# PreferredAI/cornac

Hardware: AMD Instinct MI355X
Metric: bpr_triplets_per_sec (higher is better)
Workload: dtype f32

## Files before the change

cornac_amd/_lib.py:

```python
import ctypes as C
import os
import subprocess

import numpy as np

_HERE = os.path.dirname(os.path.abspath(__file__))
PROFILE = os.environ.get("CORNAC_HIP_PROFILE", "") == "1"
LIB_PATH = os.path.join(_HERE, "lib", "libcornac_hip_profile.so" if PROFILE else "libcornac_hip.so")
CSRC = os.path.join(_HERE, "csrc")

MODE_DETERMINISTIC = 0
MODE_HOGWILD = 1
VEBPR_NO_OWNERSHIP = 0x100
HOG_FORM_MASK, HOG_FORM_SHIFT = 0xF0000, 16
FORM_AUTO, FORM_FUSED, FORM_STRATA, FORM_LDSBIN = (f << HOG_FORM_SHIFT for f in range(4))
HOG_PLAIN_STORES, HOG_VEC4_LAYOUT, HOG_NO_OWNERSHIP, HOG_DENSE_BIAS, HOG_SHARE_NEG = 1, 2, 4, 8, 16
HOG_BINNED, HOG_FUSED_OPT_OUT = 64, 128
HOG_ABLATE_MASK, HOG_ABLATE_SHIFT = 0xFF00, 8
NEG_UNIFORM = 0
NEG_POPULARITY = 1

SYMBOLS = [
    "cornac_hip_last_error", "cornac_hip_version", "cornac_hip_device_count", "cornac_hip_device_info",
    "cornac_hip_device_probe",
    "cornac_hip_bpr_create", "cornac_hip_bpr_destroy", "cornac_hip_bpr_set_factors", "cornac_hip_bpr_get_factors",
    "cornac_hip_bpr_bind_device", "cornac_hip_bpr_rebind_items", "cornac_hip_bpr_conveyor_setup", "cornac_hip_bpr_conveyor_layout", "cornac_hip_bpr_conveyor_enqueue", "cornac_hip_bpr_set_negative_population", "cornac_hip_bpr_device_ptrs", "cornac_hip_bpr_set_stream",
    "cornac_hip_bpr_seed_mt19937", "cornac_hip_bpr_seed_hogwild", "cornac_hip_bpr_fit_epochs",
    "cornac_hip_bpr_set_factors_f64", "cornac_hip_bpr_get_factors_f64", "cornac_hip_bpr_fit_epochs_f64",
    "cornac_hip_bpr_hogwild_enqueue", "cornac_hip_bpr_sync", "cornac_hip_bpr_debug_draw",
    "cornac_hip_bpr_last_timing", "cornac_hip_bpr_kernel_timing", "cornac_hip_mf_kernel_timing",
    "cornac_hip_bpr_debug_ownership", "cornac_hip_bpr_set_views", "cornac_hip_bpr_seed_view_stream",
    "cornac_hip_vebpr_fit_epochs", "cornac_hip_vebpr_fit_epochs_f64", "cornac_hip_vebpr_hogwild_form",
    "cornac_hip_mmmf_fit_epochs", "cornac_hip_mmmf_fit_epochs_f64", "cornac_hip_mmmf_hogwild_enqueue",
    "cornac_hip_bpr_strata_config", "cornac_hip_bpr_chunk_records", "cornac_hip_bpr_strata_stats", "cornac_hip_bpr_debug_strata",
    "cornac_hip_bpr_ldsbin_config", "cornac_hip_bpr_ldsbin_pass_config", "cornac_hip_bpr_ldsbin_stats",
    "cornac_hip_bpr_ldsbin_deal_config", "cornac_hip_bpr_debug_ldsbin_deal",
    "cornac_hip_bpr_sample_triplets", "cornac_hip_bpr_apply_triplets", "cornac_hip_bpr_gather_rows",
    "cornac_hip_bpr_staged_slots", "cornac_hip_bpr_emit_triplets", "cornac_hip_bpr_apply_staged",
    "cornac_hip_bpr_shard_mark", "cornac_hip_bpr_shard_slots", "cornac_hip_bpr_shard_uniq",
    "cornac_hip_bpr_scatter_diff_rows", "cornac_hip_bpr_switch_stream",
    "cornac_hip_bpr_scatter_add_rows", "cornac_hip_bpr_table_delta_begin", "cornac_hip_bpr_table_delta_finish",
    "cornac_hip_bpr_table_delta_step", "cornac_hip_table_delta", "cornac_hip_bpr_table_delta",
    "cornac_hip_bpr_resident_exchange_bins", "cornac_hip_bpr_epoch_resident_enqueue", "cornac_hip_bpr_resident_flush",
    "cornac_hip_stream_wait_counter", "cornac_hip_stream_set_flag", "cornac_hip_stream_ring_standin",
    "cornac_hip_vbpr_create", "cornac_hip_vbpr_destroy", "cornac_hip_vbpr_set_params", "cornac_hip_vbpr_get_params",
    "cornac_hip_vbpr_fit_batches", "cornac_hip_vbpr_item_tables",
    "cornac_hip_wmf_create", "cornac_hip_wmf_destroy", "cornac_hip_wmf_set_factors", "cornac_hip_wmf_get_factors",
    "cornac_hip_wmf_fit_batches", "cornac_hip_wmf_kernel_timing", "cornac_hip_wmf_last_timing",
    "cornac_hip_mf_create", "cornac_hip_mf_destroy", "cornac_hip_mf_set_factors", "cornac_hip_mf_get_factors",
    "cornac_hip_mf_fit", "cornac_hip_mf_bind_items", "cornac_hip_mf_bind_users", "cornac_hip_mf_set_stream", "cornac_hip_mf_epoch_enqueue",
    "cornac_hip_mf_sync", "cornac_hip_mf_fit_sgd", "cornac_hip_mf_last_timing",
    "cornac_hip_mf_hogwild_form", "cornac_hip_mf_hogwild_stats", "cornac_hip_mf_debug_split", "cornac_hip_mf_debug_ownership",
    "cornac_hip_mf_fit_minibatch", "cornac_hip_mf_fit_minibatch_dropout", "cornac_hip_mf_reset_optimizer",
    "cornac_hip_mf_pmf_set_factors", "cornac_hip_mf_pmf_get_factors", "cornac_hip_mf_pmf_fit", "cornac_hip_mf_pmf_form",
    "cornac_hip_mf_nmf_set_factors", "cornac_hip_mf_nmf_get_factors", "cornac_hip_mf_nmf_fit", "cornac_hip_mf_nmf_form",
    "cornac_hip_mf_hpf_set_tables", "cornac_hip_mf_hpf_get_tables", "cornac_hip_mf_hpf_fit", "cornac_hip_mf_hpf_elog",
    "cornac_hip_mf_hpf_form",
    "cornac_hip_scorer_create", "cornac_hip_scorer_destroy", "cornac_hip_scorer_set", "cornac_hip_score_user",
    "cornac_hip_scorer_set_f64", "cornac_hip_score_user_f64",
    "cornac_hip_score_block", "cornac_hip_rank_topk", "cornac_hip_rank_topk_device", "cornac_hip_score_pairs",
    "cornac_hip_scorer_set_exclusions", "cornac_hip_rank_topk_resident", "cornac_hip_scorer_host_buffer",
    "cornac_hip_rank_positions",
    "cornac_hip_knn_sim_create", "cornac_hip_knn_sim_destroy", "cornac_hip_knn_sim_run", "cornac_hip_knn_sim_nnz",
    "cornac_hip_knn_sim_get",
    "cornac_hip_knn_scorer_create", "cornac_hip_knn_scorer_destroy", "cornac_hip_knn_scorer_score_users",
    "cornac_hip_knn_scorer_score_pairs",
    "cornac_hip_ease_create", "cornac_hip_ease_destroy", "cornac_hip_ease_gram", "cornac_hip_ease_invert",
    "cornac_hip_ease_weights", "cornac_hip_ease_fit", "cornac_hip_ease_get_table", "cornac_hip_ease_set_table",
    "cornac_hip_ease_score_users", "cornac_hip_ease_score_pairs",
    "cornac_hip_vaecf_create", "cornac_hip_vaecf_destroy", "cornac_hip_vaecf_set_params", "cornac_hip_vaecf_get_params",
    "cornac_hip_vaecf_get_state", "cornac_hip_vaecf_reset_optimizer", "cornac_hip_vaecf_fit_epoch",
    "cornac_hip_vaecf_encode_users", "cornac_hip_vaecf_score_users", "cornac_hip_vaecf_score_pairs",
]


class HipError(RuntimeError):

    def __init__(self, code, msg):
        super().__init__("libcornac_hip error %d: %s" % (code, msg))
        self.code = code


def build(force=False, verbose=False):
    cmd = ["make", "-C", CSRC, "-j", "4"] + (["-B"] if force else []) + (["PROFILE=1"] if PROFILE else [])
    out = subprocess.run(cmd, stdout=subprocess.PIPE, stderr=subprocess.STDOUT, text=True)
    if verbose or out.returncode != 0:
        print(out.stdout)
    if out.returncode != 0:
        raise RuntimeError("building libcornac_hip.so failed")
    return LIB_PATH


_lib = None

_f32 = np.ctypeslib.ndpointer(np.float32, flags="C_CONTIGUOUS")
_i32 = np.ctypeslib.ndpointer(np.int32, flags="C_CONTIGUOUS")
_i64 = np.ctypeslib.ndpointer(np.int64, flags="C_CONTIGUOUS")
_vp = C.c_void_p


def _preload_torch_hip_runtime():
    import importlib.util
    import sys

    if "torch" in sys.modules:
        return
    try:
        spec = importlib.util.find_spec("torch")
        libdir = os.path.join(list(spec.submodule_search_locations)[0], "lib")
    except Exception:
        return
    for name in ("libhsa-runtime64.so", "libamdhip64.so"):
        path = os.path.join(libdir, name)
        if os.path.exists(path):
            try:
                C.CDLL(path, mode=C.RTLD_GLOBAL)
            except OSError:
                return


def lib():
    global _lib
    if _lib is None:
        if not os.path.exists(LIB_PATH):
            raise RuntimeError(
                "libcornac_hip.so not found at %s. Build it with `python -c 'import __graft_entry__ as g; g.build()'` "
                "or `make -C cornac_amd/csrc`. cornac_amd has no CPU fallback." % LIB_PATH)
        _preload_torch_hip_runtime()
        L = C.CDLL(LIB_PATH)
        L.cornac_hip_last_error.restype = C.c_char_p
        L.cornac_hip_version.restype = C.c_char_p
        L.cornac_hip_device_count.argtypes = [C.POINTER(C.c_int)]
        L.cornac_hip_device_info.argtypes = [C.c_int, C.c_char_p, C.c_int, C.POINTER(C.c_int), C.POINTER(C.c_int64)]
        L.cornac_hip_device_probe.argtypes = [C.c_int, C.c_int64, C.POINTER(C.c_double)]
        L.cornac_hip_bpr_create.argtypes = [C.POINTER(_vp), C.c_int, C.c_int64, C.c_int64, C.c_int64, C.c_int64,
                                            C.c_int, _i32, _i32, C.c_int64]
        L.cornac_hip_bpr_destroy.argtypes = [_vp]
        L.cornac_hip_bpr_set_factors.argtypes = [_vp, _vp, _vp, _vp]
        L.cornac_hip_bpr_get_factors.argtypes = [_vp, _vp, _vp, _vp]
        L.cornac_hip_bpr_bind_device.argtypes = [_vp, _vp, _vp, _vp]
        L.cornac_hip_bpr_rebind_items.argtypes = [_vp, _vp, _vp]
        L.cornac_hip_bpr_conveyor_setup.argtypes = [_vp, C.c_int, _vp, C.c_uint64, C.c_int, C.POINTER(C.c_int), C.POINTER(C.c_int),
                                                    C.POINTER(C.c_int)]
        L.cornac_hip_bpr_conveyor_layout.argtypes = [_vp, C.c_uint32, _vp, _vp]
        L.cornac_hip_bpr_conveyor_enqueue.argtypes = [_vp, C.c_uint32, C.c_uint32, C.c_int, C.POINTER(C.c_int32), C.POINTER(_vp),
                                                      C.c_float, C.c_float, C.c_int, C.c_int, C.c_int]
        L.cornac_hip_bpr_set_negative_population.argtypes = [_vp, _vp, C.c_int64]
        L.cornac_hip_bpr_device_ptrs.argtypes = [_vp, C.POINTER(_vp), C.POINTER(_vp), C.POINTER(_vp)]
        L.cornac_hip_bpr_set_stream.argtypes = [_vp, _vp]
        L.cornac_hip_bpr_switch_stream.argtypes = [_vp, _vp]
        L.cornac_hip_bpr_seed_mt19937.argtypes = [_vp, C.c_uint32, C.c_uint32, C.c_int]
        L.cornac_hip_bpr_seed_hogwild.argtypes = [_vp, C.c_uint64]
        L.cornac_hip_bpr_fit_epochs.argtypes = [_vp, C.c_int, C.c_float, C.c_float, C.c_int, C.c_int, C.c_int,
                                                C.c_int, C.POINTER(C.c_int64), C.POINTER(C.c_int64)]
        L.cornac_hip_bpr_set_factors_f64.argtypes = [_vp, _vp, _vp, _vp]
        L.cornac_hip_bpr_get_factors_f64.argtypes = [_vp, _vp, _vp, _vp]
        L.cornac_hip_bpr_fit_epochs_f64.argtypes = [_vp, C.c_int, C.c_double, C.c_double, C.c_int, C.c_int,
                                                    C.POINTER(C.c_int64), C.POINTER(C.c_int64)]
        L.cornac_hip_bpr_hogwild_enqueue.argtypes = [_vp, C.c_int64, C.c_float, C.c_float, C.c_int, C.c_int, C.c_int]
        L.cornac_hip_bpr_sync.argtypes = [_vp, C.POINTER(C.c_int64), C.POINTER(C.c_int64)]
        L.cornac_hip_bpr_debug_draw.argtypes = [_vp, C.c_int, C.c_uint64, C.c_int64, _i64]
        L.cornac_hip_bpr_last_timing.argtypes = [_vp, C.POINTER(C.c_double)]
        L.cornac_hip_bpr_set_views.argtypes = [_vp, _i32, _i32, C.c_int64]
        L.cornac_hip_bpr_seed_view_stream.argtypes = [_vp, C.c_uint32]
        L.cornac_hip_vebpr_hogwild_form.argtypes = [_vp, C.POINTER(C.c_int)]
        L.cornac_hip_vebpr_fit_epochs.argtypes = [_vp, C.c_int, C.c_float, C.c_float, C.c_float, C.c_int,
                                                  C.POINTER(C.c_int64), C.POINTER(C.c_int64)]
        L.cornac_hip_vebpr_fit_epochs_f64.argtypes = [_vp, C.c_int, C.c_double, C.c_double, C.c_double,
                                                      C.POINTER(C.c_int64), C.POINTER(C.c_int64)]
        L.cornac_hip_mmmf_fit_epochs.argtypes = [_vp, C.c_int, C.c_float, C.c_float, C.c_int, C.POINTER(C.c_int64),
                                                 C.POINTER(C.c_int64)]
        L.cornac_hip_mmmf_fit_epochs_f64.argtypes = [_vp, C.c_int, C.c_double, C.c_double, C.POINTER(C.c_int64),
                                                     C.POINTER(C.c_int64)]
        L.cornac_hip_mmmf_hogwild_enqueue.argtypes = [_vp, C.c_int64, C.c_float, C.c_float]
        L.cornac_hip_bpr_sample_triplets.argtypes = [_vp, C.c_int64, C.c_int, _vp, _vp, _vp]
        L.cornac_hip_bpr_apply_triplets.argtypes = [_vp, _vp, _vp, _vp, C.c_int64, _vp, _vp, C.c_int, C.c_float,
                                                    C.c_float, C.c_int]
        L.cornac_hip_bpr_gather_rows.argtypes = [_vp, _vp, _vp, C.c_int64, C.c_int, _vp]
        L.cornac_hip_bpr_staged_slots.argtypes = [_vp, C.c_int64, C.POINTER(C.c_int64)]
        L.cornac_hip_bpr_emit_triplets.argtypes = [_vp, C.c_int64, C.c_int, _vp, _vp, _vp, C.c_int64, C.POINTER(C.c_int64)]
        L.cornac_hip_bpr_apply_staged.argtypes = [_vp, _vp, _vp, _vp, C.c_int64, _vp, _vp, C.c_int, C.c_float, C.c_float,
                                                  C.c_int]
        L.cornac_hip_bpr_shard_mark.argtypes = [_vp, _vp, _vp, C.c_int64, C.c_int, C.c_int64, _vp]
        L.cornac_hip_bpr_shard_slots.argtypes = [_vp, _vp, _vp, C.c_int64, C.c_int, C.c_int64, _vp, _vp, _vp]
        L.cornac_hip_bpr_shard_uniq.argtypes = [_vp, _vp, _vp, C.c_int64, C.c_int64, _vp]
        L.cornac_hip_bpr_scatter_diff_rows.argtypes = [_vp, _vp, _vp, C.c_int64, C.c_int, _vp, _vp, _vp]
        L.cornac_hip_bpr_scatter_add_rows.argtypes = [_vp, _vp, _vp, C.c_int64, C.c_int, _vp]
        L.cornac_hip_bpr_table_delta_begin.argtypes = [_vp, _vp, _vp, C.c_int64, C.c_int, _vp, _vp]
        L.cornac_hip_bpr_table_delta_finish.argtypes = [_vp, _vp, _vp, _vp, _vp, C.c_int64, C.c_int]
        L.cornac_hip_bpr_table_delta_step.argtypes = [_vp, _vp, _vp, _vp, _vp, C.c_int64, C.c_int, _vp, _vp]
        L.cornac_hip_table_delta.argtypes = [C.c_int, C.c_int, _vp, _vp, _vp, _vp, _vp, C.c_int64, C.c_int, _vp, _vp]
        L.cornac_hip_bpr_table_delta.argtypes = [_vp, C.c_int, C.c_int, _vp, _vp, _vp, _vp, C.c_int64, C.c_int, _vp, _vp]
        L.cornac_hip_bpr_resident_exchange_bins.argtypes = [_vp, C.c_int, C.c_int, C.POINTER(C.c_int)]
        L.cornac_hip_bpr_epoch_resident_enqueue.argtypes = [_vp, C.c_float, C.c_float, C.c_int, C.c_int, C.c_int, C.c_int,
                                                            C.c_int, _vp, _vp, C.c_int64, _vp, C.c_int64, _vp, _vp, _vp,
                                                            C.POINTER(C.c_int)]
        L.cornac_hip_bpr_resident_flush.argtypes = [_vp, C.c_int, C.c_int, _vp, _vp, C.c_int64, _vp, C.c_int64, _vp, _vp]
        L.cornac_hip_stream_wait_counter.argtypes = [C.c_int, _vp, _vp, C.c_uint32, _vp, C.c_int]
        L.cornac_hip_stream_set_flag.argtypes = [C.c_int, _vp, _vp, C.c_uint32, _vp]
        L.cornac_hip_stream_ring_standin.argtypes = [C.c_int, _vp, _vp, C.c_int64, _vp, C.c_int64, C.c_int64, C.c_int]
        L.cornac_hip_bpr_debug_ownership.argtypes = [_vp, C.POINTER(C.c_int64), _vp, _vp, _vp]
        L.cornac_hip_bpr_strata_config.argtypes = [_vp, C.c_int, C.c_int, C.c_int]
        L.cornac_hip_bpr_chunk_records.argtypes = [_vp, C.c_int]
        L.cornac_hip_bpr_strata_stats.argtypes = [_vp, C.POINTER(C.c_int64)]
        L.cornac_hip_bpr_debug_strata.argtypes = [_vp, C.c_uint32, _vp, _vp, _vp, _vp, C.POINTER(C.c_uint32)]
        L.cornac_hip_bpr_ldsbin_config.argtypes = [_vp, C.c_int, C.c_int, C.c_int]
        L.cornac_hip_bpr_ldsbin_pass_config.argtypes = [_vp, C.c_int, C.c_int, C.c_int, C.c_int]
        L.cornac_hip_bpr_ldsbin_stats.argtypes = [_vp, C.POINTER(C.c_int64)]
        L.cornac_hip_bpr_ldsbin_deal_config.argtypes = [_vp, C.c_int, C.c_int]
        L.cornac_hip_bpr_debug_ldsbin_deal.argtypes = [_vp, C.c_uint64, C.c_uint32, _vp, _vp, _vp, _vp, _vp]
        L.cornac_hip_bpr_kernel_timing.argtypes = [_vp, C.c_int, C.POINTER(C.c_double), C.POINTER(C.c_int64)]
        L.cornac_hip_mf_kernel_timing.argtypes = [_vp, C.c_int, C.POINTER(C.c_double), C.POINTER(C.c_int64)]
        L.cornac_hip_vbpr_create.argtypes = [C.POINTER(_vp), C.c_int, C.c_int64, C.c_int64, C.c_int, C.c_int, C.c_int, _f32]
        L.cornac_hip_vbpr_destroy.argtypes = [_vp]
        L.cornac_hip_vbpr_set_params.argtypes = [_vp] + [_vp] * 6
        L.cornac_hip_vbpr_get_params.argtypes = [_vp] + [_vp] * 6
        L.cornac_hip_vbpr_fit_batches.argtypes = [_vp, _i32, _i32, _i32, C.c_int64, C.c_int, C.c_float, C.c_float,
                                                  C.c_float, C.c_float, C.POINTER(C.c_double)]
        L.cornac_hip_vbpr_item_tables.argtypes = [_vp, _f32, _f32]
        L.cornac_hip_mf_fit_minibatch.argtypes = [_vp, _i64, C.c_int64, C.c_int, C.c_int, C.c_float, C.c_float,
                                                  C.c_float, C.c_int, C.POINTER(C.c_double)]
        L.cornac_hip_mf_fit_minibatch_dropout.argtypes = [_vp, _i64, C.c_int64, C.c_int, C.c_int, C.c_float, C.c_float,
                                                          C.c_float, C.c_int, _vp, _vp, C.c_float, C.POINTER(C.c_double)]
        L.cornac_hip_mf_reset_optimizer.argtypes = [_vp]
        L.cornac_hip_mf_pmf_set_factors.argtypes = [_vp, _vp, _vp]
        L.cornac_hip_mf_pmf_get_factors.argtypes = [_vp, _vp, _vp]
        L.cornac_hip_mf_pmf_fit.argtypes = [_vp, C.c_int, C.c_float, C.c_float, C.c_float, C.c_int, _vp]
        L.cornac_hip_mf_pmf_form.argtypes = [_vp, C.POINTER(C.c_int), C.POINTER(C.c_int)]
        L.cornac_hip_mf_nmf_set_factors.argtypes = [_vp, _vp, _vp, _vp, _vp]
        L.cornac_hip_mf_nmf_get_factors.argtypes = [_vp, _vp, _vp, _vp, _vp]
        L.cornac_hip_mf_nmf_fit.argtypes = [_vp, C.c_int] + [C.c_float] * 6 + [C.c_int, C.c_int, _vp]
        L.cornac_hip_mf_nmf_form.argtypes = [_vp] + [C.POINTER(C.c_int)] * 3
        L.cornac_hip_mf_hpf_set_tables.argtypes = [_vp] * 5
        L.cornac_hip_mf_hpf_get_tables.argtypes = [_vp] * 7
        L.cornac_hip_mf_hpf_fit.argtypes = [_vp, C.c_int, C.c_int]
        L.cornac_hip_mf_hpf_elog.argtypes = [_vp, _vp, _vp]
        L.cornac_hip_mf_hpf_form.argtypes = [_vp] + [C.POINTER(C.c_int)] * 2
        L.cornac_hip_wmf_create.argtypes = [C.POINTER(_vp), C.c_int, C.c_int64, C.c_int64, C.c_int, _i64, _i32, _f32,
                                            C.c_int64]
        L.cornac_hip_wmf_destroy.argtypes = [_vp]
        L.cornac_hip_wmf_destroy.restype = None
        L.cornac_hip_wmf_set_factors.argtypes = [_vp, _f32, _f32]
        L.cornac_hip_wmf_get_factors.argtypes = [_vp, _f32, _f32]
        L.cornac_hip_wmf_fit_batches.argtypes = [_vp, _i32, _i64, C.c_int64, C.c_float, C.c_float, C.c_float,
                                                 C.c_float, C.c_float, _vp]
        L.cornac_hip_wmf_kernel_timing.argtypes = [_vp, C.c_int]
        L.cornac_hip_wmf_last_timing.argtypes = [_vp, C.POINTER(C.c_double)]
        L.cornac_hip_mf_create.argtypes = [C.POINTER(_vp), C.c_int, C.c_int64, C.c_int64, C.c_int, _i64, _i64, _f32,
                                           C.c_int64]
        L.cornac_hip_mf_destroy.argtypes = [_vp]
        L.cornac_hip_mf_set_factors.argtypes = [_vp, _vp, _vp, _vp, _vp]
        L.cornac_hip_mf_get_factors.argtypes = [_vp, _vp, _vp, _vp, _vp]
        L.cornac_hip_mf_bind_items.argtypes = [_vp, _vp, _vp]
        L.cornac_hip_mf_bind_users.argtypes = [_vp, _vp, _vp]
        L.cornac_hip_mf_set_stream.argtypes = [_vp, _vp]
        L.cornac_hip_mf_epoch_enqueue.argtypes = [_vp, C.c_int, C.c_int, C.c_float, C.c_float, C.c_float, C.c_int]
        L.cornac_hip_mf_sync.argtypes = [_vp, C.POINTER(C.c_double)]
        L.cornac_hip_mf_fit.argtypes = [_vp, C.c_int, C.c_float, C.c_float, C.c_float, C.c_int, C.c_int, C.c_int, _vp,
                                        C.POINTER(C.c_int)]
        L.cornac_hip_mf_fit_sgd.argtypes = [C.c_int, _i64, _i64, _f32, C.c_int64, _f32, _f32, _f32, _f32, C.c_int64,
                                            C.c_int64, C.c_int, C.c_float, C.c_float, C.c_float, C.c_int, C.c_int,
                                            C.c_int, C.c_int, _vp, C.POINTER(C.c_int)]
        L.cornac_hip_mf_last_timing.argtypes = [_vp, C.POINTER(C.c_double)]
        L.cornac_hip_mf_hogwild_form.argtypes = [_vp, C.c_int]
        L.cornac_hip_mf_hogwild_stats.argtypes = [_vp, C.POINTER(C.c_int64)]
        L.cornac_hip_mf_debug_split.argtypes = [_vp, C.POINTER(C.c_int64), C.POINTER(C.c_int64), _vp, _vp]
        L.cornac_hip_mf_debug_ownership.argtypes = [_vp, C.POINTER(C.c_int64), _vp, _vp, _vp]
        L.cornac_hip_scorer_create.argtypes = [C.POINTER(_vp), C.c_int, C.c_int64, C.c_int64, C.c_int]
        L.cornac_hip_scorer_destroy.argtypes = [_vp]
        L.cornac_hip_scorer_set.argtypes = [_vp, _f32, _f32, _vp, _vp]
        L.cornac_hip_score_user.argtypes = [_vp, C.c_int64, _f32]
        L.cornac_hip_scorer_set_f64.argtypes = [_vp, _vp, _vp, _vp, _vp]
        L.cornac_hip_score_user_f64.argtypes = [_vp, C.c_int64, _vp]
        L.cornac_hip_score_block.argtypes = [_vp, _i32, C.c_int64, _f32]
        L.cornac_hip_score_pairs.argtypes = [_vp, _i32, _i32, C.c_int64, C.c_int, C.c_float, C.c_float, _f32]
        L.cornac_hip_rank_topk.argtypes = [_vp, _i32, C.c_int64, C.c_int, _vp, _vp, _i32, _f32]
        L.cornac_hip_rank_positions.argtypes = [_vp, _i32, C.c_int64, _vp, _vp, _vp, _vp, _i32, _i32, _i32, _f32]
        L.cornac_hip_rank_topk_device.argtypes = [_vp, C.c_int64, C.c_int64, C.c_int, C.c_int, C.POINTER(C.c_double)]
        L.cornac_hip_scorer_set_exclusions.argtypes = [_vp, _vp, _vp]
        L.cornac_hip_scorer_host_buffer.argtypes = [_vp, C.c_size_t, C.POINTER(_vp)]
        L.cornac_hip_rank_topk_resident.argtypes = [_vp, _vp, C.c_int64, C.c_int64, C.c_int, _vp, _vp, _vp]
        L.cornac_hip_knn_sim_create.argtypes = [C.POINTER(_vp), C.c_int, C.c_int64, C.c_int64, _vp, _vp, _vp]
        L.cornac_hip_knn_sim_destroy.argtypes = [_vp]
        L.cornac_hip_knn_sim_run.argtypes = [_vp, C.c_int64]
        L.cornac_hip_knn_sim_nnz.argtypes = [_vp, C.POINTER(C.c_int64)]
        L.cornac_hip_knn_sim_get.argtypes = [_vp, _vp, _vp, _vp]
        L.cornac_hip_knn_scorer_create.argtypes = [C.POINTER(_vp), C.c_int, C.c_int64, C.c_int64, C.c_int64] + [_vp] * 6 + [C.c_int]
        L.cornac_hip_knn_scorer_destroy.argtypes = [_vp]
        L.cornac_hip_knn_scorer_score_users.argtypes = [_vp, _vp, C.c_int64, C.c_int, _vp]
        L.cornac_hip_knn_scorer_score_pairs.argtypes = [_vp, _vp, _vp, C.c_int64, C.c_int, _vp]
        L.cornac_hip_ease_create.argtypes = [C.POINTER(_vp), C.c_int, C.c_int64, C.c_int64, _vp, _vp, _vp]
        L.cornac_hip_ease_destroy.argtypes = [_vp]
        L.cornac_hip_ease_gram.argtypes = [_vp]
        L.cornac_hip_ease_invert.argtypes = [_vp, C.c_double]
        L.cornac_hip_ease_weights.argtypes = [_vp, C.c_int]
        L.cornac_hip_ease_fit.argtypes = [_vp, C.c_double, C.c_int]
        L.cornac_hip_ease_get_table.argtypes = [_vp, _vp]
        L.cornac_hip_ease_set_table.argtypes = [_vp, _vp]
        L.cornac_hip_ease_score_users.argtypes = [_vp, _vp, C.c_int64, _vp]
        L.cornac_hip_ease_score_pairs.argtypes = [_vp, _vp, _vp, C.c_int64, _vp]
        L.cornac_hip_vaecf_create.argtypes = [C.POINTER(_vp), C.c_int, C.c_int64, C.c_int64, _vp, _vp, C.c_int, C.c_int, C.c_int,
                                              C.c_int]
        L.cornac_hip_vaecf_destroy.argtypes = [_vp]
        L.cornac_hip_vaecf_set_params.argtypes = [_vp, _vp]
        L.cornac_hip_vaecf_get_params.argtypes = [_vp, _vp]
        L.cornac_hip_vaecf_get_state.argtypes = [_vp, _vp, _vp, C.POINTER(C.c_int64)]
        L.cornac_hip_vaecf_reset_optimizer.argtypes = [_vp]
        L.cornac_hip_vaecf_fit_epoch.argtypes = [_vp, C.c_int64, C.c_float, C.c_float, _vp, C.c_uint64, C.POINTER(C.c_double), _vp]
        L.cornac_hip_vaecf_encode_users.argtypes = [_vp, _vp, C.c_int64, _vp]
        L.cornac_hip_vaecf_score_users.argtypes = [_vp, _vp, C.c_int64, _vp]
        L.cornac_hip_vaecf_score_pairs.argtypes = [_vp, _vp, _vp, C.c_int64, _vp]
        _lib = L
    return _lib


def check(rc):
    if rc != 0:
        raise HipError(rc, lib().cornac_hip_last_error().decode("utf-8", "replace"))


def stream_wait_counter(device, stream, d_counter, target, d_error, timeout_ms=5000):
    check(lib().cornac_hip_stream_wait_counter(int(device), stream, d_counter, int(target), d_error, int(timeout_ms)))


def stream_ring_standin(device, stream, d_src, src_floats, d_dst, dst_floats, n_floats, n_workgroups=16):
    check(lib().cornac_hip_stream_ring_standin(int(device), stream, d_src, int(src_floats), d_dst, int(dst_floats),
                                               int(n_floats), int(n_workgroups)))


def stream_set_flag(device, stream, d_flag, value=1, d_unless=None):
    check(lib().cornac_hip_stream_set_flag(int(device), stream, d_flag, int(value), d_unless))


def device_count():
    n = C.c_int(0)
    check(lib().cornac_hip_device_count(C.byref(n)))
    return n.value


def device_probe(device=0, nbytes=6 << 30):
    o = (C.c_double * 3)()
    check(lib().cornac_hip_device_probe(device, int(nbytes), o))
    return {"d2d_copy_GBps": o[0], "stream_read_GBps": o[1], "row_gather_512B_GBps": o[2], "buffer_bytes": int(nbytes)}


def device_info(device=0):
    name = C.create_string_buffer(256)
    cus = C.c_int()
    mem = C.c_int64()
    check(lib().cornac_hip_device_info(device, name, 256, C.byref(cus), C.byref(mem)))
    return {"name": name.value.decode(), "compute_units": cus.value, "hbm_bytes": mem.value}


def _ptr(a):
    return None if a is None else a.ctypes.data


def _f32c(a):
    return None if a is None else np.ascontiguousarray(a, dtype=np.float32)


class _HandleOwner:
    _DESTROY = None
    _HANDLE = "h"

    def close(self):
        h = getattr(self, self._HANDLE, None)
        if h is not None and h and lib is not None:
            getattr(lib(), self._DESTROY)(h)
            setattr(self, self._HANDLE, None)

    __del__ = close


def _score_by_ids(symbol, h, dtype, users, items=None, width=None, extra=()):
    ids = [np.ascontiguousarray(users, np.int32)] + ([] if items is None else [np.ascontiguousarray(items, np.int32)])
    n = len(ids[0])
    assert all(len(a) == n for a in ids)
    out = np.empty(n if width is None else (n, width), dtype)
    check(getattr(lib(), symbol)(h, *[_ptr(a) for a in ids], n, *extra, _ptr(out)))
    return out


class BprTrainer(_HandleOwner):
    _DESTROY = "cornac_hip_bpr_destroy"

    def __init__(self, indptr, indices, n_users, n_items, total_users, total_items, k, device=0):
        self.indptr = np.ascontiguousarray(indptr, np.int32)
        self.indices = np.ascontiguousarray(indices, np.int32)
        self.shape = (int(total_users), int(total_items), int(k))
        self.nnz = len(self.indices)
        self.n_items = int(n_items)
        self.device, self._stream = int(device), None
        self.h = _vp()
        check(lib().cornac_hip_bpr_create(C.byref(self.h), device, n_users, n_items, total_users, total_items, k,
                                          self.indptr, self.indices, self.nnz))

    def set_factors(self, U=None, V=None, B=None):
        U, V, B = _f32c(U), _f32c(V), _f32c(B)
        tu, ti, k = self.shape
        assert U is None or U.shape == (tu, k)
        assert V is None or V.shape == (ti, k)
        assert B is None or B.shape == (ti,)
        check(lib().cornac_hip_bpr_set_factors(self.h, _ptr(U), _ptr(V), _ptr(B)))

    def get_factors(self):
        tu, ti, k = self.shape
        U, V, B = np.empty((tu, k), np.float32), np.empty((ti, k), np.float32), np.empty(ti, np.float32)
        check(lib().cornac_hip_bpr_get_factors(self.h, U.ctypes.data, V.ctypes.data, B.ctypes.data))
        return U, V, B

    def set_factors_f64(self, U, V, B):
        tu, ti, k = self.shape
        U, V, B = (np.ascontiguousarray(a, np.float64) for a in (U, V, B))
        assert U.shape == (tu, k) and V.shape == (ti, k) and B.shape == (ti,)
        check(lib().cornac_hip_bpr_set_factors_f64(self.h, U.ctypes.data, V.ctypes.data, B.ctypes.data))

    def get_factors_f64(self):
        tu, ti, k = self.shape
        U, V, B = np.empty((tu, k), np.float64), np.empty((ti, k), np.float64), np.empty(ti, np.float64)
        check(lib().cornac_hip_bpr_get_factors_f64(self.h, U.ctypes.data, V.ctypes.data, B.ctypes.data))
        return U, V, B

    def fit_epochs_f64(self, n_epochs, lr, reg, use_bias=True, neg_population=NEG_UNIFORM):
        c, s = C.c_int64(), C.c_int64()
        check(lib().cornac_hip_bpr_fit_epochs_f64(self.h, n_epochs, float(lr), float(reg), int(use_bias), neg_population,
                                                  C.byref(c), C.byref(s)))
        return c.value, s.value

    def get_user_factors(self):
        tu, _, k = self.shape
        U = np.empty((tu, k), np.float32)
        check(lib().cornac_hip_bpr_get_factors(self.h, U.ctypes.data, None, None))
        return U

    def get_item_factors(self):
        _, ti, k = self.shape
        V, B = np.empty((ti, k), np.float32), np.empty(ti, np.float32)
        check(lib().cornac_hip_bpr_get_factors(self.h, None, V.ctypes.data, B.ctypes.data))
        return V, B

    def seed_mt19937(self, seed_pos, seed_neg, shared_stream=False):
        check(lib().cornac_hip_bpr_seed_mt19937(self.h, seed_pos, seed_neg, int(shared_stream)))

    def seed_hogwild(self, seed):
        check(lib().cornac_hip_bpr_seed_hogwild(self.h, int(seed) & 0xFFFFFFFFFFFFFFFF))

    def fit_epochs(self, n_epochs, lr, reg, use_bias=True, neg_population=NEG_UNIFORM, mode=MODE_HOGWILD, flags=0):
        c, s = C.c_int64(), C.c_int64()
        check(lib().cornac_hip_bpr_fit_epochs(self.h, n_epochs, lr, reg, int(use_bias), neg_population, mode, flags,
                                              C.byref(c), C.byref(s)))
        return c.value, s.value

    def hogwild_enqueue(self, n_samples, lr, reg, use_bias=True, neg_population=NEG_UNIFORM, flags=0):
        check(lib().cornac_hip_bpr_hogwild_enqueue(self.h, n_samples, lr, reg, int(use_bias), neg_population, flags))

    def sync(self):
        c, s = C.c_int64(), C.c_int64()
        check(lib().cornac_hip_bpr_sync(self.h, C.byref(c), C.byref(s)))
        return c.value, s.value

    def bind_device(self, dU=None, dV=None, dB=None):
        check(lib().cornac_hip_bpr_bind_device(self.h, dU, dV, dB))

    def set_negative_population(self, items):
        items = np.ascontiguousarray(items if items is not None else [], np.int32)
        check(lib().cornac_hip_bpr_set_negative_population(self.h, items.ctypes.data if len(items) else None, len(items)))

    def rebind_items(self, dV, dB):
        check(lib().cornac_hip_bpr_rebind_items(self.h, dV, dB))

    def conveyor_setup(self, n_blocks, rank_item=None, deal_seed=0, release_item_tables=True):
        order = None if rank_item is None else np.ascontiguousarray(rank_item, np.int32)
        nb, bpb, cap = C.c_int(), C.c_int(), C.c_int()
        check(lib().cornac_hip_bpr_conveyor_setup(self.h, int(n_blocks), None if order is None else order.ctypes.data,
                                                  int(deal_seed) & 0xFFFFFFFFFFFFFFFF, int(bool(release_item_tables)),
                                                  C.byref(nb), C.byref(bpb), C.byref(cap)))
        return nb.value, bpb.value, cap.value

    def conveyor_layout(self, layout_epoch, d_slot_item, d_item_slot):
        check(lib().cornac_hip_bpr_conveyor_layout(self.h, int(layout_epoch), d_slot_item, d_item_slot))

    def conveyor_enqueue(self, epoch, layout_epoch, first_blocks, d_rows, lr, reg, use_bias=True, neg_population=NEG_UNIFORM,
                         flags=0):
        n = len(first_blocks)
        fb = (C.c_int32 * n)(*[int(b) for b in first_blocks])
        rows = (_vp * n)(*[int(p) for p in d_rows])
        check(lib().cornac_hip_bpr_conveyor_enqueue(self.h, int(epoch), int(layout_epoch), n, fb, rows, lr, reg, int(use_bias),
                                                    neg_population, int(flags)))

    def device_ptrs(self):
        u, v, b = _vp(), _vp(), _vp()
        check(lib().cornac_hip_bpr_device_ptrs(self.h, C.byref(u), C.byref(v), C.byref(b)))
        return u.value, v.value, b.value

    def set_stream(self, stream_ptr):
        check(lib().cornac_hip_bpr_set_stream(self.h, stream_ptr))
        self._stream = stream_ptr

    def switch_stream(self, stream_ptr):
        check(lib().cornac_hip_bpr_switch_stream(self.h, stream_ptr))
        self._stream = stream_ptr

    def sample_triplets(self, n_draws, d_u, d_i, d_j, neg_population=NEG_UNIFORM):
        check(lib().cornac_hip_bpr_sample_triplets(self.h, int(n_draws), neg_population, d_u, d_i, d_j))

    def apply_triplets(self, d_u, d_slot_i, d_slot_j, n, d_rows, d_bias, bias_stride, lr, reg, use_bias=True):
        check(lib().cornac_hip_bpr_apply_triplets(self.h, d_u, d_slot_i, d_slot_j, int(n), d_rows, d_bias,
                                                  int(bias_stride), lr, reg, int(use_bias)))

    def staged_slots(self, n_draws):
        n = C.c_int64()
        check(lib().cornac_hip_bpr_staged_slots(self.h, int(n_draws), C.byref(n)))
        return n.value

    def emit_triplets(self, n_draws, d_u, d_i, d_j, slots_cap, neg_population=NEG_UNIFORM):
        n = C.c_int64()
        check(lib().cornac_hip_bpr_emit_triplets(self.h, int(n_draws), neg_population, d_u, d_i, d_j, int(slots_cap),
                                                 C.byref(n)))
        return n.value

    def apply_staged(self, d_u, d_slot_i, d_slot_j, n_slots, d_rows, d_bias, bias_stride, lr, reg, use_bias=True):
        check(lib().cornac_hip_bpr_apply_staged(self.h, d_u, d_slot_i, d_slot_j, int(n_slots), d_rows, d_bias,
                                                int(bias_stride), lr, reg, int(use_bias)))

    def shard_mark(self, d_i, d_j, n, world, rows_per_rank, d_mark):
        check(lib().cornac_hip_bpr_shard_mark(self.h, d_i, d_j, int(n), int(world), int(rows_per_rank), d_mark))

    def shard_slots(self, d_i, d_j, n, world, rows_per_rank, d_scan, d_slot_i, d_slot_j):
        check(lib().cornac_hip_bpr_shard_slots(self.h, d_i, d_j, int(n), int(world), int(rows_per_rank), d_scan, d_slot_i,
                                               d_slot_j))

    def shard_uniq(self, d_mark, d_scan, n_rows, rows_per_rank, d_uniq_local):
        check(lib().cornac_hip_bpr_shard_uniq(self.h, d_mark, d_scan, int(n_rows), int(rows_per_rank), d_uniq_local))

    def scatter_diff_rows(self, d_table, d_ids, n, width, d_now, d_before, d_scale=None):
        check(lib().cornac_hip_bpr_scatter_diff_rows(self.h, d_table, d_ids, int(n), int(width), d_now, d_before, d_scale))

    def _delta(self, op, rule, *args):
        check(lib().cornac_hip_bpr_table_delta(self.h, op, int(rule), *args))

    def table_delta_begin(self, d_flat, d_base, n_items, k, d_bucket, d_local, rule=0):
        if rule:
            return self._delta(0, rule, d_flat, d_base, None, None, int(n_items), int(k), d_bucket, d_local)
        check(lib().cornac_hip_bpr_table_delta_begin(self.h, d_flat, d_base, int(n_items), int(k), d_bucket, d_local))

    def table_delta_finish(self, d_flat, d_base, d_bucket, d_local, n_items, k, rule=0):
        if rule:
            return self._delta(1, rule, d_flat, d_base, d_bucket, d_local, int(n_items), int(k), None, None)
        check(lib().cornac_hip_bpr_table_delta_finish(self.h, d_flat, d_base, d_bucket, d_local, int(n_items), int(k)))

    def table_delta_step(self, d_flat, d_base, d_bucket_prev, d_local_prev, n_items, k, d_bucket, d_local, rule=0):
        if rule:
            return self._delta(2, rule, d_flat, d_base, d_bucket_prev, d_local_prev, int(n_items), int(k), d_bucket, d_local)
        check(lib().cornac_hip_bpr_table_delta_step(self.h, d_flat, d_base, d_bucket_prev, d_local_prev, int(n_items),
                                                    int(k), d_bucket, d_local))

    def resident_exchange_bins(self, neg_population=NEG_UNIFORM, flags=0):
        n = C.c_int()
        check(lib().cornac_hip_bpr_resident_exchange_bins(self.h, neg_population, flags, C.byref(n)))
        return n.value

    def epoch_resident_enqueue(self, lr, reg, use_bias, neg_population, flags, n_exchanges, rule, d_base, d_buckets,
                               bucket_stride, d_keeps, keep_stride, d_arrive, d_landed, d_applied):
        n = C.c_int()
        check(lib().cornac_hip_bpr_epoch_resident_enqueue(self.h, lr, reg, int(use_bias), neg_population, flags,
                                                          int(n_exchanges), int(rule), d_base, d_buckets, int(bucket_stride),
                                                          d_keeps, int(keep_stride), d_arrive, d_landed, d_applied, C.byref(n)))
        return n.value

    def resident_flush(self, n_exchanges, rule, d_base, d_buckets, bucket_stride, d_keeps, keep_stride, d_applied, d_landed=None):
        check(lib().cornac_hip_bpr_resident_flush(self.h, int(n_exchanges), int(rule), d_base, d_buckets, int(bucket_stride),
                                                  d_keeps, int(keep_stride), d_applied, d_landed))

    def gather_rows(self, d_table, d_ids, n, width, d_out):
        check(lib().cornac_hip_bpr_gather_rows(self.h, d_table, d_ids, int(n), int(width), d_out))

    def scatter_add_rows(self, d_table, d_ids, n, width, d_delta):
        check(lib().cornac_hip_bpr_scatter_add_rows(self.h, d_table, d_ids, int(n), int(width), d_delta))

    def debug_draw(self, stream, hi, n):
        out = np.empty(n, np.int64)
        check(lib().cornac_hip_bpr_debug_draw(self.h, stream, hi, n, out))
# ... 129 lines not shown
        nu, ni, k = self.shape
        U, V = np.empty((nu, k), np.float32), np.empty((ni, k), np.float32)
        Bu, Bi = np.empty(nu, np.float32), np.empty(ni, np.float32)
        check(lib().cornac_hip_mf_get_factors(self.h, U.ctypes.data, V.ctypes.data, Bu.ctypes.data, Bi.ctypes.data))
        return U, V, Bu, Bi

    def fit(self, max_iter, lr, reg, mu, use_bias=True, early_stop=False, mode=MODE_HOGWILD):
        loss = np.zeros(max(max_iter, 1), np.float32)
        n = C.c_int()
        check(lib().cornac_hip_mf_fit(self.h, max_iter, lr, reg, mu, int(use_bias), int(early_stop), mode,
                                      loss.ctypes.data, C.byref(n)))
        return loss[:n.value], n.value

    def bind_items(self, d_V, d_Bi):
        check(lib().cornac_hip_mf_bind_items(self.h, d_V, d_Bi))

    def bind_users(self, d_U, d_Bu):
        check(lib().cornac_hip_mf_bind_users(self.h, d_U, d_Bu))

    def set_stream(self, hip_stream):
        check(lib().cornac_hip_mf_set_stream(self.h, hip_stream))
        self._stream = hip_stream

    def epoch_enqueue(self, part, n_parts, lr, reg, mu, use_bias=True):
        check(lib().cornac_hip_mf_epoch_enqueue(self.h, int(part), int(n_parts), lr, reg, mu, int(use_bias)))

    def sync(self):
        l = C.c_double()
        check(lib().cornac_hip_mf_sync(self.h, C.byref(l)))
        return l.value

    def table_delta_begin(self, d_flat, d_base, n_items, k, d_bucket, d_local, rule=0):
        check(lib().cornac_hip_table_delta(0 | (int(rule) << 4), self.device, self._stream, d_flat, d_base, None, None,
                                           int(n_items), int(k), d_bucket, d_local))

    def table_delta_finish(self, d_flat, d_base, d_bucket, d_local, n_items, k, rule=0):
        check(lib().cornac_hip_table_delta(1 | (int(rule) << 4), self.device, self._stream, d_flat, d_base, d_bucket, d_local,
                                           int(n_items), int(k), None, None))

    def table_delta_step(self, d_flat, d_base, d_bucket_prev, d_local_prev, n_items, k, d_bucket, d_local, rule=0):
        check(lib().cornac_hip_table_delta(2 | (int(rule) << 4), self.device, self._stream, d_flat, d_base, d_bucket_prev,
                                           d_local_prev, int(n_items), int(k), d_bucket, d_local))

    OPTIMIZERS = {"sgd": 0, "adam": 1, "rmsprop": 2, "adagrad": 3}

    def fit_minibatch(self, order, batch_size, optimizer, lr, reg, mu, use_bias=True, keep_u=None, keep_i=None,
                      keep_scale=1.0):
        order = np.ascontiguousarray(order, np.int64)
        loss = C.c_double()
        if keep_u is not None:
            keep_u, keep_i = np.ascontiguousarray(keep_u, np.uint8), np.ascontiguousarray(keep_i, np.uint8)
            if keep_u.shape != (len(order), self.shape[2]) or keep_i.shape != keep_u.shape:
                raise ValueError("keep masks must be [len(order), k] = %r, got %r / %r"
                                 % ((len(order), self.shape[2]), keep_u.shape, keep_i.shape))
            check(lib().cornac_hip_mf_fit_minibatch_dropout(self.h, order, len(order), int(batch_size),
                                                            self.OPTIMIZERS[optimizer], lr, reg, mu, int(use_bias),
                                                            keep_u.ctypes.data, keep_i.ctypes.data, float(keep_scale),
                                                            C.byref(loss)))
            return loss.value
        check(lib().cornac_hip_mf_fit_minibatch(self.h, order, len(order), int(batch_size), self.OPTIMIZERS[optimizer],
                                                lr, reg, mu, int(use_bias), C.byref(loss)))
        return loss.value

    def reset_optimizer(self):
        check(lib().cornac_hip_mf_reset_optimizer(self.h))

    PMF_VARIANTS = {"linear": 0, "non_linear": 1}

    def pmf_set_factors(self, U, V):
        nu, ni, k = self.shape
        U, V = np.ascontiguousarray(U, np.float64), np.ascontiguousarray(V, np.float64)
        if U.shape != (nu, k) or V.shape != (ni, k):
            raise ValueError("PMF tables must be %r and %r, got %r and %r" % ((nu, k), (ni, k), U.shape, V.shape))
        check(lib().cornac_hip_mf_pmf_set_factors(self.h, U.ctypes.data, V.ctypes.data))

    def pmf_get_factors(self):
        nu, ni, k = self.shape
        U, V = np.empty((nu, k), np.float64), np.empty((ni, k), np.float64)
        check(lib().cornac_hip_mf_pmf_get_factors(self.h, U.ctypes.data, V.ctypes.data))
        return U, V

    def pmf_fit(self, n_epochs, lr, reg, gamma, variant):
        loss = np.zeros(max(int(n_epochs), 1), np.float64)
        check(lib().cornac_hip_mf_pmf_fit(self.h, int(n_epochs), lr, reg, gamma, self.PMF_VARIANTS.get(variant, variant),
                                          loss.ctypes.data))
        return loss[:max(int(n_epochs), 0)]

    def pmf_form(self):
        form, group = C.c_int(), C.c_int()
        check(lib().cornac_hip_mf_pmf_form(self.h, C.byref(form), C.byref(group)))
        return form.value, group.value

    def nmf_set_factors(self, U, V, Bu=None, Bi=None):
        nu, ni, k = self.shape
        U, V, Bu, Bi = _f32c(U), _f32c(V), _f32c(Bu), _f32c(Bi)
        if U.shape != (nu, k) or V.shape != (ni, k):
            raise ValueError("NMF tables must be %r and %r, got %r and %r" % ((nu, k), (ni, k), U.shape, V.shape))
        if (Bu is not None and Bu.shape != (nu,)) or (Bi is not None and Bi.shape != (ni,)):
            raise ValueError("NMF biases must be (%d,) and (%d,)" % (nu, ni))
        check(lib().cornac_hip_mf_nmf_set_factors(self.h, _ptr(U), _ptr(V), _ptr(Bu), _ptr(Bi)))

    def nmf_get_factors(self):
        nu, ni, k = self.shape
        U, V = np.empty((nu, k), np.float32), np.empty((ni, k), np.float32)
        Bu, Bi = np.empty(nu, np.float32), np.empty(ni, np.float32)
        check(lib().cornac_hip_mf_nmf_get_factors(self.h, U.ctypes.data, V.ctypes.data, Bu.ctypes.data, Bi.ctypes.data))
        return U, V, Bu, Bi

    def nmf_fit(self, n_epochs, lr, lambda_u, lambda_v, lambda_bu, lambda_bi, mu, use_bias=False, mode=MODE_HOGWILD):
        loss = np.zeros(max(int(n_epochs), 1), np.float64)
        check(lib().cornac_hip_mf_nmf_fit(self.h, int(n_epochs), lr, lambda_u, lambda_v, lambda_bu, lambda_bi, mu,
                                          int(bool(use_bias)), int(mode), loss.ctypes.data))
        return loss[:max(int(n_epochs), 0)]

    def nmf_form(self):
        o = [C.c_int(), C.c_int(), C.c_int()]
        check(lib().cornac_hip_mf_nmf_form(self.h, *[C.byref(x) for x in o]))
        return tuple(x.value for x in o)

    HPF_MAX_K = 256

    def hpf_set_tables(self, G_s, G_r, L_s, L_r):
        nu, ni, k = self.shape
        if k > self.HPF_MAX_K:
            raise ValueError("HPF keeps a row's sums in registers: k = %d is above its limit of %d" % (k, self.HPF_MAX_K))
        tables = [np.ascontiguousarray(a, np.float64) for a in (G_s, G_r, L_s, L_r)]
        for a, name, shape in zip(tables, ("G_s", "G_r", "L_s", "L_r"), ((nu, k), (nu, k), (ni, k), (ni, k))):
            if a.shape != shape:
                raise ValueError("HPF table %s must be %r, got %r" % (name, shape, a.shape))
            if not (np.isfinite(a).all() and (a > 0).all()):
                raise ValueError("HPF table %s must be strictly positive and finite" % name)
        check(lib().cornac_hip_mf_hpf_set_tables(self.h, *[a.ctypes.data for a in tables]))

    def hpf_get_tables(self):
        nu, ni, k = self.shape
        out = [np.empty(s, np.float64) for s in ((nu, k), (nu, k), (ni, k), (ni, k), (nu,), (ni,))]
        check(lib().cornac_hip_mf_hpf_get_tables(self.h, *[a.ctypes.data for a in out]))
        return tuple(out)

    def hpf_fit(self, n_iters, hierarchical=True):
        check(lib().cornac_hip_mf_hpf_fit(self.h, int(n_iters), int(bool(hierarchical))))

    def hpf_elog(self):
        nu, ni, k = self.shape
        Lt, Lb = np.empty((nu, k), np.float64), np.empty((ni, k), np.float64)
        check(lib().cornac_hip_mf_hpf_elog(self.h, Lt.ctypes.data, Lb.ctypes.data))
        return Lt, Lb

    def hpf_form(self):
        o = [C.c_int(), C.c_int()]
        check(lib().cornac_hip_mf_hpf_form(self.h, *[C.byref(x) for x in o]))
        return tuple(x.value for x in o)

    def kernel_timing(self, enable=True):
        ms, n = C.c_double(), C.c_int64()
        check(lib().cornac_hip_mf_kernel_timing(self.h, int(enable), C.byref(ms), C.byref(n)))
        return ms.value, n.value

    def hogwild_form(self, form):
        check(lib().cornac_hip_mf_hogwild_form(self.h, int(form)))

    def hogwild_stats(self):
        o = (C.c_int64 * 4)()
        check(lib().cornac_hip_mf_hogwild_stats(self.h, o))
        return {"form_used": o[0], "tiles": o[1], "rows_per_bin": o[2], "gave_up": bool(o[3])}

    def debug_split(self):
        ns, nv = C.c_int64(), C.c_int64()
        check(lib().cornac_hip_mf_debug_split(self.h, C.byref(ns), C.byref(nv), None, None))
        items, ptr = np.empty(ns.value, np.int32), np.zeros(ns.value + 1, np.int32)
        if ns.value:
            check(lib().cornac_hip_mf_debug_split(self.h, C.byref(ns), C.byref(nv), items.ctypes.data, ptr.ctypes.data))
        return items, ptr

    def debug_ownership(self):
        w = C.c_int64()
        check(lib().cornac_hip_mf_debug_ownership(self.h, C.byref(w), None, None, None))
        if w.value == 0:
            return None
        wp = np.empty(w.value + 1, np.int64)
        ou, oi = np.empty(len(self.val), np.int32), np.empty(len(self.val), np.int32)
        check(lib().cornac_hip_mf_debug_ownership(self.h, C.byref(w), wp.ctypes.data, ou.ctypes.data, oi.ctypes.data))
        return wp, ou, oi

    def last_timing(self):
        t = (C.c_double * 4)()
        check(lib().cornac_hip_mf_last_timing(self.h, t))
        return {"schedule_ms": t[1], "sgd_ms": t[2], "total_ms": t[3]}


def mf_fit_sgd(rid, cid, val, U, V, Bu, Bi, lr, reg, mu, max_iter, use_bias, early_stop, mode, device=0):
    loss = np.zeros(max(max_iter, 1), np.float32)
    n = C.c_int()
    check(lib().cornac_hip_mf_fit_sgd(device, np.ascontiguousarray(rid, np.int64), np.ascontiguousarray(cid, np.int64),
                                      np.ascontiguousarray(val, np.float32), len(val), U, V, Bu, Bi, U.shape[0],
                                      V.shape[0], U.shape[1], lr, reg, mu, max_iter, int(use_bias), int(early_stop),
                                      mode, loss.ctypes.data, C.byref(n)))
    return loss[:n.value]


class Scorer(_HandleOwner):
    _DESTROY = "cornac_hip_scorer_destroy"

    def __init__(self, U, V, item_base=None, user_base=None, device=0):
        U, V = _f32c(U), _f32c(V)
        self.n_users, self.k = U.shape
        self.n_items = V.shape[0]
        self.h = _vp()
        check(lib().cornac_hip_scorer_create(C.byref(self.h), device, self.n_users, self.n_items, self.k))
        self.set(U, V, item_base, user_base)

    def set(self, U, V, item_base=None, user_base=None):
        ib, ub = _f32c(item_base), _f32c(user_base)
        check(lib().cornac_hip_scorer_set(self.h, _f32c(U), _f32c(V), _ptr(ib), _ptr(ub)))

    def score_user(self, user):
        out = np.empty(self.n_items, np.float32)
        check(lib().cornac_hip_score_user(self.h, int(user), out))
        return out

    def set_f64(self, U, V, item_base=None, user_base=None):
        U, V = np.ascontiguousarray(U, np.float64), np.ascontiguousarray(V, np.float64)
        assert U.shape == (self.n_users, self.k) and V.shape == (self.n_items, self.k)
        ib = None if item_base is None else np.ascontiguousarray(item_base, np.float64)
        ub = None if user_base is None else np.ascontiguousarray(user_base, np.float64)
        check(lib().cornac_hip_scorer_set_f64(self.h, U.ctypes.data, V.ctypes.data, _ptr(ib), _ptr(ub)))

    def score_user_f64(self, user):
        out = np.empty(self.n_items, np.float64)
        check(lib().cornac_hip_score_user_f64(self.h, int(user), out.ctypes.data))
        return out

    def score_block(self, users):
        users = np.ascontiguousarray(users, np.int32)
        out = np.empty((len(users), self.n_items), np.float32)
        check(lib().cornac_hip_score_block(self.h, users, len(users), out))
        return out

    def score_pairs(self, users, items, clip=None):
        users = np.ascontiguousarray(users, np.int32)
        items = np.ascontiguousarray(items, np.int32)
        out = np.empty(len(users), np.float32)
        lo, hi = (0.0, 0.0) if clip is None else (float(clip[0]), float(clip[1]))
        check(lib().cornac_hip_score_pairs(self.h, users, items, len(users), int(clip is not None), lo, hi, out))
        return out

    def rank_topk(self, users, topk, exclude=None):
        users = np.ascontiguousarray(users, np.int32)
        items = np.empty((len(users), topk), np.int32)
        scores = np.empty((len(users), topk), np.float32)
        ip = ix = None
        if exclude is not None:
            ip = np.ascontiguousarray(exclude[0], np.int64)
            ix = np.ascontiguousarray(exclude[1], np.int32)
        check(lib().cornac_hip_rank_topk(self.h, users, len(users), topk, _ptr(ip), _ptr(ix), items, scores))
        return items, scores

    def rank_positions(self, users, targets, exclude=None):
        users = np.ascontiguousarray(users, np.int32)
        tp = np.ascontiguousarray(targets[0], np.int64)
        tx = np.ascontiguousarray(targets[1], np.int32)
        nt = int(tp[-1])
        greater, pos, ge = (np.empty(nt, np.int32) for _ in range(3))
        scores = np.empty(nt, np.float32)
        ip = ix = None
        if exclude is not None:
            ip = np.ascontiguousarray(exclude[0], np.int64)
            ix = np.ascontiguousarray(exclude[1], np.int32)
        check(lib().cornac_hip_rank_positions(self.h, users, len(users), _ptr(ip), _ptr(ix), _ptr(tp), _ptr(tx), greater,
                                              pos, ge, scores))
        return greater, pos, ge, scores

    def set_exclusions(self, indptr=None, indices=None):
        if indptr is None:
            check(lib().cornac_hip_scorer_set_exclusions(self.h, None, None))
            return
        ip = np.ascontiguousarray(indptr, np.int64)
        ix = np.ascontiguousarray(indices, np.int32)
        assert len(ip) == self.n_users + 1
        check(lib().cornac_hip_scorer_set_exclusions(self.h, ip.ctypes.data, _ptr(ix) if len(ix) else None))

    def rank_topk_resident(self, users, topk, fetch=True, timed=False, pinned=False):
        if isinstance(users, tuple):
            up, u0, n = None, int(users[0]), int(users[1])
        else:
            ua = np.ascontiguousarray(users, np.int32)
            up, u0, n = ua.ctypes.data, 0, len(ua)
        if fetch and pinned:
            want_scores = fetch != "items"
            nbytes = n * topk * 4 * (2 if want_scores else 1)
            buf = _vp()
            check(lib().cornac_hip_scorer_host_buffer(self.h, nbytes, C.byref(buf)))
            raw = (C.c_char * nbytes).from_address(buf.value)
            items = np.frombuffer(raw, np.int32, n * topk).reshape(n, topk)
            scores = np.frombuffer(raw, np.float32, n * topk, offset=n * topk * 4).reshape(n, topk) if want_scores else None
        else:
            items = np.empty((n, topk), np.int32) if fetch else None
            scores = np.empty((n, topk), np.float32) if fetch and fetch != "items" else None
        ms = C.c_double()
        check(lib().cornac_hip_rank_topk_resident(self.h, up, u0, n, topk, _ptr(items), _ptr(scores),
                                                  C.cast(C.byref(ms), _vp) if timed else None))
        return (items, scores, ms.value) if timed else (items, scores)

    def rank_topk_device_ms(self, u0, n, topk, repeats=1):
        ms = C.c_double()
        check(lib().cornac_hip_rank_topk_device(self.h, u0, n, topk, repeats, C.byref(ms)))
        return ms.value


class VbprTrainer(_HandleOwner):
    _DESTROY = "cornac_hip_vbpr_destroy"
    NAMES = ("Bi", "Gu", "Gi", "Tu", "E", "Bp")

    def __init__(self, features, n_users, n_items, k, k2, device=0):
        self.F = np.ascontiguousarray(features, np.float32)
        assert self.F.shape[0] == n_items
        self.dims = dict(n_users=int(n_users), n_items=int(n_items), k=int(k), k2=int(k2), n_feat=self.F.shape[1])
        self.h = _vp()
        check(lib().cornac_hip_vbpr_create(C.byref(self.h), device, n_users, n_items, k, k2, self.F.shape[1], self.F))

    def _shapes(self):
        d = self.dims
        return {"Bi": (d["n_items"],), "Gu": (d["n_users"], d["k"]), "Gi": (d["n_items"], d["k"]),
                "Tu": (d["n_users"], d["k2"]), "E": (d["n_feat"], d["k2"]), "Bp": (d["n_feat"],)}

    def set_params(self, **params):
        arrs = []
        for n in self.NAMES:
            a = params.get(n)
            if a is not None:
                a = np.ascontiguousarray(np.asarray(a, np.float32).reshape(self._shapes()[n]))
            arrs.append(a)
        check(lib().cornac_hip_vbpr_set_params(self.h, *[_ptr(a) for a in arrs]))

    def get_params(self):
        out = {n: np.empty(s, np.float32) for n, s in self._shapes().items()}
        check(lib().cornac_hip_vbpr_get_params(self.h, *[out[n].ctypes.data for n in self.NAMES]))
        return out

    def fit_batches(self, u, i, j, batch_size, lr, lambda_w, lambda_b, lambda_e):
        u, i, j = (np.ascontiguousarray(x, np.int32) for x in (u, i, j))
        nll = C.c_double()
        check(lib().cornac_hip_vbpr_fit_batches(self.h, u, i, j, len(u), batch_size, lr, lambda_w, lambda_b, lambda_e,
                                                C.byref(nll)))
        return nll.value

    def item_tables(self):
        d = self.dims
        th, vb = np.empty((d["n_items"], d["k2"]), np.float32), np.empty(d["n_items"], np.float32)
        check(lib().cornac_hip_vbpr_item_tables(self.h, th, vb))
        return th, vb


class WmfTrainer(_HandleOwner):
    _DESTROY = "cornac_hip_wmf_destroy"

    def __init__(self, csc, k, device=0):
        csc = csc.tocsc()
        self.n_users, self.n_items = (int(x) for x in csc.shape)
        self.k = int(k)
        self._indptr = np.ascontiguousarray(csc.indptr, np.int64)
        self._rows = np.ascontiguousarray(csc.indices, np.int32)
        self._vals = np.ascontiguousarray(csc.data, np.float32)
        self.h = _vp()
        check(lib().cornac_hip_wmf_create(C.byref(self.h), device, self.n_users, self.n_items, self.k, self._indptr,
                                          self._rows if len(self._rows) else np.zeros(1, np.int32),
                                          self._vals if len(self._vals) else np.zeros(1, np.float32), len(self._vals)))

    def set_factors(self, U, V):
        U = np.ascontiguousarray(np.asarray(U, np.float32).reshape(self.n_users, self.k))
        V = np.ascontiguousarray(np.asarray(V, np.float32).reshape(self.n_items, self.k))
        check(lib().cornac_hip_wmf_set_factors(self.h, U, V))

    def get_factors(self):
        U, V = np.empty((self.n_users, self.k), np.float32), np.empty((self.n_items, self.k), np.float32)
        check(lib().cornac_hip_wmf_get_factors(self.h, U, V))
        return U, V

    def fit_batches(self, batches, lambda_u, lambda_v, a, b, lr):
        batches = [np.asarray(x, np.int32).ravel() for x in batches]
        if not batches:
            return np.zeros(0)
        ptr = np.zeros(len(batches) + 1, np.int64)
        np.cumsum([len(x) for x in batches], out=ptr[1:])
        ids = np.ascontiguousarray(np.concatenate(batches), np.int32)
        loss = np.zeros(len(batches), np.float64)
        check(lib().cornac_hip_wmf_fit_batches(self.h, ids, ptr, len(batches), lambda_u, lambda_v, a, b, lr,
                                               loss.ctypes.data))
        return loss

    def kernel_timing(self, enabled=True):
        check(lib().cornac_hip_wmf_kernel_timing(self.h, int(enabled)))

    def last_device_ms(self):
        ms = C.c_double()
        check(lib().cornac_hip_wmf_last_timing(self.h, C.byref(ms)))
        return ms.value


KNN_MAX_K = 64


def _csr_arrays(mat):
    mat = mat.tocsr()
    if not mat.has_sorted_indices:
        mat = mat.sorted_indices()
    return (np.ascontiguousarray(mat.indptr, np.int64), np.ascontiguousarray(mat.indices, np.int32),
            np.ascontiguousarray(mat.data, np.float64))


class KnnSimilarity(_HandleOwner):
    _DESTROY = "cornac_hip_knn_sim_destroy"

    def __init__(self, W, device=0):
        self.shape = tuple(int(x) for x in W.shape)
        self._csr = _csr_arrays(W)
        self.h = _vp()
        check(lib().cornac_hip_knn_sim_create(C.byref(self.h), device, self.shape[0], self.shape[1],
                                              *[_ptr(a) for a in self._csr]))

    def run(self, rows_per_pass=0):
        import scipy.sparse as sp

        check(lib().cornac_hip_knn_sim_run(self.h, int(rows_per_pass)))
        nnz = C.c_int64()
        check(lib().cornac_hip_knn_sim_nnz(self.h, C.byref(nnz)))
        n = self.shape[0]
        indptr, indices, data = np.empty(n + 1, np.int64), np.empty(nnz.value, np.int32), np.empty(nnz.value, np.float64)
        check(lib().cornac_hip_knn_sim_get(self.h, _ptr(indptr), _ptr(indices), _ptr(data)))
        return sp.csr_matrix((data, indices, indptr.astype(np.int32) if nnz.value < 2 ** 31 else indptr), shape=(n, n))


class KnnScorer(_HandleOwner):
    _DESTROY = "cornac_hip_knn_scorer_destroy"

    MAX_K = KNN_MAX_K

    def __init__(self, N, Q, user_mode, device=0):
        self.n_items, self.n_neighbours = (int(x) for x in N.shape)
        self.n_users = int(Q.shape[0])
        assert int(Q.shape[1]) == self.n_neighbours, "N and Q must have the same number of columns"
        n, q = _csr_arrays(N), _csr_arrays(Q)
        self.h = _vp()
        check(lib().cornac_hip_knn_scorer_create(C.byref(self.h), device, self.n_items, self.n_neighbours, self.n_users,
                                                 *[_ptr(a) for a in n + q], int(bool(user_mode))))

    def score_users(self, users, k):
        return _score_by_ids("cornac_hip_knn_scorer_score_users", self.h, np.float64, users, width=self.n_items, extra=(int(k),))

    def score_pairs(self, users, items, k):
        return _score_by_ids("cornac_hip_knn_scorer_score_pairs", self.h, np.float64, users, items, extra=(int(k),))


class EaseModel(_HandleOwner):
    _DESTROY = "cornac_hip_ease_destroy"

    def __init__(self, X, device=0):
        self.n_users, self.n_items = (int(x) for x in X.shape)
        csr = _csr_arrays(X)
        self.h = _vp()
        check(lib().cornac_hip_ease_create(C.byref(self.h), device, self.n_users, self.n_items, *[_ptr(a) for a in csr]))

    def gram(self):
        check(lib().cornac_hip_ease_gram(self.h))

    def invert(self, lamb):
        check(lib().cornac_hip_ease_invert(self.h, float(lamb)))

    def weights(self, posB):
        check(lib().cornac_hip_ease_weights(self.h, int(bool(posB))))

    def fit(self, lamb, posB):
        check(lib().cornac_hip_ease_fit(self.h, float(lamb), int(bool(posB))))

    def get_table(self):
        out = np.empty((self.n_items, self.n_items), np.float64)
        check(lib().cornac_hip_ease_get_table(self.h, _ptr(out)))
        return out

    def set_table(self, table):
        table = np.ascontiguousarray(table, np.float64)
        assert table.shape == (self.n_items, self.n_items), "the table is items x items"
        check(lib().cornac_hip_ease_set_table(self.h, _ptr(table)))

    def score_users(self, users):
        return _score_by_ids("cornac_hip_ease_score_users", self.h, np.float64, users, width=self.n_items)

    def score_pairs(self, users, items):
        return _score_by_ids("cornac_hip_ease_score_pairs", self.h, np.float64, users, items)


class VaecfModel(_HandleOwner):
    _DESTROY = "cornac_hip_vaecf_destroy"
    _HANDLE = "h_"
    NAMES = ("encoder.fc0.weight", "encoder.fc0.bias", "enc_mu.weight", "enc_mu.bias", "enc_logvar.weight", "enc_logvar.bias",
             "decoder.fc0.weight", "decoder.fc0.bias", "decoder.fc1.weight", "decoder.fc1.bias")
    ACTS = ("tanh", "sigmoid", "relu", "relu6", "elu")
    LIKELIHOODS = ("mult", "bern", "gaus", "pois")

    @staticmethod
    def shapes(n_items, k, h):
        return dict(zip(VaecfModel.NAMES, ((h, n_items), (h,), (k, h), (k,), (k, h), (k,), (h, k), (h,), (n_items, h), (n_items,))))

    def __init__(self, X, k, h, act_fn="tanh", likelihood="mult", device=0):
        self.n_users, self.n_items = (int(x) for x in X.shape)
        self.k, self.h = int(k), int(h)
        indptr, indices, _ = _csr_arrays(X)
        self.h_ = _vp()
        check(lib().cornac_hip_vaecf_create(C.byref(self.h_), device, self.n_users, self.n_items, _ptr(indptr), _ptr(indices),
                                            self.k, self.h, self.ACTS.index(act_fn), self.LIKELIHOODS.index(likelihood)))

    def _empty(self):
        sh = self.shapes(self.n_items, self.k, self.h)
        return {n: np.empty(sh[n], np.float32) for n in self.NAMES}

    def _pointers(self, tables):
        return (_vp * 10)(*[None if tables.get(n) is None else tables[n].ctypes.data for n in self.NAMES])

    def set_params(self, params):
        sh = self.shapes(self.n_items, self.k, self.h)
        tables = {n: np.ascontiguousarray(a, np.float32) for n, a in params.items() if a is not None}
        for n, a in tables.items():
            assert a.shape == sh[n], "%s is %r, not %r" % (n, a.shape, sh[n])
        check(lib().cornac_hip_vaecf_set_params(self.h_, self._pointers(tables)))

    def get_params(self):
        out = self._empty()
        check(lib().cornac_hip_vaecf_get_params(self.h_, self._pointers(out)))
        return out

    def get_state(self):
        m, v, t = self._empty(), self._empty(), C.c_int64()
        check(lib().cornac_hip_vaecf_get_state(self.h_, self._pointers(m), self._pointers(v), C.byref(t)))
        return m, v, int(t.value)

    def reset_optimizer(self):
        check(lib().cornac_hip_vaecf_reset_optimizer(self.h_))

    def fit_epoch(self, batch_size, lr, beta, eps=None, seed=0):
        if eps is not None:
            eps = np.ascontiguousarray(eps, np.float32)
            assert eps.shape == (self.n_users, self.k)
        steps = np.zeros(max(1, -(-self.n_users // max(int(batch_size), 1))), np.float64)
        total = C.c_double()
        check(lib().cornac_hip_vaecf_fit_epoch(self.h_, int(batch_size), float(lr), float(beta), _ptr(eps),
                                               int(seed) & 0xFFFFFFFFFFFFFFFF, C.byref(total), _ptr(steps)))
        return float(total.value), steps

    def encode_users(self, users):
        return _score_by_ids("cornac_hip_vaecf_encode_users", self.h_, np.float32, users, width=self.h)

    def score_users(self, users):
        return _score_by_ids("cornac_hip_vaecf_score_users", self.h_, np.float32, users, width=self.n_items)

    def score_pairs(self, users, items):
        return _score_by_ids("cornac_hip_vaecf_score_pairs", self.h_, np.float32, users, items)
```

cornac_amd/csrc/score.hip:

```cpp
#include <algorithm>
#include <cmath>
#include <cstdlib>

#include "common.h"

namespace chip {

constexpr int kBlk = 256;
typedef float f32x16 __attribute__((ext_vector_type(16)));
typedef float v4f32 __attribute__((ext_vector_type(4)));

__device__ __forceinline__ uint32_t order_key(float s) {
    const uint32_t b = __float_as_uint(s);
    const uint32_t k = (b & 0x80000000u) ? ~b : (b | 0x80000000u);
    return k ? k : 1u;
}
__device__ __forceinline__ float key_to_float(uint32_t k) {
    const uint32_t b = (k & 0x80000000u) ? (k & 0x7fffffffu) : ~k;
    return __uint_as_float(b);
}

__global__ __launch_bounds__(kBlk) void score_valu_kernel(const float *__restrict__ U, const float *__restrict__ V,
                                                          const float *__restrict__ item_base,
                                                          const float *__restrict__ user_base,
                                                          const int32_t *__restrict__ users, int64_t u0,
                                                          int64_t n_items, int k, int ld, float *__restrict__ out) {
    extern __shared__ float urow[];
    const int64_t b = blockIdx.y;
    const int64_t u = users ? (int64_t)users[b] : u0 + b;
    for (int f = threadIdx.x; f < k; f += kBlk) urow[f] = U[u * ld + f];
    __syncthreads();
    const int64_t i = (int64_t)blockIdx.x * kBlk + threadIdx.x;
    if (i >= n_items) return;
    const float *row = V + i * ld;
    float acc = 0.f;
    for (int f = 0; f < k; ++f) acc = fmaf(urow[f], row[f], acc);
    const float ub = user_base ? user_base[u] : 0.f;
    const float ib = item_base ? item_base[i] : 0.f;
    out[b * n_items + i] = (ib + ub) + acc;
}

__global__ __launch_bounds__(kBlk) void score_pairs_kernel(const float *__restrict__ U, const float *__restrict__ V,
                                                           const float *__restrict__ item_base,
                                                           const float *__restrict__ user_base,
                                                           const int32_t *__restrict__ users,
                                                           const int32_t *__restrict__ items, int64_t n, int k, int ld,
                                                           int do_clip, float lo, float hi, float *__restrict__ out) {
    const int64_t p = (int64_t)blockIdx.x * kBlk + threadIdx.x;
    if (p >= n) return;
    const int64_t u = users[p], i = items[p];
    const float *pu = U + u * ld, *pv = V + i * ld;
    float acc = 0.f;
    for (int f = 0; f < k; ++f) acc = fmaf(pu[f], pv[f], acc);
    float s = ((item_base ? item_base[i] : 0.f) + (user_base ? user_base[u] : 0.f)) + acc;
    if (do_clip) s = fminf(fmaxf(s, lo), hi);
    out[p] = s;
}

template <int KT, int MT>
__global__ __launch_bounds__(kBlk) void score_gemm_mfma_kernel(const float *__restrict__ U,
                                                               const float *__restrict__ V,
                                                               const float *__restrict__ item_base,
                                                               const float *__restrict__ user_base,
                                                               const int32_t *__restrict__ users, int64_t u0,
                                                               int64_t n_rows, int64_t n_items, int k,
                                                               int tiles_per_strip, float *__restrict__ out) {
    const int wave = threadIdx.x >> 6, lane = threadIdx.x & 63;
    const int col = lane & 31, half = lane >> 5;
    const int64_t row_tile0 = ((int64_t)blockIdx.y * (kBlk / 64) + wave) * MT;
    if (row_tile0 * 32 >= n_rows) return;
    float a[MT][KT];
    float ubias[MT];
    int64_t urow[MT];
#pragma unroll
    for (int m = 0; m < MT; ++m) {
        const int64_t r = (row_tile0 + m) * 32 + col;
        const bool ok = r < n_rows;
        const int64_t u = ok ? (users ? (int64_t)users[r] : u0 + r) : 0;
        urow[m] = u;
        const float *p = U + u * (2 * KT) + half;
#pragma unroll
        for (int t = 0; t < KT; ++t) a[m][t] = p[2 * t];
        ubias[m] = 0.f;
    }
    const int64_t n_item_tiles = (n_items + 31) / 32;
    const int64_t t_begin = (int64_t)blockIdx.x * tiles_per_strip;
    const int64_t t_end = min(n_item_tiles, t_begin + tiles_per_strip);
    for (int64_t it = t_begin; it < t_end; ++it) {
        const int64_t item = it * 32 + col;
        const bool iok = item < n_items;
        const float *q = V + (iok ? item : 0) * (2 * KT) + half;
        float bfrag[KT];
#pragma unroll
        for (int t = 0; t < KT; ++t) bfrag[t] = q[2 * t];
        const float ib = (iok && item_base) ? item_base[item] : 0.f;
#pragma unroll
        for (int m = 0; m < MT; ++m) {
            f32x16 acc = {0.f, 0.f, 0.f, 0.f, 0.f, 0.f, 0.f, 0.f, 0.f, 0.f, 0.f, 0.f, 0.f, 0.f, 0.f, 0.f};
#pragma unroll
            for (int t = 0; t < KT; ++t) acc = __builtin_amdgcn_mfma_f32_32x32x2f32(a[m][t], bfrag[t], acc, 0, 0, 0);
            if (iok) {
#pragma unroll
                for (int r = 0; r < 16; ++r) {
                    const int64_t row = (row_tile0 + m) * 32 + (r & 3) + 8 * (r >> 2) + 4 * half;
                    if (row < n_rows) {
                        float ub = 0.f;
                        if (user_base) ub = user_base[users ? (int64_t)users[row] : u0 + row];
                        out[row * n_items + item] = (ib + ub) + acc[r];
                    }
                }
            }
        }
    }
    (void)ubias;
    (void)urow;
}

template <typename T>
__device__ __forceinline__ uint32_t lds_offset(T *p) {
    return (uint32_t)(uintptr_t)(__attribute__((address_space(3))) T *)p;
}

template <int KT, int CAP, bool UB>
__global__ __launch_bounds__(kBlk, ((KT <= 32 || CAP <= 42) ? 2 : 1)) void rank_fused_kernel(const float *__restrict__ U, const float *__restrict__ V,
                                                          const float *__restrict__ item_base,
                                                          const float *__restrict__ user_base,
                                                          const int32_t *__restrict__ users, int64_t u0,
                                                          int64_t n_rows, int64_t n_items, int64_t work_per_wg,
                                                          int topk, const int64_t *__restrict__ excl_indptr,
                                                          const int32_t *__restrict__ excl_indices, int64_t excl_row0,
                                                          const uint32_t *__restrict__ excl_bits,
                                                          const int32_t *__restrict__ perm, float *tau_pub,
                                                          unsigned long long *__restrict__ part, int ablate) {
    constexpr int KP = 2 * KT;
    __shared__ unsigned long long keys[kBlk / 64][32][CAP];
    __shared__ int32_t ipos[3][32];
    __shared__ int cnt[kBlk / 64][32];
    __shared__ float tau[kBlk / 64][32];
    __shared__ float btile[2][32][KP + 1];
    __shared__ uint32_t meta_dump[1];
    __shared__ uint32_t wmask[3][kBlk / 64][32];
    __shared__ float ibase[3][32];
    const int wave = threadIdx.x >> 6, lane = threadIdx.x & 63;
    const int col = lane & 31, half = lane >> 5;
    const int64_t n_item_tiles = (n_items + 31) / 32;
    const int64_t n_row_blocks = (n_rows + 127) / 128;
    const int64_t work_total = n_row_blocks * n_item_tiles;
    int64_t pos = (int64_t)blockIdx.x * work_per_wg;
    const int64_t work_end = min(work_total, pos + work_per_wg);
    int64_t cur_rb = 0;
    float bcur[KT];
    constexpr int STG = (32 * KP / 4 + kBlk - 1) / kBlk;
    v4f32 stg[STG];
    uint32_t voff[STG];
#pragma unroll
    for (int q = 0; q < STG; ++q) {
        const int idx = threadIdx.x + q * kBlk;
        voff[q] = idx < 32 * KP / 4 ? (uint32_t)(((idx / (KP / 4)) * KP + 4 * (idx % (KP / 4))) * 4) : 0u;
    }
    uint32_t stg_a = 0;
    int32_t stg_id = 0;
    const uint32_t *pa = reinterpret_cast<const uint32_t *>(item_base);
    int64_t pa_stride = 0;
    const bool wave0 = __builtin_amdgcn_readfirstlane((int)(threadIdx.x >> 6)) == 0;
    const int32_t *pb = perm;
    auto stage_seek = [&](int64_t it) {
        if (threadIdx.x < 32) {
            pa = reinterpret_cast<const uint32_t *>(item_base) + it * 32 + threadIdx.x;
            pa_stride = 32;
        } else if (excl_bits && threadIdx.x < 32 + 32 * (kBlk / 64) && !(ablate & 32)) {
            const int w = (threadIdx.x - 32) >> 5, rl = (threadIdx.x - 32) & 31;
            pa = excl_bits + ((cur_rb * (kBlk / 64) + w) * 32 + rl) * n_item_tiles + it;
            pa_stride = 1;
        } else {
            pa = reinterpret_cast<const uint32_t *>(item_base);
            pa_stride = 0;
        }
        pb = perm + it * 32 + (threadIdx.x & 31);
    };
    auto stage_load = [&](int64_t it) {
        const char *vb = reinterpret_cast<const char *>(V) + it * (int64_t)(32 * KP * 4);
#pragma unroll
        for (int q = 0; q < STG; ++q) stg[q] = *reinterpret_cast<const v4f32 *>(vb + voff[q]);
        stg_a = *pa;
        pa += pa_stride;
        if (wave0) {
            stg_id = *pb;
            pb += 32;
        }
    };
    uint32_t meta_addr0 = lds_offset(&meta_dump[0]), meta_stride = 0;
    if (threadIdx.x < 32) {
        meta_addr0 = lds_offset(&ibase[0][threadIdx.x]);
        meta_stride = 32 * sizeof(float);
    } else if (excl_bits && threadIdx.x < 32 + 32 * (kBlk / 64)) {
        meta_addr0 = lds_offset(&wmask[0][(threadIdx.x - 32) >> 5][(threadIdx.x - 32) & 31]);
        meta_stride = (kBlk / 64) * 32 * sizeof(uint32_t);
    }
    auto stage_store = [&](int buf, int wbuf) {
#pragma unroll
        for (int q = 0; q < STG; ++q) {
            const int idx = threadIdx.x + q * kBlk;
            if ((q + 1) * kBlk <= 32 * KP / 4 || idx < 32 * KP / 4) {
                float *dst = &btile[buf][idx / (KP / 4)][4 * (idx % (KP / 4))];
                dst[0] = stg[q].x; dst[1] = stg[q].y; dst[2] = stg[q].z; dst[3] = stg[q].w;
            }
        }
        *reinterpret_cast<__attribute__((address_space(3))) uint32_t *>(meta_addr0 + (uint32_t)wbuf * meta_stride) = stg_a;
        if (wave0) ipos[wbuf][threadIdx.x & 31] = stg_id;
    };
    constexpr int FG = KT < 8 ? KT : 8;
    auto load_frags = [&](int buf, int g) {
#pragma unroll
        for (int t = g * FG; t < (g + 1) * FG; ++t) bcur[t] = btile[buf][col][2 * t + half];
    };
    const f32x16 zero16 = {0.f, 0.f, 0.f, 0.f, 0.f, 0.f, 0.f, 0.f, 0.f, 0.f, 0.f, 0.f, 0.f, 0.f, 0.f, 0.f};

    int64_t pos_hi = work_end;
    while (pos_hi > pos) {
        const int64_t rb = (pos_hi - 1) / n_item_tiles;
        cur_rb = rb;
        const int64_t seg_lo = max(pos, rb * n_item_tiles);
        const int64_t t_begin = seg_lo - rb * n_item_tiles;
        const int64_t t_end = pos_hi - rb * n_item_tiles;
        const int64_t seg = (int64_t)blockIdx.x - (rb * n_item_tiles) / work_per_wg;
        pos_hi = seg_lo;
        const int64_t row_tile = rb * (kBlk / 64) + wave;
        if (lane < 32) {
            cnt[wave][lane] = 0;
            const int64_t row = row_tile * 32 + lane;
            float t0 = -INFINITY;
            if (row >= n_rows) t0 = INFINITY;
            else if (t_begin > 0) t0 = __hip_atomic_load(tau_pub + row, __ATOMIC_RELAXED, __HIP_MEMORY_SCOPE_AGENT);
            tau[wave][lane] = t0;
        }
        float a[KT];
        {
            const int64_t r = row_tile * 32 + col;
            const bool ok = r < n_rows;
            const int64_t u = ok ? (users ? (int64_t)users[r] : u0 + r) : 0;
            const float *p = U + u * (2 * KT) + half;
#pragma unroll
            for (int t = 0; t < KT; ++t) a[t] = p[2 * t];
        }
        float ubias[16], thr[16];
        int cnt_r[16];
#pragma unroll
        for (int r = 0; r < 16; ++r) {
            const int rl = (r & 3) + 8 * (r >> 2) + 4 * half;
            const int64_t row = row_tile * 32 + rl;
            const bool row_ok = row < n_rows;
            ubias[r] = 0.f;
            if (user_base && row_ok) ubias[r] = user_base[users ? (int64_t)users[row] : u0 + row];
            thr[r] = row_ok ? -INFINITY : INFINITY;
            cnt_r[r] = 0;
        }
        if (t_begin > 0) {
            __builtin_amdgcn_fence(__ATOMIC_ACQ_REL, "wavefront");
            __builtin_amdgcn_wave_barrier();
#pragma unroll
            for (int r = 0; r < 16; ++r) thr[r] = tau[wave][(r & 3) + 8 * (r >> 2) + 4 * half];
        }
        auto compact = [&](unsigned need_l) __attribute__((always_inline)) {
            unsigned need = __builtin_amdgcn_readlane(need_l, 0) | __builtin_amdgcn_readlane(need_l, 32);
            if (col == 0) {
#pragma unroll
                for (int r = 0; r < 16; ++r) cnt[wave][(r & 3) + 8 * (r >> 2) + 4 * half] = cnt_r[r];
            }
            __builtin_amdgcn_fence(__ATOMIC_ACQ_REL, "wavefront");
            __builtin_amdgcn_wave_barrier();
            while (need) {
                const int rl = __builtin_ctz(need);
                need &= need - 1u;
                const int c = cnt[wave][rl];
                unsigned long long *krow = keys[wave][rl];
                unsigned long long mine = lane < c ? krow[lane] : 0ull;
                if (excl_indptr && !excl_bits) {
                    bool dropped = false;
                    if (mine != 0ull) {
                        const int32_t item = (int32_t)(uint32_t)mine;
                        const int64_t grow = excl_row0 + row_tile * 32 + rl;
                        int64_t lo = excl_indptr[grow], hi = excl_indptr[grow + 1];
                        const int64_t end = hi;
                        while (lo < hi) {
                            const int64_t mid = lo + ((hi - lo) >> 1);
                            if (excl_indices[mid] < item) lo = mid + 1; else hi = mid;
                        }
                        dropped = lo < end && excl_indices[lo] == item;
                    }
                    if (dropped) {
                        mine = 0ull;
                        krow[lane] = 0ull;
                    }
                    __builtin_amdgcn_fence(__ATOMIC_ACQ_REL, "wavefront");
                    __builtin_amdgcn_wave_barrier();
                }
                int rank = 0;
                for (int j0 = 0; j0 < c; j0 += 8) {
                    unsigned long long kj[8];
#pragma unroll
                    for (int q = 0; q < 8; ++q) kj[q] = krow[min(j0 + q, CAP - 1)];
#pragma unroll
                    for (int q = 0; q < 8; ++q) rank += (j0 + q < c && kj[q] > mine) ? 1 : 0;
                }
                const bool live = mine != 0ull;
                const int n_keep = min(__popcll(__ballot(live)), topk);
                const unsigned long long kth_mask = __ballot(live && rank == topk - 1);
                if (lane < CAP) krow[lane] = 0ull;
                if (live && rank < topk) krow[rank] = mine;
                if (kth_mask != 0ull) {
                    const int src = __builtin_ctzll(kth_mask);
                    const unsigned hi = __builtin_amdgcn_readlane((unsigned)(mine >> 32), src);
                    if (lane == 0 && row_tile * 32 + rl < n_rows) tau[wave][rl] = key_to_float(hi);
                }
                if (lane == 0) cnt[wave][rl] = n_keep;
            }
            __builtin_amdgcn_fence(__ATOMIC_ACQ_REL, "wavefront");
            __builtin_amdgcn_wave_barrier();
#pragma unroll
            for (int r = 0; r < 16; ++r) {
                const int rl = (r & 3) + 8 * (r >> 2) + 4 * half;
                thr[r] = tau[wave][rl];
                cnt_r[r] = cnt[wave][rl];
            }
        };
        f32x16 acc_a = zero16, acc_b = zero16;
        int wb = 0;
        float ib_a = 0.f, ib_b = 0.f;
        int32_t id_a = 0, id_b = 0;
        stage_seek(t_begin);
        stage_load(t_begin);
        stage_store(0, 0);
        __syncthreads();
        if (t_begin + 1 < t_end) stage_load(t_begin + 1);
        {
#pragma unroll
            for (int t = 0; t < KT; ++t) bcur[t] = btile[0][col][2 * t + half];
            ib_a = ibase[0][col];
            id_a = ipos[0][col];
#pragma unroll
            for (int t = 0; t < KT; ++t) acc_a = __builtin_amdgcn_mfma_f32_32x32x2f32(a[t], bcur[t], acc_a, 0, 0, 0);
        }
        if (t_begin + 1 < t_end) stage_store(1, 1);
        __syncthreads();
        auto step = [&](int64_t it, f32x16 &acc_cur, f32x16 &acc_nxt, float &ib_cur, float &ib_nxt, int32_t &id_cur,
                        int32_t &id_nxt) __attribute__((always_inline)) {
            const int buf_next = (int)((it + 1 - t_begin) & 1);
            load_frags(buf_next, 0);
            __builtin_amdgcn_sched_barrier(0);
            if (it + 2 < t_end && !(ablate & 2)) stage_load(it + 2);
            const int wb1 = wb == 2 ? 0 : wb + 1, wb2 = wb1 == 2 ? 0 : wb1 + 1;
            ib_nxt = ibase[wb1][col];
            id_nxt = ipos[wb1][col];
            const int32_t item = id_cur;
            unsigned long long hm[16];
            float sc[16];
#pragma unroll
            for (int g = 0; g < KT / FG; ++g) {
                if (g + 1 < KT / FG) load_frags(buf_next, g + 1);
                __builtin_amdgcn_sched_barrier(0);
#pragma unroll
                for (int t = g * FG; t < (g + 1) * FG; ++t) {
                    if (t == 0) acc_nxt = __builtin_amdgcn_mfma_f32_32x32x2f32(a[t], bcur[t], zero16, 0, 0, 0);
                    else acc_nxt = __builtin_amdgcn_mfma_f32_32x32x2f32(a[t], bcur[t], acc_nxt, 0, 0, 0);
                    if (t < 16) {
                        const int r = t;
                        sc[r] = UB ? (ib_cur + ubias[r]) + acc_cur[r] : ib_cur + acc_cur[r];
                        hm[r] = __ballot(sc[r] >= thr[r]);
                    }
                }
                __builtin_amdgcn_sched_barrier(0);
            }
            if (KT < 16) {
#pragma unroll
                for (int r = KT; r < 16; ++r) {
                    sc[r] = UB ? (ib_cur + ubias[r]) + acc_cur[r] : ib_cur + acc_cur[r];
                    hm[r] = __ballot(sc[r] >= thr[r]);
                }
            }
            unsigned long long any = 0ull;
#pragma unroll
            for (int r = 0; r < 16; ++r) any |= hm[r];
            if (ablate & 1) any = 0ull;
            auto drop_excluded = [&]() __attribute__((always_inline)) {
                const uint32_t wv = wmask[wb][wave][col];
                unsigned long long left = 0ull;
#pragma unroll
                for (int r = 0; r < 16; ++r) {
                    if (hm[r] != 0ull) {
                        const int rl = (r & 3) + 8 * (r >> 2);
                        const unsigned long long m = (unsigned long long)(uint32_t)__builtin_amdgcn_readlane(wv, rl) |
                                                     ((unsigned long long)(uint32_t)__builtin_amdgcn_readlane(wv, rl + 4) << 32);
                        hm[r] &= ~m;
                        left |= hm[r];
                    }
                }
                return left;
            };
            if (any != 0ull && excl_bits) any = drop_excluded();
            if (any != 0ull) {
                unsigned over_l = 0;
#pragma unroll
                for (int r = 0; r < 16; ++r) {
                    if (hm[r] != 0ull) {
                        const unsigned mine = half ? (unsigned)(hm[r] >> 32) : (unsigned)hm[r];
                        if (cnt_r[r] + __popc(mine) > CAP) over_l |= 1u << ((r & 3) + 8 * (r >> 2) + 4 * half);
                    }
                }
                if ((__builtin_amdgcn_readlane(over_l, 0) | __builtin_amdgcn_readlane(over_l, 32)) != 0u) {
                    compact(over_l);
#pragma unroll
                    for (int r = 0; r < 16; ++r) hm[r] = __ballot(sc[r] >= thr[r]);
                    if (excl_bits) (void)drop_excluded();
                }
#pragma unroll
                for (int r = 0; r < 16; ++r) {
                    const unsigned long long m = hm[r];
                    if (m != 0ull) {
                        const unsigned mine = half ? (unsigned)(m >> 32) : (unsigned)m;
                        if ((mine >> col) & 1u) {
                            const int rl = (r & 3) + 8 * (r >> 2) + 4 * half;
                            const int slot = cnt_r[r] + __popc(mine & ((1u << col) - 1u));
                            keys[wave][rl][slot] =
                                ((unsigned long long)order_key(sc[r]) << 32) | (unsigned long long)(uint32_t)item;
                        }
                        cnt_r[r] += __popc(mine);
                    }
                }
            }
            if (it + 2 < t_end && !(ablate & 8)) stage_store((int)((it + 2 - t_begin) & 1), wb2);
            if (!(ablate & 4)) __syncthreads();
            wb = wb1;
        };
        for (int64_t it = t_begin; it < t_end; it += 2) {
            step(it, acc_a, acc_b, ib_a, ib_b, id_a, id_b);
            if (it + 1 < t_end) step(it + 1, acc_b, acc_a, ib_b, ib_a, id_b, id_a);
        }
        compact(0xffffffffu);
        for (int rl = 0; rl < 32; ++rl) {
            const int64_t row = row_tile * 32 + rl;
            if (row >= n_rows) break;
            if (lane < topk) part[(seg * n_rows + row) * topk + lane] = keys[wave][rl][lane];
        }
        if (t_begin == 0 && t_end < n_item_tiles && lane < 32 && row_tile * 32 + lane < n_rows)
            __hip_atomic_store(tau_pub + row_tile * 32 + lane, tau[wave][lane], __ATOMIC_RELAXED, __HIP_MEMORY_SCOPE_AGENT);
        __builtin_amdgcn_fence(__ATOMIC_ACQ_REL, "wavefront");
        __builtin_amdgcn_wave_barrier();
    }
}

constexpr int kBitmapChunk = 1024;
constexpr int kBitmapRows = 1;
__global__ __launch_bounds__(kBlk) void excl_bitmap_kernel(const int64_t *__restrict__ indptr,
                                                          const int32_t *__restrict__ indices,
                                                          const int32_t *__restrict__ users, int64_t u0, int by_user,
                                                          const int32_t *__restrict__ inv_perm, int64_t n_rows,
                                                          int64_t n_rows_padded, int64_t n_item_tiles,
                                                          uint32_t *__restrict__ bits) {
    constexpr int NR = kBitmapRows;
    __shared__ uint32_t bm_all[kBlk / 64][NR][kBitmapChunk];
    const int wave = threadIdx.x >> 6, lane = threadIdx.x & 63;
    const int64_t row0 = ((int64_t)blockIdx.x * (kBlk / 64) + wave) * NR;
    if (row0 >= n_rows_padded) return;
    int64_t lo[NR], cnt[NR];
    int64_t cnt_max = 0;
#pragma unroll
    for (int q = 0; q < NR; ++q) {
        lo[q] = 0;
        cnt[q] = 0;
        const int64_t row = row0 + q;
        if (row < n_rows) {
            const int64_t key = by_user ? (users ? (int64_t)users[row] : u0 + row) : row;
            lo[q] = indptr[key];
            cnt[q] = indptr[key + 1] - lo[q];
        }
        cnt_max = max(cnt_max, cnt[q]);
    }
    for (int64_t c0 = 0; c0 < n_item_tiles; c0 += kBitmapChunk) {
        const int nt = (int)min((int64_t)kBitmapChunk, n_item_tiles - c0);
#pragma unroll
        for (int q = 0; q < NR; ++q)
            for (int i = lane; i < nt; i += 64) bm_all[wave][q][i] = 0u;
        __builtin_amdgcn_fence(__ATOMIC_ACQ_REL, "wavefront");
        __builtin_amdgcn_wave_barrier();
        for (int64_t p = lane; p < cnt_max; p += 64) {
            int32_t e[NR], pos[NR];
#pragma unroll
            for (int q = 0; q < NR; ++q) e[q] = p < cnt[q] ? indices[lo[q] + p] : 0;
#pragma unroll
            for (int q = 0; q < NR; ++q) pos[q] = inv_perm[e[q]];
#pragma unroll
            for (int q = 0; q < NR; ++q) {
                const int t = (pos[q] >> 5) - (int)c0;
                if (p < cnt[q] && t >= 0 && t < nt) atomicOr(&bm_all[wave][q][t], 1u << (pos[q] & 31));
            }
        }
        __builtin_amdgcn_fence(__ATOMIC_ACQ_REL, "wavefront");
        __builtin_amdgcn_wave_barrier();
#pragma unroll
        for (int q = 0; q < NR; ++q) {
            if (row0 + q < n_rows_padded)
                for (int i = lane; i < nt; i += 64)
                    __builtin_nontemporal_store(bm_all[wave][q][i], &bits[(row0 + q) * n_item_tiles + c0 + i]);
        }
        __builtin_amdgcn_fence(__ATOMIC_ACQ_REL, "wavefront");
        __builtin_amdgcn_wave_barrier();
    }
}

__global__ __launch_bounds__(64) void rank_merge_kernel(const unsigned long long *__restrict__ part, int n_strips,
                                                        int64_t n_rows, int topk, int pad,
                                                        int32_t *__restrict__ items_out,
                                                        float *__restrict__ scores_out) {
    extern __shared__ unsigned long long mlist[];
    const int64_t row = blockIdx.x;
    const int tid = threadIdx.x;
    const int n = n_strips * topk;
    for (int i = tid; i < pad; i += 64) {
        unsigned long long key = 0ull;
        if (i < n) key = part[((int64_t)(i / topk) * n_rows + row) * topk + (i % topk)];
        mlist[i] = key;
    }
    __syncthreads();
    for (int kk = 2; kk <= pad; kk <<= 1) {
        for (int j = kk >> 1; j > 0; j >>= 1) {
            for (int i = tid; i < pad; i += 64) {
                const int ixj = i ^ j;
                if (ixj > i) {
                    const unsigned long long x = mlist[i], y = mlist[ixj];
                    const bool desc = (i & kk) == 0;
                    if (desc ? (x < y) : (x > y)) {
                        mlist[i] = y;
                        mlist[ixj] = x;
                    }
                }
            }
            __syncthreads();
        }
    }
    for (int i = tid; i < topk; i += 64) {
        const unsigned long long key = mlist[i];
        items_out[row * topk + i] = key ? (int32_t)(uint32_t)key : -1;
        scores_out[row * topk + i] = key ? key_to_float((uint32_t)(key >> 32)) : -INFINITY;
    }
}

__global__ __launch_bounds__(kBlk) void mark_excluded_kernel(const int64_t *__restrict__ excl_indptr,
                                                             const int32_t *__restrict__ excl_indices, int64_t row0,
                                                             int64_t n_items, uint8_t *__restrict__ excl_mask) {
    const int64_t row = blockIdx.x;
    const int64_t lo = excl_indptr[row0 + row], hi = excl_indptr[row0 + row + 1];
    for (int64_t p = lo + threadIdx.x; p < hi; p += kBlk) {
        const int32_t it = excl_indices[p];
        if (it >= 0 && it < n_items) excl_mask[row * n_items + it] = 1;
    }
}

__device__ __forceinline__ unsigned long long composite_key(const float *__restrict__ scores,
                                                            const uint8_t *__restrict__ excl, int64_t i) {
    if (excl && excl[i]) return 0ull;
    return ((unsigned long long)order_key(scores[i]) << 32) | (unsigned long long)(uint32_t)i;
}

constexpr int TOPK_MAX = 2048;

__global__ __launch_bounds__(kBlk) void topk_select_kernel(const float *__restrict__ scores,
                                                           const uint8_t *__restrict__ excl_mask, int64_t n_items,
                                                           int topk, int topk_pad, int32_t *__restrict__ items_out,
                                                           float *__restrict__ scores_out) {
    __shared__ unsigned int hist[256];
    __shared__ unsigned long long sh_prefix;
    __shared__ unsigned int sh_remaining, sh_count;
    extern __shared__ unsigned long long list[];
    const int64_t row = blockIdx.x;
    const float *srow = scores + row * n_items;
    const uint8_t *erow = excl_mask ? excl_mask + row * n_items : nullptr;
    const int tid = threadIdx.x;
    if (tid == 0) {
        sh_prefix = 0ull;
        sh_remaining = (unsigned)topk;
        sh_count = 0;
    }
    __syncthreads();
    for (int pass = 0; pass < 8; ++pass) {
        const int shift = 56 - 8 * pass;
        hist[tid] = 0;
        __syncthreads();
        const unsigned long long prefix = sh_prefix;
        for (int64_t i = tid; i < n_items; i += kBlk) {
            const unsigned long long key = composite_key(srow, erow, i);
            const bool match = pass == 0 ? true : ((key >> (shift + 8)) == prefix);
            if (match) atomicAdd(&hist[(unsigned)(key >> shift) & 255u], 1u);
        }
        __syncthreads();
        if (tid == 0) {
            unsigned int rem = sh_remaining, acc = 0;
            int b = 255;
            for (; b > 0; --b) {
                if (acc + hist[b] >= rem) break;
                acc += hist[b];
            }
            sh_remaining = rem - acc;
            sh_prefix = (prefix << 8) | (unsigned long long)b;
        }
        __syncthreads();
    }
    const unsigned long long thresh = sh_prefix;
    for (int i = tid; i < topk_pad; i += kBlk) list[i] = 0ull;
    __syncthreads();
    for (int64_t i = tid; i < n_items; i += kBlk) {
        const unsigned long long key = composite_key(srow, erow, i);
        if (key >= thresh && key != 0ull) {
            const unsigned int pos = atomicAdd(&sh_count, 1u);
            if (pos < (unsigned)topk_pad) list[pos] = key;
        }
    }
    __syncthreads();
    for (int kk = 2; kk <= topk_pad; kk <<= 1) {
        for (int j = kk >> 1; j > 0; j >>= 1) {
            for (int i = tid; i < topk_pad; i += kBlk) {
                const int ixj = i ^ j;
                if (ixj > i) {
                    const unsigned long long x = list[i], y = list[ixj];
                    const bool desc = (i & kk) == 0;
                    if (desc ? (x < y) : (x > y)) {
                        list[i] = y;
                        list[ixj] = x;
                    }
                }
            }
            __syncthreads();
        }
    }
    for (int i = tid; i < topk; i += kBlk) {
        const unsigned long long key = list[i];
        items_out[row * topk + i] = key ? (int32_t)(uint32_t)key : -1;
        scores_out[row * topk + i] = key ? key_to_float((uint32_t)(key >> 32)) : -INFINITY;
    }
}

constexpr int kSortBlk = 1024;
constexpr int kSortChunk = 8192;
__global__ __launch_bounds__(kSortBlk) void full_sort_kernel(const float *__restrict__ scores,
                                                             const uint8_t *__restrict__ excl_mask, int64_t n_items,
                                                             int64_t n_pad, unsigned long long *__restrict__ scratch,
                                                             int topk, int32_t *__restrict__ items_out,
                                                             float *__restrict__ scores_out) {
    __shared__ unsigned long long lk[kSortChunk];
    const int64_t row = blockIdx.x;
    const float *srow = scores + row * n_items;
    const uint8_t *erow = excl_mask ? excl_mask + row * n_items : nullptr;
    unsigned long long *keys = scratch + row * n_pad;
    const int tid = threadIdx.x;
    const int64_t ch = n_pad < kSortChunk ? n_pad : kSortChunk;
    auto lds_stages = [&](int64_t c0, int64_t kk, int64_t j_hi) {
        for (int64_t j = j_hi; j > 0; j >>= 1) {
            for (int64_t p = tid; p < (ch >> 1); p += kSortBlk) {
                const int64_t i = ((p & ~(j - 1)) << 1) | (p & (j - 1)), ixj = i | j;
                const unsigned long long x = lk[i], y = lk[ixj];
                const bool desc = ((c0 + i) & kk) == 0;
                if (desc ? (x < y) : (x > y)) {
                    lk[i] = y;
                    lk[ixj] = x;
                }
            }
            __syncthreads();
        }
    };
    for (int64_t c0 = 0; c0 < n_pad; c0 += ch) {
        for (int64_t i = tid; i < ch; i += kSortBlk) {
            const int64_t g = c0 + i;
            lk[i] = g < n_items ? composite_key(srow, erow, g) : 0ull;
        }
        __syncthreads();
        for (int64_t kk = 2; kk <= ch; kk <<= 1) lds_stages(c0, kk, kk >> 1);
        for (int64_t i = tid; i < ch; i += kSortBlk) keys[c0 + i] = lk[i];
        __syncthreads();
    }
    for (int64_t kk = ch << 1; kk <= n_pad; kk <<= 1) {
        for (int64_t j = kk >> 1; j >= ch; j >>= 1) {
            for (int64_t p = tid; p < (n_pad >> 1); p += kSortBlk) {
                const int64_t i = ((p & ~(j - 1)) << 1) | (p & (j - 1)), ixj = i | j;
                const unsigned long long x = keys[i], y = keys[ixj];
                const bool desc = (i & kk) == 0;
                if (desc ? (x < y) : (x > y)) {
                    keys[i] = y;
                    keys[ixj] = x;
                }
            }
            __syncthreads();
        }
        for (int64_t c0 = 0; c0 < n_pad; c0 += ch) {
            for (int64_t i = tid; i < ch; i += kSortBlk) lk[i] = keys[c0 + i];
            __syncthreads();
            lds_stages(c0, kk, ch >> 1);
            for (int64_t i = tid; i < ch; i += kSortBlk) keys[c0 + i] = lk[i];
            __syncthreads();
        }
    }
    for (int64_t i = tid; i < topk; i += kSortBlk) {
        const unsigned long long key = keys[i];
        items_out[row * topk + i] = key ? (int32_t)(uint32_t)key : -1;
        scores_out[row * topk + i] = key ? key_to_float((uint32_t)(key >> 32)) : -INFINITY;
    }
}


constexpr int kPosT = 8;
__global__ __launch_bounds__(kBlk) void rank_positions_kernel(const float *__restrict__ scores,
                                                              const uint8_t *__restrict__ excl_mask, int64_t n_items,
                                                              const int64_t *__restrict__ tgt_indptr,
                                                              const int32_t *__restrict__ tgt_indices, int64_t row0,
                                                              int32_t *__restrict__ greater_out,
                                                              int32_t *__restrict__ pos_out,
                                                              int32_t *__restrict__ ge_out,
                                                              float *__restrict__ score_out) {
    const int64_t row = blockIdx.x;
    const float *srow = scores + row * n_items;
    const uint8_t *erow = excl_mask ? excl_mask + row * n_items : nullptr;
    const int64_t lo = tgt_indptr[row0 + row], hi = tgt_indptr[row0 + row + 1];
    __shared__ int cnt[kPosT * 3];
    const int64_t mis = (int64_t)((reinterpret_cast<uintptr_t>(srow) >> 2) & 3);
    const int64_t head = min(n_items, (4 - mis) & 3);
    const int64_t body_end = head + ((n_items - head) & ~int64_t(3));
    const bool vec_mask = !erow || ((reinterpret_cast<uintptr_t>(erow) + head) & 3) == 0;
    for (int64_t t0 = lo; t0 < hi; t0 += kPosT) {
        uint32_t ts[kPosT];
        bool ok[kPosT];
        int32_t titem[kPosT];
#pragma unroll
        for (int q = 0; q < kPosT; ++q) {
            const int64_t t = t0 + q;
            const int32_t item = t < hi ? tgt_indices[t] : -1;
            ok[q] = item >= 0 && item < n_items && !(erow && erow[item]);
            ts[q] = ok[q] ? order_key(srow[item]) : 0xFFFFFFFFu;
            titem[q] = item;
        }
        int g[kPosT], eq[kPosT], tie[kPosT];
#pragma unroll
        for (int q = 0; q < kPosT; ++q) g[q] = eq[q] = tie[q] = 0;
        auto visit = [&](const bool *live, const float *sc, int64_t i, int n) __attribute__((always_inline)) {
            uint32_t oc[4];
            unsigned long long any_eq = 0;
#pragma unroll
            for (int c = 0; c < n; ++c) {
                oc[c] = live[c] ? order_key(sc[c]) : 0u;
#pragma unroll
                for (int q = 0; q < kPosT; ++q) {
                    g[q] += oc[c] > ts[q];
                    any_eq |= __ballot(oc[c] == ts[q]);
                }
            }
            if (any_eq) {
#pragma unroll
                for (int c = 0; c < n; ++c) {
                    asm volatile("" : "+v"(oc[c]));
#pragma unroll
                    for (int q = 0; q < kPosT; ++q) {
                        const bool same = live[c] && oc[c] == ts[q];
                        eq[q] += same;
                        tie[q] += same && (uint32_t)(i + c) > (uint32_t)titem[q];
                    }
                }
            }
        };
        for (int64_t i = threadIdx.x; i < head; i += kBlk) {
            const bool lv = !(erow && erow[i]);
            const float sc = srow[i];
            visit(&lv, &sc, i, 1);
        }
        auto fetch = [&](int64_t i0, v4f32 &sv, uint32_t &em) __attribute__((always_inline)) {
            const bool in = i0 < body_end;
            sv = in ? *reinterpret_cast<const v4f32 *>(srow + i0) : v4f32{0.f, 0.f, 0.f, 0.f};
            em = 0u;
            if (erow && in) {
                if (vec_mask) em = *reinterpret_cast<const uint32_t *>(erow + i0);
                else em = (uint32_t)erow[i0] | ((uint32_t)erow[i0 + 1] << 8) | ((uint32_t)erow[i0 + 2] << 16) | ((uint32_t)erow[i0 + 3] << 24);
            }
        };
        const int64_t i_first = head + 4 * (int64_t)threadIdx.x, i_stop = body_end + 4 * (int64_t)(kBlk - 1);
        v4f32 sv_n = {0.f, 0.f, 0.f, 0.f};
        uint32_t em_n = 0u;
        if (i_first < i_stop) fetch(i_first, sv_n, em_n);
        for (int64_t i0 = i_first; i0 < i_stop; i0 += 4 * kBlk) {
            const v4f32 sv = sv_n;
            const uint32_t em = em_n;
            if (i0 + 4 * kBlk < i_stop) fetch(i0 + 4 * kBlk, sv_n, em_n);
            const bool in = i0 < body_end;
            const bool lv[4] = {in && !(em & 0xffu), in && !(em & 0xff00u), in && !(em & 0xff0000u), in && !(em & 0xff000000u)};
            const float sc[4] = {sv.x, sv.y, sv.z, sv.w};
            visit(lv, sc, i0, 4);
        }
        for (int64_t i = body_end + threadIdx.x; i < n_items; i += kBlk) {
            const bool lv = !(erow && erow[i]);
            const float sc = srow[i];
            visit(&lv, &sc, i, 1);
        }
#pragma unroll
        for (int q = 0; q < kPosT; ++q)
            for (int o = 32; o > 0; o >>= 1) {
                g[q] += __shfl_xor(g[q], o, 64);
                eq[q] += __shfl_xor(eq[q], o, 64);
                tie[q] += __shfl_xor(tie[q], o, 64);
            }
        if (threadIdx.x < kPosT * 3) cnt[threadIdx.x] = 0;
        __syncthreads();
        if ((threadIdx.x & 63) == 0) {
#pragma unroll
            for (int q = 0; q < kPosT; ++q) {
                atomicAdd(&cnt[q * 3 + 0], g[q]);
                atomicAdd(&cnt[q * 3 + 1], g[q] + tie[q]);
                atomicAdd(&cnt[q * 3 + 2], g[q] + eq[q]);
            }
        }
        __syncthreads();
#pragma unroll
        for (int q = 0; q < kPosT; ++q) {
            const int64_t t = t0 + q;
            if (threadIdx.x == q && t < hi) {
                greater_out[t] = ok[q] ? cnt[q * 3 + 0] : -1;
                pos_out[t] = ok[q] ? cnt[q * 3 + 1] : -1;
                ge_out[t] = ok[q] ? cnt[q * 3 + 2] : -1;
                score_out[t] = ok[q] ? srow[titem[q]] : -INFINITY;
            }
        }
        __syncthreads();
    }
}

}

using namespace chip;

struct cornac_hip_scorer {
    int device = 0;
    int64_t n_users = 0, n_items = 0;
    int k = 0;
    int ld = 0;
    hipStream_t stream = nullptr;
    DevBuf<float> U, V, item_base, user_base;
    DevBuf<float> Vr, ibr;
    DevBuf<int32_t> perm, inv_perm;
    DevBuf<uint32_t> excl_bits;
    void *pinned_out = nullptr;
    size_t pinned_bytes = 0;
    std::vector<void *> pinned_retired;
    DevBuf<int64_t> res_excl_indptr;
    DevBuf<int32_t> res_excl_indices;
    bool has_res_excl = false;
    DevBuf<float> tau_pub;
    bool has_user_base = false, is_set = false;
    DevBuf<float> scores;
    DevBuf<uint8_t> excl;
    DevBuf<int32_t> d_users, d_items_out, d_excl_indices;
    DevBuf<int64_t> d_excl_indptr;
    DevBuf<float> d_scores_out;
    DevBuf<int64_t> d_tgt_indptr;
    DevBuf<int32_t> d_tgt_indices, d_tgt_counts;
    DevBuf<float> d_tgt_scores;
    DevBuf<unsigned long long> sort_scratch, part;
    DevBuf<double> U64, V64, ib64, ub64, scores64;
    bool f64_set = false, f64_user_base = false;
};

static __global__ __launch_bounds__(256) void permute_rows_kernel(const float *__restrict__ V, const float *__restrict__ ib,
                                                                  const int32_t *__restrict__ perm, int64_t n, int ld,
                                                                  float *__restrict__ Vr, float *__restrict__ ibr) {
    const int gl = threadIdx.x & 15;
    for (int64_t p = ((int64_t)blockIdx.x * 256 + threadIdx.x) >> 4; p < n; p += ((int64_t)gridDim.x * 256) >> 4) {
        const int64_t src = perm[p];
        for (int f = gl * 4; f < ld; f += 64)
            *reinterpret_cast<v4f32 *>(Vr + p * ld + f) = *reinterpret_cast<const v4f32 *>(V + src * ld + f);
        if (gl == 0) ibr[p] = ib[src];
    }
}

static void build_rank_order(cornac_hip_scorer_t h, const float *U, const float *V, const float *item_base) {
    const int64_t ni = h->n_items, nu = h->n_users;
    const int k = h->k;
    const int64_t sample = std::min<int64_t>(nu, 16384), stride = std::max<int64_t>(1, nu / sample);
    const bool full_cov = (double)ni * k * k <= 4e9;
    std::vector<double> mean((size_t)k, 0.0), cov(full_cov ? (size_t)k * k : 0, 0.0);
    double ss = 0;
    int64_t cnt = 0;
    for (int64_t u = 0; u < nu; u += stride, ++cnt) {
        const float *ur = U + u * k;
        for (int f = 0; f < k; ++f) {
            mean[(size_t)f] += ur[f];
            ss += (double)ur[f] * ur[f];
        }
        if (full_cov)
            for (int f = 0; f < k; ++f)
                for (int g = f; g < k; ++g) cov[(size_t)f * k + g] += (double)ur[f] * ur[g];
    }
    const double inv = 1.0 / (double)std::max<int64_t>(cnt, 1);
    for (int f = 0; f < k; ++f) mean[(size_t)f] *= inv;
    if (full_cov)
        for (int f = 0; f < k; ++f)
            for (int g = f; g < k; ++g) {
                const double c = cov[(size_t)f * k + g] * inv - mean[(size_t)f] * mean[(size_t)g];
                cov[(size_t)f * k + g] = cov[(size_t)g * k + f] = c;
            }
    const double iso = std::max(0.0, ss * inv - [&] { double m2 = 0; for (int f = 0; f < k; ++f) m2 += mean[(size_t)f] * mean[(size_t)f]; return m2; }()) / (double)k;
    std::vector<float> pri((size_t)ni);
    std::vector<double> tmp((size_t)k);
    for (int64_t i = 0; i < ni; ++i) {
        const float *vr = V + i * k;
        double m = 0, var = 0;
        for (int f = 0; f < k; ++f) m += mean[(size_t)f] * vr[f];
        if (full_cov) {
            for (int f = 0; f < k; ++f) {
                double t = 0;
                for (int g = 0; g < k; ++g) t += cov[(size_t)f * k + g] * vr[g];
                var += t * vr[f];
            }
        } else {
            for (int f = 0; f < k; ++f) var += (double)vr[f] * vr[f];
            var *= iso;
        }
        pri[(size_t)i] = (float)((item_base ? (double)item_base[i] : 0.0) + m + 2.0 * std::sqrt(std::max(var, 0.0)));
    }
    std::vector<int32_t> order((size_t)ni);
    for (int64_t i = 0; i < ni; ++i) order[(size_t)i] = (int32_t)i;
    std::stable_sort(order.begin(), order.end(), [&](int32_t a, int32_t b) {
        const float pa = pri[(size_t)a], pb = pri[(size_t)b];
        return (pa > pb) || (pa != pa && pb == pb);
    });
    const int64_t ni_pad = (ni + 31) / 32 * 32;
    h->perm.ensure((size_t)ni_pad);
    h->Vr.ensure((size_t)ni_pad * h->ld);
    h->ibr.ensure((size_t)ni_pad);
    HIP_CHECK(hipMemsetAsync(h->perm.p, 0, (size_t)ni_pad * sizeof(int32_t), h->stream));
    HIP_CHECK(hipMemsetAsync(h->Vr.p, 0, (size_t)ni_pad * h->ld * sizeof(float), h->stream));
    HIP_CHECK(hipMemsetD32Async((hipDeviceptr_t)h->ibr.p, 0x7fc00000u , (size_t)ni_pad, h->stream));
    h->perm.upload(order.data(), (size_t)ni, h->stream);
    std::vector<int32_t> inv_order((size_t)ni);
    for (int64_t p = 0; p < ni; ++p) inv_order[(size_t)order[(size_t)p]] = (int32_t)p;
    h->inv_perm.ensure((size_t)ni);
    h->inv_perm.upload(inv_order.data(), (size_t)ni, h->stream);
    const unsigned grid = (unsigned)std::max<int64_t>(1, std::min<int64_t>((ni * 16 + 255) / 256, 8192));
    hipLaunchKernelGGL(permute_rows_kernel, dim3(grid), dim3(256), 0, h->stream, h->V.p, h->item_base.p, h->perm.p, ni, h->ld,
                       h->Vr.p, h->ibr.p);
    HIP_CHECK(hipGetLastError());
    HIP_CHECK(hipStreamSynchronize(h->stream));
}

static void validate_csr(const int64_t *indptr, const int32_t *indices, int64_t n, int64_t n_items, const char *what) {
    REQUIRE(indptr[0] == 0, "%s_indptr must start at 0", what);
    for (int64_t r = 0; r < n; ++r)
        REQUIRE(indptr[r + 1] >= indptr[r], "%s_indptr decreases at row %lld", what, (long long)r);
    const int64_t ne = indptr[n];
    int32_t lo = 0, hi = 0;
    for (int64_t p = 0; p < ne; ++p) {
        lo = std::min(lo, indices[p]);
        hi = std::max(hi, indices[p]);
    }
    REQUIRE(lo >= 0 && hi < n_items, "%s_indices out of range [0, %lld)", what, (long long)n_items);
}

static void sc_check(cornac_hip_scorer_t h, bool need_set = true) {
    REQUIRE(h != nullptr, "scorer handle is NULL");
    HIP_CHECK(hipSetDevice(h->device));
    if (need_set) REQUIRE(h->is_set, "cornac_hip_scorer_set has not been called");
}

static int64_t rows_per_batch(cornac_hip_scorer_t h) {
    const int64_t cap = (int64_t(2) << 30) / (h->n_items * (int64_t)sizeof(float));
    return std::max<int64_t>(32, std::min<int64_t>(cap / 32 * 32, 16384));
}

static void launch_scores(cornac_hip_scorer_t h, const int32_t *d_users, int64_t u0, int64_t n, bool use_mfma) {
    const float *ub = h->has_user_base ? h->user_base.p : nullptr;
    const int k = h->k;
    if (use_mfma && k <= 128) {
        const int64_t n_item_tiles = (h->n_items + 31) / 32;
        const DeviceInfo &di = device_info(h->device);
        auto go = [&](auto kernel, int MT) {
            const int64_t row_tiles = (n + 31) / 32;
            const int64_t wg_rows = (row_tiles + (int64_t)MT * 4 - 1) / ((int64_t)MT * 4);
            int64_t strips = std::max<int64_t>(1, ((int64_t)di.cus * 8 + wg_rows - 1) / wg_rows);
            strips = std::min(strips, n_item_tiles);
            const int tiles_per_strip = (int)((n_item_tiles + strips - 1) / strips);
            const int64_t gx = (n_item_tiles + tiles_per_strip - 1) / tiles_per_strip;
            hipLaunchKernelGGL(kernel, dim3((unsigned)gx, (unsigned)wg_rows), dim3(kBlk), 0, h->stream, h->U.p, h->V.p,
                               h->item_base.p, ub, d_users, u0, n, h->n_items, k, tiles_per_strip, h->scores.p);
        };
        if (h->ld == 16) go(score_gemm_mfma_kernel<8, 2>, 2);
        else if (h->ld == 32) go(score_gemm_mfma_kernel<16, 2>, 2);
        else if (h->ld == 64) go(score_gemm_mfma_kernel<32, 2>, 2);
        else go(score_gemm_mfma_kernel<64, 1>, 1);
    } else {
        dim3 grid((unsigned)((h->n_items + kBlk - 1) / kBlk), (unsigned)n);
        hipLaunchKernelGGL(score_valu_kernel, grid, dim3(kBlk), (size_t)k * sizeof(float), h->stream, h->U.p, h->V.p,
                           h->item_base.p, ub, d_users, u0, h->n_items, k, h->ld, h->scores.p);
    }
    HIP_CHECK(hipGetLastError());
}

static void launch_rank(cornac_hip_scorer_t h, int64_t n, int topk, bool have_excl, int32_t *items_out,
                        float *scores_out) {
    const uint8_t *excl = have_excl ? h->excl.p : nullptr;
    if (topk <= TOPK_MAX) {
        int pad = 1;
        while (pad < topk) pad <<= 1;
        hipLaunchKernelGGL(topk_select_kernel, dim3((unsigned)n), dim3(kBlk), (size_t)pad * 8, h->stream, h->scores.p,
                           excl, h->n_items, topk, pad, items_out, scores_out);
    } else {
        int64_t pad = 1;
        while (pad < h->n_items) pad <<= 1;
        h->sort_scratch.ensure((size_t)(n * pad));
        hipLaunchKernelGGL(full_sort_kernel, dim3((unsigned)n), dim3(kSortBlk), 0, h->stream, h->scores.p, excl,
                           h->n_items, pad, h->sort_scratch.p, topk, items_out, scores_out);
    }
    HIP_CHECK(hipGetLastError());
}

constexpr int kFusedMaxTopk = 32;

static bool can_fuse(cornac_hip_scorer_t h, int topk) { return topk <= kFusedMaxTopk && h->k <= 128; }

constexpr int64_t kMaxBitmapTiles = 8192;

static void launch_rank_fused_rows(cornac_hip_scorer_t h, const int32_t *d_users, int64_t u0, int64_t n, int topk,
                                   const int64_t *d_excl_indptr, const int32_t *d_excl_indices, int64_t excl_row0,
                                   int32_t *items_out, float *scores_out, bool excl_by_user) {
    const float *ub = h->has_user_base ? h->user_base.p : nullptr;
    const DeviceInfo &di = device_info(h->device);
    const int ablate = prof_env_int("CORNAC_HIP_RANK_ABLATE", 0);
    const int64_t n_item_tiles = (h->n_items + 31) / 32;
    const int64_t wg_rows = (n + 127) / 128;
    const int wgs_per_cu = (h->ld <= 64 || topk <= 10) ? 2 : 1;
    const int64_t work_total = wg_rows * n_item_tiles;
    int64_t work_per_wg = std::max<int64_t>((work_total + (int64_t)di.cus * wgs_per_cu - 1) / ((int64_t)di.cus * wgs_per_cu),
                                            std::min<int64_t>(16, n_item_tiles));
    const int64_t n_wgs = (work_total + work_per_wg - 1) / work_per_wg;
    const int64_t max_segs = (n_item_tiles + work_per_wg - 1) / work_per_wg + 1;
    h->part.ensure((size_t)(max_segs * n * topk));
    HIP_CHECK(hipMemsetAsync(h->part.p, 0, (size_t)(max_segs * n * topk) * sizeof(unsigned long long), h->stream));
    h->tau_pub.ensure((size_t)n);
    HIP_CHECK(hipMemsetD32Async((hipDeviceptr_t)h->tau_pub.p, 0xff800000u , (size_t)n, h->stream));
    const uint32_t *d_bits = nullptr;
    const bool no_bitmap = prof_env_set("CORNAC_HIP_RANK_NO_BITMAP");
    if (d_excl_indptr && n_item_tiles <= kMaxBitmapTiles && !no_bitmap) {
        const int64_t rows_padded = wg_rows * 128;
        h->excl_bits.ensure((size_t)(rows_padded * n_item_tiles));
        hipLaunchKernelGGL(excl_bitmap_kernel, dim3((unsigned)((rows_padded + kBitmapRows * (kBlk / 64) - 1) / (kBitmapRows * (kBlk / 64)))), dim3(kBlk), 0,
                           h->stream, d_excl_indptr + (excl_by_user ? 0 : excl_row0), d_excl_indices, d_users, u0,
                           excl_by_user ? 1 : 0, h->inv_perm.p, n, rows_padded, n_item_tiles, h->excl_bits.p);
        d_bits = h->excl_bits.p;
    } else if (d_excl_indptr) {
        REQUIRE(!excl_by_user, "resident exclusion lists need the bitmap path (catalogue too large)");
    }
    dim3 grid((unsigned)n_wgs), block(kBlk);
#define FUSED(KT_, CAP_) do {                                                                                    \
    if (prof_env_set("CORNAC_HIP_RANK_ABLATE")) {                                                                 \
        int occ = 0;                                                                                              \
        (void)hipOccupancyMaxActiveBlocksPerMultiprocessor(&occ, rank_fused_kernel<KT_, CAP_, true>, kBlk, 0);     \
        fprintf(stderr, "[rank_fused<%d,%d>] %u workgroups x %lld block-tiles, <= %lld segments/row, %d workgroups/CU\n", \
                KT_, CAP_, grid.x, (long long)work_per_wg, (long long)max_segs, occ);                              \
    }                                                                                                             \
    if (ub)                                                                                                       \
        hipLaunchKernelGGL((rank_fused_kernel<KT_, CAP_, true>), grid, block, 0, h->stream, h->U.p, h->Vr.p,       \
                           h->ibr.p, ub, d_users, u0, n, h->n_items, work_per_wg, topk, d_bits ? nullptr : d_excl_indptr, \
                           d_excl_indices, excl_row0, d_bits, h->perm.p, h->tau_pub.p, h->part.p, ablate);       \
    else                                                                                                          \
        hipLaunchKernelGGL((rank_fused_kernel<KT_, CAP_, false>), grid, block, 0, h->stream, h->U.p, h->Vr.p,      \
                           h->ibr.p, ub, d_users, u0, n, h->n_items, work_per_wg, topk, d_bits ? nullptr : d_excl_indptr, \
                           d_excl_indices, excl_row0, d_bits, h->perm.p, h->tau_pub.p, h->part.p, ablate); } while (0)
    if (topk <= 10 && h->ld == 128) {
        FUSED(64, 42);
    } else if (topk <= 24) {
        if (h->ld == 16) FUSED(8, 56);
        else if (h->ld == 32) FUSED(16, 56);
        else if (h->ld == 64) FUSED(32, 56);
        else FUSED(64, 56);
    } else {
        if (h->ld == 16) FUSED(8, 64);
        else if (h->ld == 32) FUSED(16, 64);
        else if (h->ld == 64) FUSED(32, 64);
        else FUSED(64, 64);
    }
#undef FUSED
    int pad = 1;
    while (pad < (int)max_segs * topk) pad <<= 1;
    hipLaunchKernelGGL(rank_merge_kernel, dim3((unsigned)n), dim3(64), (size_t)pad * 8, h->stream, h->part.p,
                       (int)max_segs, n, topk, pad, items_out, scores_out);
    HIP_CHECK(hipGetLastError());
}

constexpr int64_t kExclBitmapBudget = int64_t(512) << 20;
static void launch_rank_fused(cornac_hip_scorer_t h, const int32_t *d_users, int64_t u0, int64_t n, int topk,
                              const int64_t *d_excl_indptr, const int32_t *d_excl_indices, int64_t excl_row0,
                              int32_t *items_out, float *scores_out, bool excl_by_user = false) {
    const int64_t n_item_tiles = (h->n_items + 31) / 32;
    int64_t rows = n;
    if (d_excl_indptr && n_item_tiles <= kMaxBitmapTiles)
        rows = std::max<int64_t>(128, (kExclBitmapBudget / (n_item_tiles * 4)) / 128 * 128);
    for (int64_t r0 = 0; r0 < n; r0 += rows) {
        const int64_t m = std::min(rows, n - r0);
        launch_rank_fused_rows(h, d_users ? d_users + r0 : nullptr, u0 + r0, m, topk, d_excl_indptr, d_excl_indices,
                               excl_row0 + r0, items_out + r0 * topk, scores_out ? scores_out + r0 * topk : nullptr,
                               excl_by_user);
    }
}

extern "C" {

int cornac_hip_scorer_create(cornac_hip_scorer_t *out, int device, int64_t n_users, int64_t n_items, int k) {
    return guarded([&] {
        REQUIRE(out != nullptr, "out handle pointer is NULL");
        *out = nullptr;
        REQUIRE(n_users > 0 && n_items > 0 && k > 0, "n_users, n_items and k must be positive");
        REQUIRE(n_items < (int64_t(1) << 31), "n_items exceeds int32");
        use_device(device);
        std::unique_ptr<cornac_hip_scorer> h(new cornac_hip_scorer());
        h->device = device; h->n_users = n_users; h->n_items = n_items; h->k = k;
        h->ld = k <= 16 ? 16 : k <= 32 ? 32 : k <= 64 ? 64 : k <= 128 ? 128 : k;
        HIP_CHECK(hipStreamCreateWithFlags(&h->stream, hipStreamNonBlocking));
        h->U.alloc((size_t)n_users * h->ld);
        h->V.alloc((size_t)n_items * h->ld);
        HIP_CHECK(hipMemsetAsync(h->U.p, 0, h->U.n * sizeof(float), h->stream));
        HIP_CHECK(hipMemsetAsync(h->V.p, 0, h->V.n * sizeof(float), h->stream));
        HIP_CHECK(hipStreamSynchronize(h->stream));
        h->item_base.alloc((size_t)n_items);
        h->user_base.alloc((size_t)n_users);
        *out = h.release();
    });
}

int cornac_hip_scorer_destroy(cornac_hip_scorer_t h) {
    return guarded([&] {
        if (!h) return;
        (void)hipSetDevice(h->device);
        if (h->stream) {
            (void)hipStreamSynchronize(h->stream);
            (void)hipStreamDestroy(h->stream);
        }
        if (h->pinned_out) (void)hipHostFree(h->pinned_out);
        for (void *q : h->pinned_retired) (void)hipHostFree(q);
        delete h;
    });
}

int cornac_hip_scorer_set(cornac_hip_scorer_t h, const float *U, const float *V, const float *item_base,
                          const float *user_base) {
    return guarded([&] {
        sc_check(h, false);
        REQUIRE(U && V, "U and V are required");
        HIP_CHECK(hipMemcpy2DAsync(h->U.p, (size_t)h->ld * 4, U, (size_t)h->k * 4, (size_t)h->k * 4, (size_t)h->n_users,
                                   hipMemcpyHostToDevice, h->stream));
        HIP_CHECK(hipMemcpy2DAsync(h->V.p, (size_t)h->ld * 4, V, (size_t)h->k * 4, (size_t)h->k * 4, (size_t)h->n_items,
                                   hipMemcpyHostToDevice, h->stream));
        if (item_base) h->item_base.upload(item_base, (size_t)h->n_items, h->stream);
        else HIP_CHECK(hipMemsetAsync(h->item_base.p, 0, (size_t)h->n_items * 4, h->stream));
        h->has_user_base = user_base != nullptr;
        if (user_base) h->user_base.upload(user_base, (size_t)h->n_users, h->stream);
        build_rank_order(h, U, V, item_base);
        HIP_CHECK(hipStreamSynchronize(h->stream));
        h->is_set = true;
    });
}

int cornac_hip_score_user(cornac_hip_scorer_t h, int64_t user, float *out) {
    return guarded([&] {
        sc_check(h);
        REQUIRE(user >= 0 && user < h->n_users, "user %lld out of range", (long long)user);
        REQUIRE(out != nullptr, "out is NULL");
        h->scores.ensure((size_t)h->n_items);
        launch_scores(h, nullptr, user, 1, false);
        h->scores.download(out, (size_t)h->n_items, h->stream);
        HIP_CHECK(hipStreamSynchronize(h->stream));
    });
}

namespace chip {
__global__ __launch_bounds__(256) void score_user_f64_kernel(const double *__restrict__ u, const double *__restrict__ V,
                                                             const double *__restrict__ item_base, double user_base,
                                                             int64_t n_items, int k, double *__restrict__ out) {
    const int64_t i = (int64_t)blockIdx.x * 256 + threadIdx.x;
    if (i >= n_items) return;
    double acc = 0.0;
    const double *v = V + i * k;
    for (int f = 0; f < k; ++f) acc = acc + u[f] * v[f];
    out[i] = (item_base ? item_base[i] : 0.0) + user_base + acc;
}
}

int cornac_hip_scorer_set_f64(cornac_hip_scorer_t h, const double *U, const double *V, const double *item_base,
                              const double *user_base) {
    return guarded([&] {
        sc_check(h, false);
        REQUIRE(U && V, "U and V are required");
        h->U64.ensure((size_t)h->n_users * h->k);
        h->V64.ensure((size_t)h->n_items * h->k);
        h->U64.upload(U, (size_t)h->n_users * h->k, h->stream);
        h->V64.upload(V, (size_t)h->n_items * h->k, h->stream);
        h->ib64.ensure((size_t)h->n_items);
        if (item_base) h->ib64.upload(item_base, (size_t)h->n_items, h->stream);
        else HIP_CHECK(hipMemsetAsync(h->ib64.p, 0, (size_t)h->n_items * sizeof(double), h->stream));
        h->f64_user_base = user_base != nullptr;
        if (user_base) {
            h->ub64.ensure((size_t)h->n_users);
            h->ub64.upload(user_base, (size_t)h->n_users, h->stream);
        }
        h->scores64.ensure((size_t)h->n_items);
        HIP_CHECK(hipStreamSynchronize(h->stream));
        h->f64_set = true;
    });
}

int cornac_hip_score_user_f64(cornac_hip_scorer_t h, int64_t user, double *out) {
    return guarded([&] {
        sc_check(h, false);
        REQUIRE(h->f64_set, "no float64 tables (cornac_hip_scorer_set_f64)");
        REQUIRE(user >= 0 && user < h->n_users, "user %lld out of range", (long long)user);
        REQUIRE(out != nullptr, "out is NULL");
        double ub = 0.0;
        if (h->f64_user_base) HIP_CHECK(hipMemcpyAsync(&ub, h->ub64.p + user, sizeof ub, hipMemcpyDeviceToHost, h->stream));
        if (h->f64_user_base) HIP_CHECK(hipStreamSynchronize(h->stream));
        hipLaunchKernelGGL(score_user_f64_kernel, dim3((unsigned)((h->n_items + 255) / 256)), dim3(256), 0, h->stream,
                           h->U64.p + (size_t)user * h->k, h->V64.p, h->ib64.p, ub, h->n_items, h->k, h->scores64.p);
        HIP_CHECK(hipGetLastError());
        h->scores64.download(out, (size_t)h->n_items, h->stream);
        HIP_CHECK(hipStreamSynchronize(h->stream));
    });
}

int cornac_hip_score_block(cornac_hip_scorer_t h, const int32_t *users, int64_t n, float *out) {
    return guarded([&] {
        sc_check(h);
        REQUIRE(users && out && n > 0, "bad arguments");
        for (int64_t b = 0; b < n; ++b)
            REQUIRE(users[b] >= 0 && users[b] < h->n_users, "user %d out of range", users[b]);
        const int64_t cap = rows_per_batch(h);
        h->scores.ensure((size_t)(std::min(cap, n) * h->n_items));
        h->d_users.ensure((size_t)std::min(cap, n));
        for (int64_t b0 = 0; b0 < n; b0 += cap) {
            const int64_t nb = std::min(cap, n - b0);
            h->d_users.upload(users + b0, (size_t)nb, h->stream);
            launch_scores(h, h->d_users.p, 0, nb, true);
            h->scores.download(out + b0 * h->n_items, (size_t)(nb * h->n_items), h->stream);
            HIP_CHECK(hipStreamSynchronize(h->stream));
        }
    });
}

int cornac_hip_rank_topk(cornac_hip_scorer_t h, const int32_t *users, int64_t n, int topk, const int64_t *excl_indptr,
                         const int32_t *excl_indices, int32_t *items_out, float *scores_out) {
    return guarded([&] {
        sc_check(h);
        REQUIRE(users && items_out && scores_out && n > 0, "bad arguments");
        REQUIRE(topk >= 1 && topk <= h->n_items, "topk must be in [1, n_items]");
        for (int64_t b = 0; b < n; ++b)
            REQUIRE(users[b] >= 0 && users[b] < h->n_users, "user %d out of range", users[b]);
        const bool have_excl = excl_indptr != nullptr && excl_indices != nullptr;
        if (have_excl) {
            validate_csr(excl_indptr, excl_indices, n, h->n_items, "excl");
            h->d_excl_indptr.ensure((size_t)n + 1);
            h->d_excl_indptr.upload(excl_indptr, (size_t)n + 1, h->stream);
            const int64_t ne = excl_indptr[n];
            h->d_excl_indices.ensure((size_t)std::max<int64_t>(ne, 1));
            if (ne > 0) h->d_excl_indices.upload(excl_indices, (size_t)ne, h->stream);
        }
        if (can_fuse(h, topk)) {
            if (have_excl && (h->n_items + 31) / 32 > kMaxBitmapTiles)
                for (int64_t b = 0; b < n; ++b)
                    for (int64_t p = excl_indptr[b] + 1; p < excl_indptr[b + 1]; ++p)
                        REQUIRE(excl_indices[p] > excl_indices[p - 1], "exclusion row %lld is not strictly sorted",
                                (long long)b);
            h->d_users.ensure((size_t)n);
            h->d_items_out.ensure((size_t)(n * topk));
            h->d_scores_out.ensure((size_t)(n * topk));
            h->d_users.upload(users, (size_t)n, h->stream);
            launch_rank_fused(h, h->d_users.p, 0, n, topk, have_excl ? h->d_excl_indptr.p : nullptr,
                              have_excl ? h->d_excl_indices.p : nullptr, 0, h->d_items_out.p, h->d_scores_out.p);
            h->d_items_out.download(items_out, (size_t)(n * topk), h->stream);
            h->d_scores_out.download(scores_out, (size_t)(n * topk), h->stream);
            HIP_CHECK(hipStreamSynchronize(h->stream));
            return;
        }
        int64_t cap = rows_per_batch(h);
        if (topk > TOPK_MAX) cap = std::min<int64_t>(cap, 1024);
        const int64_t nb_max = std::min(cap, n);
        h->scores.ensure((size_t)(nb_max * h->n_items));
        h->d_users.ensure((size_t)nb_max);
        h->d_items_out.ensure((size_t)(nb_max * topk));
        h->d_scores_out.ensure((size_t)(nb_max * topk));
        if (have_excl) h->excl.ensure((size_t)(nb_max * h->n_items));
        for (int64_t b0 = 0; b0 < n; b0 += cap) {
            const int64_t nb = std::min(cap, n - b0);
            h->d_users.upload(users + b0, (size_t)nb, h->stream);
            launch_scores(h, h->d_users.p, 0, nb, true);
            if (have_excl) {
                HIP_CHECK(hipMemsetAsync(h->excl.p, 0, (size_t)(nb * h->n_items), h->stream));
                hipLaunchKernelGGL(mark_excluded_kernel, dim3((unsigned)nb), dim3(kBlk), 0, h->stream,
                                   h->d_excl_indptr.p, h->d_excl_indices.p, b0, h->n_items, h->excl.p);
            }
            launch_rank(h, nb, topk, have_excl, h->d_items_out.p, h->d_scores_out.p);
            h->d_items_out.download(items_out + b0 * topk, (size_t)(nb * topk), h->stream);
            h->d_scores_out.download(scores_out + b0 * topk, (size_t)(nb * topk), h->stream);
            HIP_CHECK(hipStreamSynchronize(h->stream));
        }
    });
}

int cornac_hip_rank_positions(cornac_hip_scorer_t h, const int32_t *users, int64_t n, const int64_t *excl_indptr,
                              const int32_t *excl_indices, const int64_t *tgt_indptr, const int32_t *tgt_indices,
                              int32_t *greater_out, int32_t *pos_out, int32_t *ge_out, float *tgt_scores_out) {
    return guarded([&] {
        sc_check(h);
        REQUIRE(users && tgt_indptr && n > 0, "bad arguments");
        REQUIRE(tgt_indptr[0] == 0, "tgt_indptr must start at 0");
        for (int64_t b = 0; b < n; ++b) {
            REQUIRE(users[b] >= 0 && users[b] < h->n_users, "user %d out of range", users[b]);
            REQUIRE(tgt_indptr[b + 1] >= tgt_indptr[b], "tgt_indptr must not decrease");
        }
        const int64_t nt = tgt_indptr[n];
        if (nt == 0) return;
        REQUIRE(tgt_indices && greater_out && pos_out && ge_out && tgt_scores_out, "bad arguments");
        const bool have_excl = excl_indptr != nullptr && excl_indices != nullptr;
        if (have_excl) {
            validate_csr(excl_indptr, excl_indices, n, h->n_items, "excl");
            h->d_excl_indptr.ensure((size_t)n + 1);
            h->d_excl_indptr.upload(excl_indptr, (size_t)n + 1, h->stream);
            const int64_t ne = excl_indptr[n];
            h->d_excl_indices.ensure((size_t)std::max<int64_t>(ne, 1));
            if (ne > 0) h->d_excl_indices.upload(excl_indices, (size_t)ne, h->stream);
        }
        h->d_tgt_indptr.ensure((size_t)n + 1);
        h->d_tgt_indptr.upload(tgt_indptr, (size_t)n + 1, h->stream);
        h->d_tgt_indices.ensure((size_t)nt);
        h->d_tgt_indices.upload(tgt_indices, (size_t)nt, h->stream);
        h->d_tgt_counts.ensure((size_t)(3 * nt));
        h->d_tgt_scores.ensure((size_t)nt);
        const int64_t cap = rows_per_batch(h);
        const int64_t nb_max = std::min(cap, n);
        h->scores.ensure((size_t)(nb_max * h->n_items));
        h->d_users.ensure((size_t)nb_max);
        if (have_excl) h->excl.ensure((size_t)(nb_max * h->n_items));
        for (int64_t b0 = 0; b0 < n; b0 += cap) {
            const int64_t nb = std::min(cap, n - b0);
            h->d_users.upload(users + b0, (size_t)nb, h->stream);
            launch_scores(h, h->d_users.p, 0, nb, true);
            if (have_excl) {
                HIP_CHECK(hipMemsetAsync(h->excl.p, 0, (size_t)(nb * h->n_items), h->stream));
                hipLaunchKernelGGL(mark_excluded_kernel, dim3((unsigned)nb), dim3(kBlk), 0, h->stream,
                                   h->d_excl_indptr.p, h->d_excl_indices.p, b0, h->n_items, h->excl.p);
            }
            hipLaunchKernelGGL(rank_positions_kernel, dim3((unsigned)nb), dim3(kBlk), 0, h->stream, h->scores.p,
                               have_excl ? h->excl.p : nullptr, h->n_items, h->d_tgt_indptr.p, h->d_tgt_indices.p, b0,
                               h->d_tgt_counts.p, h->d_tgt_counts.p + nt, h->d_tgt_counts.p + 2 * nt,
                               h->d_tgt_scores.p);
            HIP_CHECK(hipGetLastError());
            HIP_CHECK(hipStreamSynchronize(h->stream));
        }
        HIP_CHECK(hipMemcpyAsync(greater_out, h->d_tgt_counts.p, (size_t)nt * 4, hipMemcpyDeviceToHost, h->stream));
        HIP_CHECK(hipMemcpyAsync(pos_out, h->d_tgt_counts.p + nt, (size_t)nt * 4, hipMemcpyDeviceToHost, h->stream));
        HIP_CHECK(hipMemcpyAsync(ge_out, h->d_tgt_counts.p + 2 * nt, (size_t)nt * 4, hipMemcpyDeviceToHost, h->stream));
        h->d_tgt_scores.download(tgt_scores_out, (size_t)nt, h->stream);
        HIP_CHECK(hipStreamSynchronize(h->stream));
    });
}

int cornac_hip_score_pairs(cornac_hip_scorer_t h, const int32_t *users, const int32_t *items, int64_t n, int clip,
                           float lo, float hi, float *out) {
    return guarded([&] {
        sc_check(h);
        REQUIRE(users && items && out && n > 0, "bad arguments");
        for (int64_t p = 0; p < n; ++p)
            REQUIRE(users[p] >= 0 && users[p] < h->n_users && items[p] >= 0 && items[p] < h->n_items,
                    "pair %lld is out of range", (long long)p);
        DevBuf<int32_t> du, di;
        DevBuf<float> dout;
        du.alloc((size_t)n);
        di.alloc((size_t)n);
        dout.alloc((size_t)n);
        du.upload(users, (size_t)n, h->stream);
        di.upload(items, (size_t)n, h->stream);
        hipLaunchKernelGGL(score_pairs_kernel, dim3((unsigned)((n + kBlk - 1) / kBlk)), dim3(kBlk), 0, h->stream,
                           h->U.p, h->V.p, h->item_base.p, h->has_user_base ? h->user_base.p : nullptr, du.p, di.p, n,
                           h->k, h->ld, clip, lo, hi, dout.p);
        HIP_CHECK(hipGetLastError());
        dout.download(out, (size_t)n, h->stream);
        HIP_CHECK(hipStreamSynchronize(h->stream));
    });
}

int cornac_hip_scorer_set_exclusions(cornac_hip_scorer_t h, const int64_t *indptr, const int32_t *indices) {
    return guarded([&] {
        sc_check(h, false);
        if (!indptr) {
            h->has_res_excl = false;
            return;
        }
        REQUIRE(indices != nullptr || indptr[h->n_users] == 0, "indices is NULL");
        validate_csr(indptr, indices, h->n_users, h->n_items, "excl");
        const int64_t ne = indptr[h->n_users];
        h->res_excl_indptr.ensure((size_t)h->n_users + 1);
        h->res_excl_indices.ensure((size_t)std::max<int64_t>(ne, 1));
        h->res_excl_indptr.upload(indptr, (size_t)h->n_users + 1, h->stream);
        if (ne > 0) h->res_excl_indices.upload(indices, (size_t)ne, h->stream);
        HIP_CHECK(hipStreamSynchronize(h->stream));
        h->has_res_excl = true;
    });
}

int cornac_hip_rank_topk_resident(cornac_hip_scorer_t h, const int32_t *users, int64_t u0, int64_t n, int topk,
                                  int32_t *items_out, float *scores_out, double *device_ms) {
    return guarded([&] {
        sc_check(h);
        REQUIRE(h->has_res_excl, "cornac_hip_scorer_set_exclusions has not been called");
        REQUIRE(n > 0 && topk >= 1 && topk <= h->n_items, "bad arguments");
        REQUIRE(can_fuse(h, topk) && (h->n_items + 31) / 32 <= kMaxBitmapTiles,
                "resident exclusion lists serve the fused top-k path (topk <= 32, k <= 128, <= 262144 items)");
        if (users) {
            for (int64_t b = 0; b < n; ++b) REQUIRE(users[b] >= 0 && users[b] < h->n_users, "user %d out of range", users[b]);
            h->d_users.ensure((size_t)n);
            h->d_users.upload(users, (size_t)n, h->stream);
        } else {
            REQUIRE(u0 >= 0 && u0 + n <= h->n_users, "user range out of bounds");
        }
        h->d_items_out.ensure((size_t)(n * topk));
        h->d_scores_out.ensure((size_t)(n * topk));
        hipEvent_t e0 = nullptr, e1 = nullptr;
        if (device_ms) {
            HIP_CHECK(hipEventCreate(&e0));
            HIP_CHECK(hipEventCreate(&e1));
            HIP_CHECK(hipEventRecord(e0, h->stream));
        }
        launch_rank_fused(h, users ? h->d_users.p : nullptr, u0, n, topk, h->res_excl_indptr.p, h->res_excl_indices.p, 0,
                          h->d_items_out.p, h->d_scores_out.p, true);
        if (device_ms) HIP_CHECK(hipEventRecord(e1, h->stream));
        if (items_out) h->d_items_out.download(items_out, (size_t)(n * topk), h->stream);
        if (scores_out) h->d_scores_out.download(scores_out, (size_t)(n * topk), h->stream);
        HIP_CHECK(hipStreamSynchronize(h->stream));
        if (device_ms) {
            float t = 0.f;
            HIP_CHECK(hipEventElapsedTime(&t, e0, e1));
            (void)hipEventDestroy(e0);
            (void)hipEventDestroy(e1);
            *device_ms = (double)t;
        }
    });
}

int cornac_hip_scorer_host_buffer(cornac_hip_scorer_t h, size_t bytes, void **out) {
    return guarded([&] {
        sc_check(h);
        REQUIRE(out != nullptr, "out is NULL");
        if (bytes > h->pinned_bytes) {
            if (h->pinned_out) h->pinned_retired.push_back(h->pinned_out);
            h->pinned_out = nullptr;
            const size_t want = std::max(bytes, 2 * h->pinned_bytes);
            h->pinned_bytes = 0;
            HIP_CHECK(hipHostMalloc(&h->pinned_out, want, hipHostMallocDefault));
            h->pinned_bytes = want;
        }
        *out = h->pinned_out;
    });
}

int cornac_hip_rank_topk_device(cornac_hip_scorer_t h, int64_t u0, int64_t n, int topk, int repeats, double *ms) {
    return guarded([&] {
        sc_check(h);
        REQUIRE(u0 >= 0 && n > 0 && u0 + n <= h->n_users, "user range out of bounds");
        REQUIRE(topk >= 1 && topk <= h->n_items, "topk out of range");
        REQUIRE(repeats >= 1 && ms, "bad arguments");
        const bool fused = can_fuse(h, topk);
        const int64_t cap = fused ? n : rows_per_batch(h);
        const int64_t nb_max = std::min(cap, n);
        if (!fused) h->scores.ensure((size_t)(nb_max * h->n_items));
        if (!fused && topk > TOPK_MAX) {
            int64_t pad = 1;
            while (pad < h->n_items) pad <<= 1;
            h->sort_scratch.ensure((size_t)(nb_max * pad));
        }
        h->d_items_out.ensure((size_t)(nb_max * topk));
        h->d_scores_out.ensure((size_t)(nb_max * topk));
        hipEvent_t e0, e1;
        HIP_CHECK(hipEventCreate(&e0));
        HIP_CHECK(hipEventCreate(&e1));
        HIP_CHECK(hipEventRecord(e0, h->stream));
        for (int r = 0; r < repeats; ++r) {
            for (int64_t b0 = 0; b0 < n; b0 += cap) {
                const int64_t nb = std::min(cap, n - b0);
                if (fused) {
                    launch_rank_fused(h, nullptr, u0 + b0, nb, topk, nullptr, nullptr, 0, h->d_items_out.p,
                                      h->d_scores_out.p);
                } else {
                    launch_scores(h, nullptr, u0 + b0, nb, true);
                    launch_rank(h, nb, topk, false, h->d_items_out.p, h->d_scores_out.p);
                }
            }
        }
        HIP_CHECK(hipEventRecord(e1, h->stream));
        HIP_CHECK(hipEventSynchronize(e1));
        float t = 0.f;
        HIP_CHECK(hipEventElapsedTime(&t, e0, e1));
        (void)hipEventDestroy(e0);
        (void)hipEventDestroy(e1);
        *ms = (double)t;
    });
}
}
```

include/cornac_hip.h:

```cpp
#ifndef CORNAC_HIP_H_
#define CORNAC_HIP_H_

#include <stdint.h>

#ifdef __cplusplus
extern "C" {
#endif

#define CORNAC_HIP_OK 0
#define CORNAC_HIP_ERR_INVALID 1
#define CORNAC_HIP_ERR_HIP 2
#define CORNAC_HIP_ERR_NO_DEVICE 3
#define CORNAC_HIP_ERR_UNSUPPORTED 4

#define CORNAC_HIP_MODE_DETERMINISTIC 0
#define CORNAC_HIP_MODE_HOGWILD 1

#define CORNAC_HIP_NEG_UNIFORM 0
#define CORNAC_HIP_NEG_POPULARITY 1

const char *cornac_hip_last_error(void);
const char *cornac_hip_version(void);
int cornac_hip_device_count(int *count);
int cornac_hip_device_info(int device, char *name, int name_len, int *compute_units, int64_t *hbm_bytes);
int cornac_hip_device_probe(int device, int64_t bytes, double *out3);

typedef struct cornac_hip_bpr *cornac_hip_bpr_t;

int cornac_hip_bpr_create(cornac_hip_bpr_t *out, int device, int64_t n_users, int64_t n_items,
                          int64_t total_users, int64_t total_items, int k, const int32_t *indptr,
                          const int32_t *indices, int64_t nnz);
int cornac_hip_bpr_destroy(cornac_hip_bpr_t h);

int cornac_hip_bpr_set_factors(cornac_hip_bpr_t h, const float *U, const float *V, const float *B);
int cornac_hip_bpr_get_factors(cornac_hip_bpr_t h, float *U, float *V, float *B);

int cornac_hip_bpr_set_factors_f64(cornac_hip_bpr_t h, const double *U, const double *V, const double *B);
int cornac_hip_bpr_get_factors_f64(cornac_hip_bpr_t h, double *U, double *V, double *B);
int cornac_hip_bpr_fit_epochs_f64(cornac_hip_bpr_t h, int n_epochs, double lr, double reg, int use_bias, int neg_population,
                                  int64_t *correct, int64_t *skipped);

int cornac_hip_bpr_bind_device(cornac_hip_bpr_t h, float *dU, float *dV, float *dB);
int cornac_hip_bpr_device_ptrs(cornac_hip_bpr_t h, float **dU, float **dV, float **dB);
int cornac_hip_bpr_rebind_items(cornac_hip_bpr_t h, float *dV, float *dB);
int cornac_hip_bpr_set_stream(cornac_hip_bpr_t h, void *hip_stream);
int cornac_hip_bpr_switch_stream(cornac_hip_bpr_t h, void *hip_stream);

int cornac_hip_bpr_seed_mt19937(cornac_hip_bpr_t h, uint32_t mt_seed_pos, uint32_t mt_seed_neg, int shared_stream);
int cornac_hip_bpr_seed_hogwild(cornac_hip_bpr_t h, uint64_t seed);

int cornac_hip_bpr_set_negative_population(cornac_hip_bpr_t h, const int32_t *items, int64_t n);

#define CORNAC_HIP_HOG_PLAIN_STORES 1
#define CORNAC_HIP_HOG_VEC4_LAYOUT 2
#define CORNAC_HIP_HOG_NO_OWNERSHIP 4
#define CORNAC_HIP_HOG_DENSE_BIAS 8
#define CORNAC_HIP_HOG_SHARE_NEG 16
#define CORNAC_HIP_HOG_BINNED 64
#define CORNAC_HIP_HOG_FUSED_OPT_OUT 128
#define CORNAC_HIP_HOG_ABLATE_MASK 0xff00
#define CORNAC_HIP_HOG_ABLATE_SHIFT 8
#define CORNAC_HIP_HOG_FORM_MASK 0xf0000
#define CORNAC_HIP_HOG_FORM_SHIFT 16
#define CORNAC_HIP_FORM_AUTO (0 << CORNAC_HIP_HOG_FORM_SHIFT)
#define CORNAC_HIP_FORM_FUSED (1 << CORNAC_HIP_HOG_FORM_SHIFT)
#define CORNAC_HIP_FORM_STRATA (2 << CORNAC_HIP_HOG_FORM_SHIFT)
#define CORNAC_HIP_FORM_LDSBIN (3 << CORNAC_HIP_HOG_FORM_SHIFT)

int cornac_hip_bpr_fit_epochs(cornac_hip_bpr_t h, int n_epochs, float lr, float reg, int use_bias, int neg_population,
                              int mode, int hogwild_flags, int64_t *correct, int64_t *skipped);
int cornac_hip_bpr_hogwild_enqueue(cornac_hip_bpr_t h, int64_t n_samples, float lr, float reg, int use_bias,
                                   int neg_population, int hogwild_flags);
int cornac_hip_bpr_sync(cornac_hip_bpr_t h, int64_t *correct, int64_t *skipped);

int cornac_hip_bpr_debug_draw(cornac_hip_bpr_t h, int stream, uint64_t hi, int64_t n, int64_t *out);
int cornac_hip_bpr_debug_ownership(cornac_hip_bpr_t h, int64_t *n_waves, int64_t *wave_ptr, int32_t *own_u,
                                   int32_t *own_i);
int cornac_hip_bpr_strata_config(cornac_hip_bpr_t h, int hot_permille, int hot_min_mult_x100, int rehash_period);
int cornac_hip_bpr_chunk_records(cornac_hip_bpr_t h, int enable);
int cornac_hip_bpr_strata_stats(cornac_hip_bpr_t h, int64_t *out4);
int cornac_hip_bpr_debug_strata(cornac_hip_bpr_t h, uint32_t epoch, int64_t *sptr, int32_t *rec_u, int32_t *rec_i,
                                int32_t *rank_item, uint32_t *key);
int cornac_hip_bpr_ldsbin_config(cornac_hip_bpr_t h, int hot_x1000, int min_candidates, int max_rounds);
int cornac_hip_bpr_ldsbin_pass_config(cornac_hip_bpr_t h, int enable, int waves, int lds_kb, int min_draws_x100);
int cornac_hip_bpr_ldsbin_stats(cornac_hip_bpr_t h, int64_t *out8);
int cornac_hip_bpr_ldsbin_deal_config(cornac_hip_bpr_t h, int strata_groups, int hot_cost_x16);
int cornac_hip_bpr_debug_ldsbin_deal(cornac_hip_bpr_t h, uint64_t seed, uint32_t epoch, int32_t *bin_of_item,
                                     uint32_t *cold_mass, uint32_t *hot_off, int32_t *hot_u, int32_t *hot_i);
int cornac_hip_bpr_kernel_timing(cornac_hip_bpr_t h, int enable, double *total_ms, int64_t *launches);
int cornac_hip_bpr_last_timing(cornac_hip_bpr_t h, double *ms4);

int cornac_hip_bpr_sample_triplets(cornac_hip_bpr_t h, int64_t n_draws, int neg_population, int32_t *d_u,
                                   int32_t *d_i, int32_t *d_j);
int cornac_hip_bpr_apply_triplets(cornac_hip_bpr_t h, const int32_t *d_u, const int32_t *d_slot_i,
                                  const int32_t *d_slot_j, int64_t n, float *d_rows, float *d_bias, int bias_stride,
                                  float lr, float reg, int use_bias);
int cornac_hip_bpr_staged_slots(cornac_hip_bpr_t h, int64_t n_draws, int64_t *n_slots);
int cornac_hip_bpr_emit_triplets(cornac_hip_bpr_t h, int64_t n_draws, int neg_population, int32_t *d_u, int32_t *d_i,
                                 int32_t *d_j, int64_t slots_cap, int64_t *n_slots);
int cornac_hip_bpr_apply_staged(cornac_hip_bpr_t h, const int32_t *d_u, const int32_t *d_slot_i, const int32_t *d_slot_j,
                                int64_t n_slots, float *d_rows, float *d_bias, int bias_stride, float lr, float reg,
                                int use_bias);
int cornac_hip_bpr_shard_mark(cornac_hip_bpr_t h, const int32_t *d_i, const int32_t *d_j, int64_t n, int world,
                              int64_t rows_per_rank, int32_t *d_mark);
int cornac_hip_bpr_shard_slots(cornac_hip_bpr_t h, const int32_t *d_i, const int32_t *d_j, int64_t n, int world,
                               int64_t rows_per_rank, const int32_t *d_scan, int32_t *d_slot_i, int32_t *d_slot_j);
int cornac_hip_bpr_shard_uniq(cornac_hip_bpr_t h, const int32_t *d_mark, const int32_t *d_scan, int64_t n_rows,
                              int64_t rows_per_rank, int32_t *d_uniq_local);
int cornac_hip_bpr_scatter_diff_rows(cornac_hip_bpr_t h, float *d_table, const int32_t *d_ids, int64_t n, int width,
                                     const float *d_now, const float *d_before, const float *d_scale);
int cornac_hip_bpr_gather_rows(cornac_hip_bpr_t h, const float *d_table, const int32_t *d_ids, int64_t n, int width,
                               float *d_out);
int cornac_hip_bpr_scatter_add_rows(cornac_hip_bpr_t h, float *d_table, const int32_t *d_ids, int64_t n, int width,
                                    const float *d_delta);
int cornac_hip_bpr_table_delta_begin(cornac_hip_bpr_t h, const float *d_flat, const float *d_base, int64_t n_items,
                                     int k, float *d_bucket, float *d_local);
int cornac_hip_bpr_table_delta_finish(cornac_hip_bpr_t h, float *d_flat, float *d_base, const float *d_bucket,
                                      const float *d_local, int64_t n_items, int k);
int cornac_hip_bpr_table_delta_step(cornac_hip_bpr_t h, float *d_flat, float *d_base, const float *d_bucket_prev,
                                    const float *d_local_prev, int64_t n_items, int k, float *d_bucket, float *d_local);
int cornac_hip_bpr_table_delta(cornac_hip_bpr_t h, int op, int rule, float *d_flat, float *d_base, const float *d_bucket_prev,
                               const float *d_local_prev, int64_t n_items, int k, float *d_bucket, float *d_local);
int cornac_hip_table_delta(int op, int device, void *hip_stream, float *d_flat, float *d_base, const float *d_bucket_prev,
                           const float *d_local_prev, int64_t n_items, int k, float *d_bucket, float *d_local);
int cornac_hip_bpr_resident_exchange_bins(cornac_hip_bpr_t h, int neg_population, int hogwild_flags, int *n_bins);
int cornac_hip_bpr_epoch_resident_enqueue(cornac_hip_bpr_t h, float lr, float reg, int use_bias, int neg_population,
                                          int hogwild_flags, int n_exchanges, int rule, float *d_base, float *d_buckets,
                                          int64_t bucket_stride, float *d_keeps, int64_t keep_stride, uint32_t *d_arrive,
                                          const uint32_t *d_landed, uint32_t *d_applied, int *n_arrivals);
int cornac_hip_bpr_resident_flush(cornac_hip_bpr_t h, int n_exchanges, int rule, float *d_base, const float *d_buckets,
                                  int64_t bucket_stride, const float *d_keeps, int64_t keep_stride,
                                  const uint32_t *d_applied, const uint32_t *d_landed);
int cornac_hip_bpr_conveyor_setup(cornac_hip_bpr_t h, int n_blocks, const int32_t *rank_item, uint64_t deal_seed,
                                  int release_item_tables, int *n_bins, int *bins_per_block, int *cap);
int cornac_hip_bpr_conveyor_layout(cornac_hip_bpr_t h, uint32_t layout_epoch, int32_t *d_slot_item, int32_t *d_item_slot);
int cornac_hip_bpr_conveyor_enqueue(cornac_hip_bpr_t h, uint32_t epoch, uint32_t layout_epoch, int n_ranges,
                                    const int32_t *first_block, float *const *d_rows, float lr, float reg, int use_bias,
                                    int neg_population, int hogwild_flags);
int cornac_hip_stream_wait_counter(int device, void *hip_stream, const uint32_t *d_counter, uint32_t target,
                                   uint32_t *d_error, int timeout_ms);
int cornac_hip_stream_set_flag(int device, void *hip_stream, uint32_t *d_flag, uint32_t value, const uint32_t *d_unless);
int cornac_hip_stream_ring_standin(int device, void *hip_stream, const float *d_src, int64_t src_floats, float *d_dst,
                                   int64_t dst_floats, int64_t n_floats, int n_workgroups);

int cornac_hip_bpr_set_views(cornac_hip_bpr_t h, const int32_t *view_indptr, const int32_t *view_indices,
                             int64_t nnz_view);
int cornac_hip_bpr_seed_view_stream(cornac_hip_bpr_t h, uint32_t mt_seed_view);
int cornac_hip_vebpr_fit_epochs(cornac_hip_bpr_t h, int n_epochs, float lr, float reg, float alpha, int mode,
                                int64_t *correct, int64_t *skipped);
int cornac_hip_vebpr_fit_epochs_f64(cornac_hip_bpr_t h, int n_epochs, double lr, double reg, double alpha, int64_t *correct,
                                    int64_t *skipped);
#define CORNAC_HIP_VEBPR_NO_OWNERSHIP 0x100
int cornac_hip_vebpr_hogwild_form(cornac_hip_bpr_t h, int *owned);

int cornac_hip_mmmf_fit_epochs(cornac_hip_bpr_t h, int n_epochs, float lr, float reg, int mode, int64_t *correct,
                               int64_t *skipped);
int cornac_hip_mmmf_fit_epochs_f64(cornac_hip_bpr_t h, int n_epochs, double lr, double reg, int64_t *correct,
                                   int64_t *skipped);
int cornac_hip_mmmf_hogwild_enqueue(cornac_hip_bpr_t h, int64_t n_samples, float lr, float reg);

typedef struct cornac_hip_mf *cornac_hip_mf_t;

int cornac_hip_mf_create(cornac_hip_mf_t *out, int device, int64_t n_users, int64_t n_items, int k,
                         const int64_t *rid, const int64_t *cid, const float *val, int64_t nnz);
int cornac_hip_mf_destroy(cornac_hip_mf_t h);
int cornac_hip_mf_set_factors(cornac_hip_mf_t h, const float *U, const float *V, const float *Bu, const float *Bi);
int cornac_hip_mf_get_factors(cornac_hip_mf_t h, float *U, float *V, float *Bu, float *Bi);
int cornac_hip_mf_fit(cornac_hip_mf_t h, int max_iter, float lr, float reg, float mu, int use_bias, int early_stop,
                      int mode, float *loss_per_epoch, int *epochs_run);
int cornac_hip_mf_hogwild_form(cornac_hip_mf_t h, int form);
int cornac_hip_mf_hogwild_stats(cornac_hip_mf_t h, int64_t *out4);
int cornac_hip_mf_debug_split(cornac_hip_mf_t h, int64_t *n_split, int64_t *n_virtual, int32_t *split_item, int32_t *split_ptr);
int cornac_hip_mf_debug_ownership(cornac_hip_mf_t h, int64_t *n_waves, int64_t *wave_ptr, int32_t *own_u, int32_t *own_i);
int cornac_hip_mf_fit_sgd(int device, const int64_t *rid, const int64_t *cid, const float *val, int64_t nnz, float *U,
                          float *V, float *Bu, float *Bi, int64_t n_users, int64_t n_items, int k, float lr, float reg,
                          float mu, int max_iter, int use_bias, int early_stop, int mode, float *loss_per_epoch,
                          int *epochs_run);
int cornac_hip_mf_bind_items(cornac_hip_mf_t h, float *dV, float *dBi);
int cornac_hip_mf_bind_users(cornac_hip_mf_t h, float *dU, float *dBu);
int cornac_hip_mf_set_stream(cornac_hip_mf_t h, void *hip_stream);
int cornac_hip_mf_epoch_enqueue(cornac_hip_mf_t h, int part, int n_parts, float lr, float reg, float mu, int use_bias);
int cornac_hip_mf_sync(cornac_hip_mf_t h, double *sq_err_sum);
int cornac_hip_mf_kernel_timing(cornac_hip_mf_t h, int enable, double *total_ms, int64_t *launches);
int cornac_hip_mf_last_timing(cornac_hip_mf_t h, double *ms4);

#define CORNAC_HIP_PMF_LINEAR 0
#define CORNAC_HIP_PMF_NON_LINEAR 1
int cornac_hip_mf_pmf_set_factors(cornac_hip_mf_t h, const double *U, const double *V);
int cornac_hip_mf_pmf_get_factors(cornac_hip_mf_t h, double *U, double *V);
int cornac_hip_mf_pmf_fit(cornac_hip_mf_t h, int n_epochs, float lr, float reg, float gamma, int variant, double *loss_per_epoch);
int cornac_hip_mf_pmf_form(cornac_hip_mf_t h, int *form, int *group);

int cornac_hip_mf_nmf_set_factors(cornac_hip_mf_t h, const float *U, const float *V, const float *Bu, const float *Bi);
int cornac_hip_mf_nmf_get_factors(cornac_hip_mf_t h, float *U, float *V, float *Bu, float *Bi);
int cornac_hip_mf_nmf_fit(cornac_hip_mf_t h, int n_epochs, float lr, float lambda_u, float lambda_v, float lambda_bu,
                          float lambda_bi, float mu, int use_bias, int mode, double *loss_per_epoch);
int cornac_hip_mf_nmf_form(cornac_hip_mf_t h, int *sum_form, int *bias_form, int *rows_split);

int cornac_hip_mf_hpf_set_tables(cornac_hip_mf_t h, const double *G_s, const double *G_r, const double *L_s, const double *L_r);
int cornac_hip_mf_hpf_get_tables(cornac_hip_mf_t h, double *G_s, double *G_r, double *L_s, double *L_r, double *K_r, double *T_r);
int cornac_hip_mf_hpf_fit(cornac_hip_mf_t h, int n_iters, int hierarchical);
int cornac_hip_mf_hpf_elog(cornac_hip_mf_t h, double *Lt, double *Lb);
int cornac_hip_mf_hpf_form(cornac_hip_mf_t h, int *group, int *rows_split);

#define CORNAC_HIP_OPT_SGD 0
#define CORNAC_HIP_OPT_ADAM 1
#define CORNAC_HIP_OPT_RMSPROP 2
#define CORNAC_HIP_OPT_ADAGRAD 3
int cornac_hip_mf_fit_minibatch(cornac_hip_mf_t h, const int64_t *order, int64_t n_total, int batch_size,
                                int optimizer, float lr, float reg, float mu, int use_bias, double *loss_sum);
int cornac_hip_mf_fit_minibatch_dropout(cornac_hip_mf_t h, const int64_t *order, int64_t n_total, int batch_size,
                                        int optimizer, float lr, float reg, float mu, int use_bias, const uint8_t *keep_u,
                                        const uint8_t *keep_i, float keep_scale, double *loss_sum);
int cornac_hip_mf_reset_optimizer(cornac_hip_mf_t h);

typedef struct cornac_hip_vbpr *cornac_hip_vbpr_t;

int cornac_hip_vbpr_create(cornac_hip_vbpr_t *out, int device, int64_t n_users, int64_t n_items, int k, int k2,
                           int n_feat, const float *features);
int cornac_hip_vbpr_destroy(cornac_hip_vbpr_t h);
int cornac_hip_vbpr_set_params(cornac_hip_vbpr_t h, const float *Bi, const float *Gu, const float *Gi, const float *Tu,
                               const float *E, const float *Bp);
int cornac_hip_vbpr_get_params(cornac_hip_vbpr_t h, float *Bi, float *Gu, float *Gi, float *Tu, float *E, float *Bp);
int cornac_hip_vbpr_fit_batches(cornac_hip_vbpr_t h, const int32_t *u, const int32_t *i, const int32_t *j,
                                int64_t n_total, int batch_size, float lr, float lambda_w, float lambda_b,
                                float lambda_e, double *sum_nll);
int cornac_hip_vbpr_item_tables(cornac_hip_vbpr_t h, float *theta_item, float *visual_bias);

typedef struct cornac_hip_wmf *cornac_hip_wmf_t;

int cornac_hip_wmf_create(cornac_hip_wmf_t *out, int device, int64_t n_users, int64_t n_items, int k,
                          const int64_t *csc_indptr, const int32_t *csc_rows, const float *csc_vals, int64_t nnz);
void cornac_hip_wmf_destroy(cornac_hip_wmf_t h);
int cornac_hip_wmf_set_factors(cornac_hip_wmf_t h, const float *U, const float *V);
int cornac_hip_wmf_get_factors(cornac_hip_wmf_t h, float *U, float *V);
int cornac_hip_wmf_fit_batches(cornac_hip_wmf_t h, const int32_t *item_ids, const int64_t *batch_ptr,
                               int64_t n_batches, float lambda_u, float lambda_v, float a, float b,
                               float learning_rate, double *loss_out);
int cornac_hip_wmf_kernel_timing(cornac_hip_wmf_t h, int enabled);
int cornac_hip_wmf_last_timing(cornac_hip_wmf_t h, double *device_ms);

typedef struct cornac_hip_scorer *cornac_hip_scorer_t;

int cornac_hip_scorer_set_exclusions(cornac_hip_scorer_t h, const int64_t *indptr, const int32_t *indices);
int cornac_hip_scorer_host_buffer(cornac_hip_scorer_t h, size_t bytes, void **out);
int cornac_hip_rank_topk_resident(cornac_hip_scorer_t h, const int32_t *users, int64_t u0, int64_t n, int topk,
                                  int32_t *items_out, float *scores_out, double *device_ms);

int cornac_hip_scorer_create(cornac_hip_scorer_t *out, int device, int64_t n_users, int64_t n_items, int k);
int cornac_hip_scorer_destroy(cornac_hip_scorer_t h);
int cornac_hip_scorer_set(cornac_hip_scorer_t h, const float *U, const float *V, const float *item_base,
                          const float *user_base);
int cornac_hip_score_user(cornac_hip_scorer_t h, int64_t user, float *out);
int cornac_hip_scorer_set_f64(cornac_hip_scorer_t h, const double *U, const double *V, const double *item_base,
                              const double *user_base);
int cornac_hip_score_user_f64(cornac_hip_scorer_t h, int64_t user, double *out);
int cornac_hip_score_block(cornac_hip_scorer_t h, const int32_t *users, int64_t n, float *out);
int cornac_hip_score_pairs(cornac_hip_scorer_t h, const int32_t *users, const int32_t *items, int64_t n, int clip,
                           float lo, float hi, float *out);
int cornac_hip_rank_topk(cornac_hip_scorer_t h, const int32_t *users, int64_t n, int topk, const int64_t *excl_indptr,
                         const int32_t *excl_indices, int32_t *items_out, float *scores_out);
int cornac_hip_rank_positions(cornac_hip_scorer_t h, const int32_t *users, int64_t n, const int64_t *excl_indptr,
                              const int32_t *excl_indices, const int64_t *tgt_indptr, const int32_t *tgt_indices,
                              int32_t *greater_out, int32_t *pos_out, int32_t *ge_out, float *tgt_scores_out);
int cornac_hip_rank_topk_device(cornac_hip_scorer_t h, int64_t u0, int64_t n, int topk, int repeats, double *ms);

typedef struct cornac_hip_knn_sim *cornac_hip_knn_sim_t;
typedef struct cornac_hip_knn_scorer *cornac_hip_knn_scorer_t;
#define CORNAC_HIP_KNN_MAX_K 64

int cornac_hip_knn_sim_create(cornac_hip_knn_sim_t *out, int device, int64_t n_rows, int64_t n_cols, const int64_t *indptr,
                              const int32_t *indices, const double *data);
int cornac_hip_knn_sim_destroy(cornac_hip_knn_sim_t h);
int cornac_hip_knn_sim_run(cornac_hip_knn_sim_t h, int64_t rows_per_pass);
int cornac_hip_knn_sim_nnz(cornac_hip_knn_sim_t h, int64_t *nnz);
int cornac_hip_knn_sim_get(cornac_hip_knn_sim_t h, int64_t *indptr, int32_t *indices, double *data);

int cornac_hip_knn_scorer_create(cornac_hip_knn_scorer_t *out, int device, int64_t n_items, int64_t n_neighbours,
                                 int64_t n_users, const int64_t *n_indptr, const int32_t *n_indices, const double *n_data,
                                 const int64_t *q_indptr, const int32_t *q_indices, const double *q_data, int user_mode);
int cornac_hip_knn_scorer_destroy(cornac_hip_knn_scorer_t h);
int cornac_hip_knn_scorer_score_users(cornac_hip_knn_scorer_t h, const int32_t *users, int64_t n, int k, double *out);
int cornac_hip_knn_scorer_score_pairs(cornac_hip_knn_scorer_t h, const int32_t *users, const int32_t *items, int64_t n, int k,
                                      double *out);

typedef struct cornac_hip_ease *cornac_hip_ease_t;

int cornac_hip_ease_create(cornac_hip_ease_t *out, int device, int64_t n_users, int64_t n_items, const int64_t *indptr,
                           const int32_t *indices, const double *data);
int cornac_hip_ease_destroy(cornac_hip_ease_t h);
int cornac_hip_ease_gram(cornac_hip_ease_t h);
int cornac_hip_ease_invert(cornac_hip_ease_t h, double lamb);
int cornac_hip_ease_weights(cornac_hip_ease_t h, int pos_b);
int cornac_hip_ease_fit(cornac_hip_ease_t h, double lamb, int pos_b);
int cornac_hip_ease_get_table(cornac_hip_ease_t h, double *table);
int cornac_hip_ease_set_table(cornac_hip_ease_t h, const double *table);
int cornac_hip_ease_score_users(cornac_hip_ease_t h, const int32_t *users, int64_t n, double *out);
int cornac_hip_ease_score_pairs(cornac_hip_ease_t h, const int32_t *users, const int32_t *items, int64_t n, double *out);

typedef struct cornac_hip_vaecf *cornac_hip_vaecf_t;

int cornac_hip_vaecf_create(cornac_hip_vaecf_t *out, int device, int64_t n_users, int64_t n_items, const int64_t *indptr,
                            const int32_t *indices, int k, int h, int act, int likelihood);
int cornac_hip_vaecf_destroy(cornac_hip_vaecf_t h);
int cornac_hip_vaecf_set_params(cornac_hip_vaecf_t h, const float *const *tables);
int cornac_hip_vaecf_get_params(cornac_hip_vaecf_t h, float *const *tables);
int cornac_hip_vaecf_get_state(cornac_hip_vaecf_t h, float *const *m, float *const *v, int64_t *t);
int cornac_hip_vaecf_reset_optimizer(cornac_hip_vaecf_t h);
int cornac_hip_vaecf_fit_epoch(cornac_hip_vaecf_t h, int64_t batch_size, float lr, float beta, const float *eps, uint64_t seed,
                               double *loss_sum, double *step_loss);
int cornac_hip_vaecf_encode_users(cornac_hip_vaecf_t h, const int32_t *users, int64_t n, float *h2_out);
int cornac_hip_vaecf_score_users(cornac_hip_vaecf_t h, const int32_t *users, int64_t n, float *out);
int cornac_hip_vaecf_score_pairs(cornac_hip_vaecf_t h, const int32_t *users, const int32_t *items, int64_t n, float *out);

#ifdef __cplusplus
}
#endif
#endif
```

Baseline: 3.416 billion.

## Add bf16 MFMA candidate filter with fp32 rescore for top-k ranking

Result: slower. 3.356 billion (-1.8%).

```diff
diff --git a/cornac_amd/_lib.py b/cornac_amd/_lib.py
--- a/cornac_amd/_lib.py
+++ b/cornac_amd/_lib.py
@@ -59,7 +59,7 @@
     "cornac_hip_scorer_create", "cornac_hip_scorer_destroy", "cornac_hip_scorer_set", "cornac_hip_score_user",
     "cornac_hip_scorer_set_f64", "cornac_hip_score_user_f64",
     "cornac_hip_score_block", "cornac_hip_rank_topk", "cornac_hip_rank_topk_device", "cornac_hip_score_pairs",
-    "cornac_hip_scorer_set_exclusions", "cornac_hip_rank_topk_resident", "cornac_hip_scorer_host_buffer",
+    "cornac_hip_scorer_set_exclusions", "cornac_hip_rank_topk_resident", "cornac_hip_scorer_host_buffer", "cornac_hip_scorer_rank_filter",
     "cornac_hip_rank_positions",
     "cornac_hip_knn_sim_create", "cornac_hip_knn_sim_destroy", "cornac_hip_knn_sim_run", "cornac_hip_knn_sim_nnz",
     "cornac_hip_knn_sim_get",
@@ -279,6 +279,7 @@
         L.cornac_hip_rank_topk_device.argtypes = [_vp, C.c_int64, C.c_int64, C.c_int, C.c_int, C.POINTER(C.c_double)]
         L.cornac_hip_scorer_set_exclusions.argtypes = [_vp, _vp, _vp]
         L.cornac_hip_scorer_host_buffer.argtypes = [_vp, C.c_size_t, C.POINTER(_vp)]
+        L.cornac_hip_scorer_rank_filter.argtypes = [_vp, C.c_int, _vp]
         L.cornac_hip_rank_topk_resident.argtypes = [_vp, _vp, C.c_int64, C.c_int64, C.c_int, _vp, _vp, _vp]
         L.cornac_hip_knn_sim_create.argtypes = [C.POINTER(_vp), C.c_int, C.c_int64, C.c_int64, _vp, _vp, _vp]
         L.cornac_hip_knn_sim_destroy.argtypes = [_vp]
@@ -1014,6 +1015,11 @@
                                                   C.cast(C.byref(ms), _vp) if timed else None))
         return (items, scores, ms.value) if timed else (items, scores)
 
+    def rank_filter(self, mode=-1):
+        st = np.zeros(4, np.int64)
+        check(lib().cornac_hip_scorer_rank_filter(self.h, int(mode), st.ctypes.data))
+        return {"rows_filtered": int(st[0]), "rows_fallback": int(st[1]), "candidates": int(st[2]), "valid": bool(st[3])}
+
     def rank_topk_device_ms(self, u0, n, topk, repeats=1):
         ms = C.c_double()
         check(lib().cornac_hip_rank_topk_device(self.h, u0, n, topk, repeats, C.byref(ms)))
diff --git a/cornac_amd/csrc/rank_filter.inc b/cornac_amd/csrc/rank_filter.inc
--- /dev/null
+++ b/cornac_amd/csrc/rank_filter.inc
@@ -0,0 +1,454 @@
+typedef __bf16 bf16x8 __attribute__((ext_vector_type(8)));
+typedef uint32_t u32x4 __attribute__((ext_vector_type(4)));
+
+constexpr int kFiltCap = 64;
+constexpr uint32_t kFiltPosBits = 18;
+constexpr uint32_t kFiltOvf = 0x80000000u;
+
+__device__ __forceinline__ uint32_t filt_pack(float eps, uint32_t pos) {
+    return (((__float_as_uint(eps) + 0x1ffffu) >> 17) << kFiltPosBits) | pos;
+}
+__device__ __forceinline__ float filt_eps(uint32_t lo) { return __uint_as_float((lo >> kFiltPosBits) << 17); }
+
+template <int KB, int NT>
+__global__ __launch_bounds__(kBlk, 1) void rank_filter_kernel(
+    const uint16_t *__restrict__ Uf, const uint16_t *__restrict__ Vf, const float *__restrict__ ucu,
+    const float *__restrict__ ueta, const float *__restrict__ vnv, const float *__restrict__ vdl,
+    const int32_t *__restrict__ users, int64_t u0, int64_t n_rows, int64_t n_items, int64_t work_per_wg, int topk,
+    const uint32_t *__restrict__ excl_bits, float *tau_pub, uint32_t *__restrict__ cand,
+    uint32_t *__restrict__ ccount) {
+    constexpr int LDF = 16 * KB;
+    constexpr int ROWB = LDF * 2 + 16;
+    constexpr int GI = 32 * NT;
+    constexpr int CPR = LDF / 8;
+    constexpr int CHUNKS = GI * CPR;
+    constexpr int STG = (CHUNKS + kBlk - 1) / kBlk;
+    constexpr int CAP = kFiltCap;
+    static_assert(NT % 2 == 0 && GI <= 128, "two accumulators ping-pong across groups; 128 meta lanes");
+    __shared__ __attribute__((aligned(16))) unsigned char btile[2][GI * ROWB];
+    __shared__ unsigned long long keys[kBlk / 64][32][CAP];
+    __shared__ uint32_t meta[3][NT * 192 + 1];
+    __shared__ int cnt[kBlk / 64][32];
+    __shared__ float tau[kBlk / 64][32];
+    __shared__ uint32_t lkey[kBlk / 64][64];
+    __shared__ uint32_t ovf[kBlk / 64];
+    __shared__ float cu_s[kBlk / 64][32], eta_s[kBlk / 64][32];
+    const int wave = threadIdx.x >> 6, lane = threadIdx.x & 63;
+    const int col = lane & 31, half = lane >> 5;
+    const int64_t n_item_tiles = (n_items + 31) / 32;
+    const int64_t n_row_blocks = (n_rows + 127) / 128;
+    const int64_t work_total = n_row_blocks * n_item_tiles;
+    const int64_t pos = (int64_t)blockIdx.x * work_per_wg;
+    const int64_t work_end = min(work_total, pos + work_per_wg);
+
+    u32x4 stg[STG];
+    uint32_t soff[STG];
+#pragma unroll
+    for (int q = 0; q < STG; ++q) {
+        const int idx = threadIdx.x + q * kBlk;
+        soff[q] = idx < CHUNKS ? (uint32_t)((idx / CPR) * ROWB + (idx % CPR) * 16) : 0u;
+    }
+    constexpr int MW = NT * 192 + 1;
+    uint32_t stg_w[NT], maddr[NT];
+    const uint32_t *pm[NT];
+    int64_t pstride = 0;
+    {
+        const uint32_t meta_base = lds_offset(&meta[0][0]);
+#pragma unroll
+        for (int j = 0; j < NT; ++j) {
+            maddr[j] = meta_base + (uint32_t)(NT * 192) * 4u;
+            pm[j] = reinterpret_cast<const uint32_t *>(vnv);
+            stg_w[j] = 0u;
+        }
+        if (threadIdx.x < 128) {
+            if (excl_bits) {
+#pragma unroll
+                for (int j = 0; j < NT; ++j) maddr[j] = meta_base + (uint32_t)(j * 192 + threadIdx.x) * 4u;
+            }
+        } else if ((int)threadIdx.x - 128 < GI) {
+            const int i = threadIdx.x - 128;
+            maddr[0] = meta_base + (uint32_t)((i >> 5) * 192 + 128 + (i & 31)) * 4u;
+            maddr[1] = meta_base + (uint32_t)((i >> 5) * 192 + 160 + (i & 31)) * 4u;
+        }
+    }
+    int64_t cur_rb = 0;
+    int seg_t0 = 0;
+    const char *vb = reinterpret_cast<const char *>(Vf);
+    auto stage_seek = [&]() {
+        vb = reinterpret_cast<const char *>(Vf) + (int64_t)seg_t0 * (32 * LDF * 2) + (int64_t)threadIdx.x * 16;
+#pragma unroll
+        for (int j = 0; j < NT; ++j) pm[j] = reinterpret_cast<const uint32_t *>(vnv);
+        pstride = 0;
+        if (threadIdx.x < 128) {
+            if (excl_bits) {
+#pragma unroll
+                for (int j = 0; j < NT; ++j) pm[j] = excl_bits + (cur_rb * 128 + threadIdx.x) * n_item_tiles + seg_t0 + j;
+                pstride = NT;
+            }
+        } else if ((int)threadIdx.x - 128 < GI) {
+            const int i = threadIdx.x - 128;
+#pragma unroll
+            for (int j = 0; j < NT; ++j) pm[j] = reinterpret_cast<const uint32_t *>(vnv) + (int64_t)seg_t0 * 32 + i;
+            pm[1] = reinterpret_cast<const uint32_t *>(vdl) + (int64_t)seg_t0 * 32 + i;
+            pstride = GI;
+        }
+    };
+    auto stage_load = [&]() {
+#pragma unroll
+        for (int j = 0; j < NT; ++j) {
+            stg_w[j] = *pm[j];
+            pm[j] += pstride;
+        }
+#pragma unroll
+        for (int q = 0; q < STG; ++q) {
+            const int idx = threadIdx.x + q * kBlk;
+            if ((q + 1) * kBlk <= CHUNKS || idx < CHUNKS) stg[q] = *reinterpret_cast<const u32x4 *>(vb + (int64_t)q * (kBlk * 16));
+        }
+        vb += GI * LDF * 2;
+    };
+    auto stage_store = [&](int buf, int ms) {
+#pragma unroll
+        for (int j = 0; j < NT; ++j)
+            *reinterpret_cast<__attribute__((address_space(3))) uint32_t *>(maddr[j] + (uint32_t)ms * (uint32_t)(MW * 4)) = stg_w[j];
+#pragma unroll
+        for (int q = 0; q < STG; ++q) {
+            const int idx = threadIdx.x + q * kBlk;
+            if ((q + 1) * kBlk <= CHUNKS || idx < CHUNKS) *reinterpret_cast<u32x4 *>(&btile[buf][soff[q]]) = stg[q];
+        }
+    };
+    const uint32_t frag_off = (uint32_t)(col * ROWB + half * 16);
+    const float qnan = __uint_as_float(0x7fc00000u);
+    const f32x16 zero16 = {0.f, 0.f, 0.f, 0.f, 0.f, 0.f, 0.f, 0.f, 0.f, 0.f, 0.f, 0.f, 0.f, 0.f, 0.f, 0.f};
+    const f32x16 nan16 = {qnan, qnan, qnan, qnan, qnan, qnan, qnan, qnan, qnan, qnan, qnan, qnan, qnan, qnan, qnan, qnan};
+
+    int64_t pos_hi = work_end;
+    while (pos_hi > pos) {
+        const int64_t rb = (pos_hi - 1) / n_item_tiles;
+        cur_rb = rb;
+        const int64_t seg_lo = max(pos, rb * n_item_tiles);
+        const int t_begin = (int)(seg_lo - rb * n_item_tiles);
+        const int t_end = (int)(pos_hi - rb * n_item_tiles);
+        const int64_t seg = (int64_t)blockIdx.x - (rb * n_item_tiles) / work_per_wg;
+        pos_hi = seg_lo;
+        seg_t0 = t_begin;
+        const int64_t row_tile = rb * (kBlk / 64) + wave;
+        if (lane < 32) {
+            cnt[wave][lane] = 0;
+            const int64_t row = row_tile * 32 + lane;
+            float t0 = -INFINITY;
+            if (row >= n_rows) t0 = INFINITY;
+            else if (t_begin > 0) t0 = __hip_atomic_load(tau_pub + row, __ATOMIC_RELAXED, __HIP_MEMORY_SCOPE_AGENT);
+            tau[wave][lane] = t0;
+            const int64_t u = row < n_rows ? (users ? (int64_t)users[row] : u0 + row) : 0;
+            cu_s[wave][lane] = ucu[u];
+            eta_s[wave][lane] = ueta[u];
+        }
+        if (lane == 0) ovf[wave] = 0u;
+        bf16x8 a[KB];
+        {
+            const int64_t r = row_tile * 32 + col;
+            const int64_t u = r < n_rows ? (users ? (int64_t)users[r] : u0 + r) : 0;
+            const uint16_t *p = Uf + u * LDF + 8 * half;
+#pragma unroll
+            for (int kb = 0; kb < KB; ++kb) a[kb] = *reinterpret_cast<const bf16x8 *>(p + 16 * kb);
+        }
+        float thr[16];
+        int cnt_r[16];
+        __builtin_amdgcn_fence(__ATOMIC_ACQ_REL, "wavefront");
+        __builtin_amdgcn_wave_barrier();
+#pragma unroll
+        for (int r = 0; r < 16; ++r) {
+            thr[r] = tau[wave][(r & 3) + 8 * (r >> 2) + 4 * half];
+            cnt_r[r] = 0;
+        }
+
+        auto compact = [&](unsigned need) __attribute__((always_inline)) {
+            if (col == 0) {
+#pragma unroll
+                for (int r = 0; r < 16; ++r) cnt[wave][(r & 3) + 8 * (r >> 2) + 4 * half] = cnt_r[r];
+            }
+            __builtin_amdgcn_fence(__ATOMIC_ACQ_REL, "wavefront");
+            __builtin_amdgcn_wave_barrier();
+            while (need) {
+                const int rl = __builtin_ctz(need);
+                need &= need - 1u;
+                const int c = cnt[wave][rl];
+                unsigned long long *krow = keys[wave][rl];
+                const bool live = lane < c;
+                const unsigned long long mine = live ? krow[lane] : 0ull;
+                const float up = key_to_float((uint32_t)(mine >> 32));
+                const float lo_f = up - 2.f * filt_eps((uint32_t)mine);
+                const uint32_t lk = live ? order_key(lo_f) : 0u;
+                lkey[wave][lane] = lk;
+                __builtin_amdgcn_fence(__ATOMIC_ACQ_REL, "wavefront");
+                __builtin_amdgcn_wave_barrier();
+                int rank = 0;
+                for (int j0 = 0; j0 < c; j0 += 8) {
+                    uint32_t lj[8];
+#pragma unroll
+                    for (int q = 0; q < 8; ++q) lj[q] = lkey[wave][min(j0 + q, 63)];
+#pragma unroll
+                    for (int q = 0; q < 8; ++q)
+                        rank += (j0 + q < c && (lj[q] > lk || (lj[q] == lk && j0 + q < lane))) ? 1 : 0;
+                }
+                float tnew = tau[wave][rl];
+                const unsigned long long kth_mask = __ballot(live && rank == topk - 1);
+                if (kth_mask != 0ull) {
+                    const int src = __builtin_ctzll(kth_mask);
+                    tnew = fmaxf(tnew, __uint_as_float((uint32_t)__builtin_amdgcn_readlane((int)__float_as_uint(lo_f), src)));
+                }
+                const bool keep = live && up >= tnew;
+                const unsigned long long bal = __ballot(keep);
+                const int slot = __popcll(bal & ((1ull << lane) - 1ull));
+                if (keep) krow[slot] = mine;
+                if (lane == 0) {
+                    tau[wave][rl] = tnew;
+                    cnt[wave][rl] = __popcll(bal);
+                }
+                __builtin_amdgcn_fence(__ATOMIC_ACQ_REL, "wavefront");
+                __builtin_amdgcn_wave_barrier();
+            }
+#pragma unroll
+            for (int r = 0; r < 16; ++r) {
+                const int rl = (r & 3) + 8 * (r >> 2) + 4 * half;
+                thr[r] = tau[wave][rl];
+                cnt_r[r] = cnt[wave][rl];
+            }
+        };
+        auto take = [&](int r, unsigned long long m, float accv, uint32_t wv, float nv, float dl, uint32_t ipos, bool last_try,
+                        unsigned &redo, unsigned &over_rows) __attribute__((always_inline)) {
+            const int rl0 = (r & 3) + 8 * (r >> 2);
+            if (excl_bits)
+                m &= ~((unsigned long long)(uint32_t)__builtin_amdgcn_readlane(wv, rl0) |
+                       ((unsigned long long)(uint32_t)__builtin_amdgcn_readlane(wv, rl0 + 4) << 32));
+            if (m == 0ull) return;
+            const unsigned mine = half ? (unsigned)(m >> 32) : (unsigned)m;
+            const int np = __popc(mine);
+            const bool over = cnt_r[r] + np > CAP;
+            const unsigned long long ob = __ballot(over);
+            if (ob != 0ull && !last_try) {
+                redo |= 1u << r;
+                over_rows |= ((uint32_t)ob != 0u ? 1u << rl0 : 0u) | ((uint32_t)(ob >> 32) != 0u ? 1u << (rl0 + 4) : 0u);
+                return;
+            }
+            const int rl = rl0 + 4 * half;
+            if (over) {
+                thr[r] = INFINITY;
+                if (col == 0) {
+                    tau[wave][rl] = INFINITY;
+                    atomicOr(&ovf[wave], 1u << rl);
+                }
+            } else {
+                if ((mine >> col) & 1u) {
+                    const float eps = fmaf(cu_s[wave][rl], nv, dl + eta_s[wave][rl]) * 1.001f;
+                    const int slot = cnt_r[r] + __popc(mine & ((1u << col) - 1u));
+                    keys[wave][rl][slot] =
+                        ((unsigned long long)order_key(accv) << 32) | (unsigned long long)filt_pack(eps, ipos);
+                }
+                cnt_r[r] += np;
+            }
+        };
+        auto tile_step = [&](auto chain, f32x16 &acc_n, const bf16x8 (&bfr)[KB], const f32x16 &acc_p, int it_p, int ms_p, int j_p)
+                             __attribute__((always_inline)) {
+            constexpr bool CHAIN = decltype(chain)::value;
+            const bool ok_p = it_p < t_end;
+            const uint32_t *mt = &meta[ms_p][j_p * 192];
+            const uint32_t wv = mt[wave * 32 + col];
+            const float nv = __uint_as_float(mt[128 + col]), dl = __uint_as_float(mt[160 + col]);
+            const uint32_t ipos = (uint32_t)(it_p * 32 + col);
+            unsigned redo = 0u, over_rows = 0u;
+#pragma unroll
+            for (int kb = 0; kb < KB; ++kb) {
+                if (CHAIN) acc_n = __builtin_amdgcn_mfma_f32_32x32x16_bf16(a[kb], bfr[kb], kb == 0 ? zero16 : acc_n, 0, 0, 0);
+                const int r0 = (16 * kb) / KB, r1 = (16 * (kb + 1)) / KB;
+                unsigned long long gm[8];
+                unsigned long long any = 0ull;
+#pragma unroll
+                for (int r = r0; r < r1; ++r) {
+                    gm[r - r0] = __ballot(acc_p[r] >= thr[r]);
+                    any |= gm[r - r0];
+                }
+                if (any != 0ull && ok_p) {
+#pragma unroll
+                    for (int r = r0; r < r1; ++r)
+                        if (gm[r - r0] != 0ull) take(r, gm[r - r0], acc_p[r], wv, nv, dl, ipos, false, redo, over_rows);
+                }
+            }
+            if (redo != 0u) {
+                compact(over_rows);
+#pragma unroll
+                for (int r = 0; r < 16; ++r) {
+                    if ((redo >> r) & 1u) {
+                        const unsigned long long m = __ballot(acc_p[r] >= thr[r]);
+                        if (m != 0ull) take(r, m, acc_p[r], wv, nv, dl, ipos, true, redo, over_rows);
+                    }
+                }
+            }
+        };
+
+        const int n_groups = (t_end - t_begin + NT - 1) / NT;
+        f32x16 acc0 = nan16, acc1 = nan16;
+        bf16x8 bfA[KB], bfB[KB];
+        stage_seek();
+        stage_load();
+        stage_store(0, 0);
+        __syncthreads();
+        if (n_groups > 1) stage_load();
+        int ms = 0;
+        for (int g = 0; g < n_groups; ++g) {
+            const int buf = g & 1;
+            const int ms_prev = ms == 0 ? 2 : ms - 1, ms_next = ms == 2 ? 0 : ms + 1;
+            const unsigned char *bt = btile[buf] + frag_off;
+            const int it0 = t_begin + g * NT;
+#pragma unroll
+            for (int kb = 0; kb < KB; ++kb) bfA[kb] = *reinterpret_cast<const bf16x8 *>(bt + 32 * kb);
+#pragma nounroll
+            for (int jj = 0; jj < NT; jj += 2) {
+#pragma unroll
+                for (int kb = 0; kb < KB; ++kb)
+                    bfB[kb] = *reinterpret_cast<const bf16x8 *>(bt + (jj + 1) * 32 * ROWB + 32 * kb);
+                __builtin_amdgcn_sched_barrier(0);
+                tile_step(std::true_type{}, acc0, bfA, acc1, it0 + jj - 1, jj == 0 ? ms_prev : ms, jj == 0 ? NT - 1 : jj - 1);
+                if (jj + 2 < NT) {
+#pragma unroll
+                    for (int kb = 0; kb < KB; ++kb)
+                        bfA[kb] = *reinterpret_cast<const bf16x8 *>(bt + (jj + 2) * 32 * ROWB + 32 * kb);
+                }
+                __builtin_amdgcn_sched_barrier(0);
+                tile_step(std::true_type{}, acc1, bfB, acc0, it0 + jj, ms, jj);
+            }
+            if (g + 1 < n_groups) stage_store(buf ^ 1, ms_next);
+            if (g + 2 < n_groups) stage_load();
+            __syncthreads();
+            ms = ms_next;
+        }
+        tile_step(std::false_type{}, acc0, bfA, acc1, t_begin + n_groups * NT - 1, ms == 0 ? 2 : ms - 1, NT - 1);
+        compact(0xffffffffu);
+        const uint32_t ovf_w = ovf[wave];
+        for (int rl = 0; rl < 32; ++rl) {
+            const int64_t row = row_tile * 32 + rl;
+            if (row >= n_rows) break;
+            const int c = cnt[wave][rl];
+            if (lane < c) cand[(seg * n_rows + row) * CAP + lane] = (uint32_t)keys[wave][rl][lane] & ((1u << kFiltPosBits) - 1u);
+            if (lane == 0) ccount[seg * n_rows + row] = (uint32_t)c | (((ovf_w >> rl) & 1u) ? kFiltOvf : 0u);
+        }
+        if (t_begin == 0 && t_end < n_item_tiles && lane < 32 && row_tile * 32 + lane < n_rows)
+            __hip_atomic_store(tau_pub + row_tile * 32 + lane, tau[wave][lane], __ATOMIC_RELAXED, __HIP_MEMORY_SCOPE_AGENT);
+        __builtin_amdgcn_fence(__ATOMIC_ACQ_REL, "wavefront");
+        __builtin_amdgcn_wave_barrier();
+        __syncthreads();
+    }
+}
+
+constexpr int kRescoreMax = 512;
+constexpr int kRescoreCounterSlots = 128, kRescoreCounterStride = 16;
+__global__ __launch_bounds__(kBlk) void rank_rescore_kernel(const uint32_t *__restrict__ cand,
+                                                           const uint32_t *__restrict__ ccount, int n_segs, int64_t n_rows,
+                                                           int topk, const float *__restrict__ U, const float *__restrict__ V,
+                                                           const float *__restrict__ item_base,
+                                                           const float *__restrict__ user_base,
+                                                           const int32_t *__restrict__ users, int64_t u0, int k, int ld,
+                                                           const int32_t *__restrict__ perm, int32_t *__restrict__ items_out,
+                                                           float *__restrict__ scores_out, int32_t *__restrict__ fb_rows,
+                                                           unsigned long long *__restrict__ counters) {
+    __shared__ uint32_t plist_all[kBlk / 64][kRescoreMax];
+    __shared__ unsigned long long klist_all[kBlk / 64][kRescoreMax];
+    __shared__ float urow_all[kBlk / 64][128];
+    const int wave = threadIdx.x >> 6, lane = threadIdx.x & 63;
+    const int64_t row = (int64_t)blockIdx.x * (kBlk / 64) + wave;
+    if (row >= n_rows) return;
+    uint32_t *plist = plist_all[wave];
+    unsigned long long *klist = klist_all[wave];
+    float *urow = urow_all[wave];
+    const int64_t u = users ? (int64_t)users[row] : u0 + row;
+    for (int f = lane; f < k; f += 64) urow[f] = U[u * ld + f];
+    int total = 0;
+    bool fallback = false;
+    for (int s0 = 0; s0 < n_segs && !fallback; s0 += 64) {
+        const int s = s0 + lane;
+        const uint32_t w = s < n_segs ? ccount[(int64_t)s * n_rows + row] : 0u;
+        const int c = (int)(w & ~kFiltOvf);
+        int incl = c;
+#pragma unroll
+        for (int d = 1; d < 64; d <<= 1) {
+            const int t = __shfl_up(incl, d);
+            if (lane >= d) incl += t;
+        }
+        const int chunk = __shfl(incl, 63);
+        fallback = __ballot((w & kFiltOvf) != 0u) != 0ull || total + chunk > kRescoreMax;
+        if (!fallback) {
+            const int base = total + incl - c;
+            const int ns = min(64, n_segs - s0);
+            for (int q = 0; q < ns; ++q) {
+                const int cq = __shfl(c, q), bq = __shfl(base, q);
+                if (lane < cq) plist[bq + lane] = cand[((int64_t)(s0 + q) * n_rows + row) * kFiltCap + lane];
+            }
+        }
+        total += chunk;
+    }
+    if (fallback) {
+        if (lane == 0) fb_rows[atomicAdd(&counters[0], 1ull)] = (int32_t)row;
+        return;
+    }
+    __builtin_amdgcn_fence(__ATOMIC_ACQ_REL, "wavefront");
+    __builtin_amdgcn_wave_barrier();
+    const float ub = user_base ? user_base[u] : 0.f;
+    for (int i = lane; i < total; i += 64) {
+        const int32_t item = perm[plist[i]];
+        const v4f32 *vr = reinterpret_cast<const v4f32 *>(V + (int64_t)item * ld);
+        float acc = 0.f;
+        for (int f0 = 0; f0 < k; f0 += 32) {
+            v4f32 v[8];
+#pragma unroll
+            for (int q = 0; q < 8; ++q)
+                if (f0 + 4 * q < ld) v[q] = vr[f0 / 4 + q];
+#pragma unroll
+            for (int q = 0; q < 8; ++q)
+#pragma unroll
+                for (int e = 0; e < 4; ++e)
+                    if (f0 + 4 * q + e < k) acc = fmaf(urow[f0 + 4 * q + e], v[q][e], acc);
+        }
+        const float s = user_base ? (item_base[item] + ub) + acc : item_base[item] + acc;
+        klist[i] = ((unsigned long long)order_key(s) << 32) | (unsigned long long)(uint32_t)item;
+    }
+    __builtin_amdgcn_fence(__ATOMIC_ACQ_REL, "wavefront");
+    __builtin_amdgcn_wave_barrier();
+    for (int i = lane; i < total; i += 64) {
+        const unsigned long long mine = klist[i];
+        int rank = 0;
+        for (int j = 0; j < total; ++j) rank += klist[j] > mine ? 1 : 0;
+        if (rank < topk) {
+            items_out[row * topk + rank] = (int32_t)(uint32_t)mine;
+            if (scores_out) scores_out[row * topk + rank] = key_to_float((uint32_t)(mine >> 32));
+        }
+    }
+    for (int i = total + lane; i < topk; i += 64) {
+        items_out[row * topk + i] = -1;
+        if (scores_out) scores_out[row * topk + i] = -INFINITY;
+    }
+    if (lane == 0) atomicAdd(&counters[kRescoreCounterStride * (1 + (int)(row & (kRescoreCounterSlots - 1)))], (unsigned long long)total);
+}
+
+__global__ __launch_bounds__(kBlk) void filter_fallback_keys_kernel(const int32_t *__restrict__ fb_rows, int64_t n_fb,
+                                                                    const int32_t *__restrict__ users, int64_t u0,
+                                                                    int64_t excl_row0, int excl_by_user,
+                                                                    int32_t *__restrict__ fb_users,
+                                                                    int32_t *__restrict__ fb_keys) {
+    const int64_t i = (int64_t)blockIdx.x * kBlk + threadIdx.x;
+    if (i >= n_fb) return;
+    const int64_t row = fb_rows[i];
+    const int32_t u = users ? users[row] : (int32_t)(u0 + row);
+    fb_users[i] = u;
+    fb_keys[i] = excl_by_user ? u : (int32_t)(excl_row0 + row);
+}
+__global__ __launch_bounds__(kBlk) void filter_fallback_scatter_kernel(const int32_t *__restrict__ fb_rows, int64_t n_fb,
+                                                                       int topk, const int32_t *__restrict__ fb_items,
+                                                                       const float *__restrict__ fb_scores,
+                                                                       int32_t *__restrict__ items_out,
+                                                                       float *__restrict__ scores_out) {
+    const int64_t i = (int64_t)blockIdx.x * kBlk + threadIdx.x;
+    if (i >= n_fb * topk) return;
+    const int64_t row = fb_rows[i / topk];
+    items_out[row * topk + i % topk] = fb_items[i];
+    if (scores_out) scores_out[row * topk + i % topk] = fb_scores[i];
+}
diff --git a/cornac_amd/csrc/score.hip b/cornac_amd/csrc/score.hip
--- a/cornac_amd/csrc/score.hip
+++ b/cornac_amd/csrc/score.hip
@@ -1,6 +1,8 @@
 #include <algorithm>
 #include <cmath>
 #include <cstdlib>
+#include <cstring>
+#include <type_traits>
 
 #include "common.h"
 
@@ -545,6 +547,8 @@
     }
 }
 
+#include "rank_filter.inc"
+
 __global__ __launch_bounds__(kBlk) void mark_excluded_kernel(const int64_t *__restrict__ excl_indptr,
                                                              const int32_t *__restrict__ excl_indices, int64_t row0,
                                                              int64_t n_items, uint8_t *__restrict__ excl_mask) {
@@ -849,6 +853,15 @@
     DevBuf<int32_t> res_excl_indices;
     bool has_res_excl = false;
     DevBuf<float> tau_pub;
+    DevBuf<uint16_t> Uf, Vf;
+    DevBuf<float> f_cu, f_eta, f_nv, f_dl;
+    DevBuf<uint32_t> f_cand, f_ccount;
+    DevBuf<int32_t> f_fb_rows, f_fb_users, f_fb_keys, f_fb_items;
+    DevBuf<float> f_fb_scores;
+    DevBuf<unsigned long long> f_counters;
+    bool filter_valid = false;
+    int filter_mode = 1;
+    int64_t filter_stats[3] = {0, 0, 0};
     bool has_user_base = false, is_set = false;
     DevBuf<float> scores;
     DevBuf<uint8_t> excl;
@@ -875,7 +888,106 @@
     }
 }
 
-static void build_rank_order(cornac_hip_scorer_t h, const float *U, const float *V, const float *item_base) {
+static inline float bf16_to_float(uint16_t b) {
+    const uint32_t w = (uint32_t)b << 16;
+    float f;
+    memcpy(&f, &w, 4);
+    return f;
+}
+static inline uint16_t bf16_rne(float x) {
+    uint32_t w;
+    memcpy(&w, &x, 4);
+    return (uint16_t)((w + 0x7fffu + ((w >> 16) & 1u)) >> 16);
+}
+static inline uint16_t bf16_up(double x) {
+    float f = (float)x;
+    if ((double)f < x) f = std::nextafter(f, INFINITY);
+    uint32_t w;
+    memcpy(&w, &f, 4);
+    uint16_t b = (uint16_t)(w >> 16);
+    if (((uint32_t)b << 16) < w) ++b;
+    return b;
+}
+constexpr int kFilterTilePad = 4;
+
+static bool filter_magnitude_ok(float x) {
+    if (!std::isfinite(x)) return false;
+    const float a = std::fabs(x);
+    return a == 0.f || (a >= std::ldexp(1.f, CORNAC_HIP_RANK_FILTER_MIN_EXP) && a <= std::ldexp(1.f, CORNAC_HIP_RANK_FILTER_MAX_EXP));
+}
+
+static void build_filter_tables(cornac_hip_scorer_t h, const float *U, const float *V, const float *item_base,
+                                const float *user_base, const std::vector<int32_t> &order) {
+    const int64_t ni = h->n_items, nu = h->n_users;
+    const int k = h->k;
+    h->filter_valid = false;
+    if (k > 128 || (ni + 31) / 32 > 8192) return;
+    bool ok = true;
+    for (int64_t i = 0; i < nu * k && ok; ++i) ok = filter_magnitude_ok(U[i]);
+    for (int64_t i = 0; i < ni * k && ok; ++i) ok = filter_magnitude_ok(V[i]);
+    for (int64_t i = 0; item_base && i < ni && ok; ++i) ok = filter_magnitude_ok(item_base[i]);
+    for (int64_t i = 0; user_base && i < nu && ok; ++i) ok = filter_magnitude_ok(user_base[i]);
+    if (!ok) return;
+    const int ldf = h->ld + 16, x = h->ld;
+    const int64_t ni_pad = ((ni + 31) / 32 + kFilterTilePad) * 32;
+    std::vector<uint16_t> vf((size_t)ni_pad * ldf, 0), uf((size_t)nu * ldf, 0);
+    std::vector<float> nv((size_t)ni_pad, 0.f), dl((size_t)ni_pad, 0.f), cu((size_t)nu), eta((size_t)nu);
+    const uint16_t one = bf16_rne(1.f);
+    for (int64_t p = 0; p < ni_pad; ++p) {
+        uint16_t *row = vf.data() + (size_t)p * ldf;
+        if (p >= ni) {
+            row[x] = 0x7fc0;
+            continue;
+        }
+        const float *vr = V + (int64_t)order[(size_t)p] * k;
+        double ss = 0;
+        for (int f = 0; f < k; ++f) {
+            row[f] = bf16_rne(vr[f]);
+            ss += (double)vr[f] * vr[f];
+        }
+        const float ib = item_base ? item_base[order[(size_t)p]] : 0.f;
+        const uint16_t hi = bf16_rne(ib);
+        const float r1 = ib - bf16_to_float(hi);
+        const uint16_t mid = bf16_rne(r1);
+        const float r2 = r1 - bf16_to_float(mid);
+        const uint16_t lo = bf16_rne(r2);
+        if ((double)bf16_to_float(hi) + (double)bf16_to_float(mid) + (double)bf16_to_float(lo) != (double)ib) return;
+        row[x] = hi; row[x + 1] = mid; row[x + 2] = lo;
+        row[x + 3] = bf16_up(std::sqrt(ss) * (1.0 + 1e-12));
+        row[x + 4] = bf16_up(std::fabs((double)ib) * CORNAC_HIP_RANK_FILTER_BASE_SLACK);
+        row[x + 5] = one;
+        nv[(size_t)p] = bf16_to_float(row[x + 3]);
+        dl[(size_t)p] = bf16_to_float(row[x + 4]);
+    }
+    for (int64_t u = 0; u < nu; ++u) {
+        uint16_t *row = uf.data() + (size_t)u * ldf;
+        const float *ur = U + u * k;
+        double ss = 0;
+        for (int f = 0; f < k; ++f) {
+            row[f] = bf16_rne(ur[f]);
+            ss += (double)ur[f] * ur[f];
+        }
+        row[x] = row[x + 1] = row[x + 2] = one;
+        row[x + 3] = bf16_up(std::sqrt(ss) * (1.0 + 1e-12) * CORNAC_HIP_RANK_FILTER_C);
+        row[x + 4] = one;
+        row[x + 5] = bf16_up(user_base ? std::fabs((double)user_base[u]) * CORNAC_HIP_RANK_FILTER_USER_BASE_SLACK : 0.0);
+        cu[(size_t)u] = bf16_to_float(row[x + 3]);
+        eta[(size_t)u] = bf16_to_float(row[x + 5]);
+    }
+    h->Vf.ensure(vf.size()); h->Uf.ensure(uf.size());
+    h->f_nv.ensure(nv.size()); h->f_dl.ensure(dl.size()); h->f_cu.ensure(cu.size()); h->f_eta.ensure(eta.size());
+    h->Vf.upload(vf.data(), vf.size(), h->stream);
+    h->Uf.upload(uf.data(), uf.size(), h->stream);
+    h->f_nv.upload(nv.data(), nv.size(), h->stream);
+    h->f_dl.upload(dl.data(), dl.size(), h->stream);
+    h->f_cu.upload(cu.data(), cu.size(), h->stream);
+    h->f_eta.upload(eta.data(), eta.size(), h->stream);
+    HIP_CHECK(hipStreamSynchronize(h->stream));
+    h->filter_valid = true;
+}
+
+static void build_rank_order(cornac_hip_scorer_t h, const float *U, const float *V, const float *item_base,
+                             const float *user_base) {
     const int64_t ni = h->n_items, nu = h->n_users;
     const int k = h->k;
     const int64_t sample = std::min<int64_t>(nu, 16384), stride = std::max<int64_t>(1, nu / sample);
@@ -943,6 +1055,7 @@
                        h->Vr.p, h->ibr.p);
     HIP_CHECK(hipGetLastError());
     HIP_CHECK(hipStreamSynchronize(h->stream));
+    build_filter_tables(h, U, V, item_base, user_base, order);
 }
 
 static void validate_csr(const int64_t *indptr, const int32_t *indices, int64_t n, int64_t n_items, const char *what) {
@@ -1021,9 +1134,10 @@
 
 constexpr int64_t kMaxBitmapTiles = 8192;
 
-static void launch_rank_fused_rows(cornac_hip_scorer_t h, const int32_t *d_users, int64_t u0, int64_t n, int topk,
-                                   const int64_t *d_excl_indptr, const int32_t *d_excl_indices, int64_t excl_row0,
-                                   int32_t *items_out, float *scores_out, bool excl_by_user) {
+static void launch_rank_fp32_rows(cornac_hip_scorer_t h, const int32_t *d_users, int64_t u0, int64_t n, int topk,
+                                  const int64_t *d_excl_indptr, const int32_t *d_excl_indices, int64_t excl_row0,
+                                  int32_t *items_out, float *scores_out, bool excl_by_user,
+                                  const int32_t *d_bitmap_keys = nullptr) {
     const float *ub = h->has_user_base ? h->user_base.p : nullptr;
     const DeviceInfo &di = device_info(h->device);
     const int ablate = prof_env_int("CORNAC_HIP_RANK_ABLATE", 0);
@@ -1043,10 +1157,12 @@
     const bool no_bitmap = prof_env_set("CORNAC_HIP_RANK_NO_BITMAP");
     if (d_excl_indptr && n_item_tiles <= kMaxBitmapTiles && !no_bitmap) {
         const int64_t rows_padded = wg_rows * 128;
-        h->excl_bits.ensure((size_t)(rows_padded * n_item_tiles));
+        h->excl_bits.ensure((size_t)(rows_padded * n_item_tiles + kFilterTilePad));
+        const bool by_key = excl_by_user || d_bitmap_keys;
         hipLaunchKernelGGL(excl_bitmap_kernel, dim3((unsigned)((rows_padded + kBitmapRows * (kBlk / 64) - 1) / (kBitmapRows * (kBlk / 64)))), dim3(kBlk), 0,
-                           h->stream, d_excl_indptr + (excl_by_user ? 0 : excl_row0), d_excl_indices, d_users, u0,
-                           excl_by_user ? 1 : 0, h->inv_perm.p, n, rows_padded, n_item_tiles, h->excl_bits.p);
+                           h->stream, d_excl_indptr + (by_key ? 0 : excl_row0), d_excl_indices,
+                           d_bitmap_keys ? d_bitmap_keys : d_users, u0, by_key ? 1 : 0, h->inv_perm.p, n, rows_padded,
+                           n_item_tiles, h->excl_bits.p);
         d_bits = h->excl_bits.p;
     } else if (d_excl_indptr) {
         REQUIRE(!excl_by_user, "resident exclusion lists need the bitmap path (catalogue too large)");
@@ -1088,12 +1204,99 @@
     HIP_CHECK(hipGetLastError());
 }
 
+constexpr int kFilterMaxTopk = 10;
+static bool can_filter(cornac_hip_scorer_t h, int topk) {
+    return h->filter_mode != 0 && h->filter_valid && topk <= kFilterMaxTopk && h->k <= 128 &&
+           (h->n_items + 31) / 32 <= kMaxBitmapTiles;
+}
+
+static void launch_rank_filter_rows(cornac_hip_scorer_t h, const int32_t *d_users, int64_t u0, int64_t n, int topk,
+                                    const int64_t *d_excl_indptr, const int32_t *d_excl_indices, int64_t excl_row0,
+                                    int32_t *items_out, float *scores_out, bool excl_by_user) {
+    const float *ub = h->has_user_base ? h->user_base.p : nullptr;
+    const DeviceInfo &di = device_info(h->device);
+    const int64_t n_item_tiles = (h->n_items + 31) / 32;
+    const int64_t wg_rows = (n + 127) / 128;
+    const int64_t work_total = wg_rows * n_item_tiles;
+    const int64_t work_per_wg = std::max<int64_t>((work_total + di.cus - 1) / di.cus, std::min<int64_t>(16, n_item_tiles));
+    const int64_t n_wgs = (work_total + work_per_wg - 1) / work_per_wg;
+    const int64_t max_segs = (n_item_tiles + work_per_wg - 1) / work_per_wg + 1;
+    h->f_cand.ensure((size_t)(max_segs * n * kFiltCap));
+    h->f_ccount.ensure((size_t)(max_segs * n));
+    HIP_CHECK(hipMemsetAsync(h->f_ccount.p, 0, (size_t)(max_segs * n) * sizeof(uint32_t), h->stream));
+    constexpr size_t n_counters = (size_t)kRescoreCounterStride * (1 + kRescoreCounterSlots);
+    h->f_counters.ensure(n_counters);
+    HIP_CHECK(hipMemsetAsync(h->f_counters.p, 0, n_counters * sizeof(unsigned long long), h->stream));
+    h->f_fb_rows.ensure((size_t)n);
+    h->tau_pub.ensure((size_t)n);
+    HIP_CHECK(hipMemsetD32Async((hipDeviceptr_t)h->tau_pub.p, 0xff800000u , (size_t)n, h->stream));
+    const uint32_t *d_bits = nullptr;
+    if (d_excl_indptr) {
+        const int64_t rows_padded = wg_rows * 128;
+        h->excl_bits.ensure((size_t)(rows_padded * n_item_tiles + kFilterTilePad));
+        hipLaunchKernelGGL(excl_bitmap_kernel, dim3((unsigned)((rows_padded + kBitmapRows * (kBlk / 64) - 1) / (kBitmapRows * (kBlk / 64)))), dim3(kBlk), 0,
+                           h->stream, d_excl_indptr + (excl_by_user ? 0 : excl_row0), d_excl_indices, d_users, u0,
+                           excl_by_user ? 1 : 0, h->inv_perm.p, n, rows_padded, n_item_tiles, h->excl_bits.p);
+        d_bits = h->excl_bits.p;
+    }
+    dim3 grid((unsigned)n_wgs), block(kBlk);
+#define FILTER(KB_, NT_)                                                                                                    \
+    hipLaunchKernelGGL((rank_filter_kernel<KB_, NT_>), grid, block, 0, h->stream, h->Uf.p, h->Vf.p, h->f_cu.p, h->f_eta.p, \
+                       h->f_nv.p, h->f_dl.p, d_users, u0, n, h->n_items, work_per_wg, topk, d_bits, h->tau_pub.p,          \
+                       h->f_cand.p, h->f_ccount.p)
+    if (h->ld == 16) FILTER(2, 4);
+    else if (h->ld == 32) FILTER(3, 4);
+    else if (h->ld == 64) FILTER(5, 4);
+    else FILTER(9, 2);
+#undef FILTER
+    HIP_CHECK(hipGetLastError());
+    hipLaunchKernelGGL(rank_rescore_kernel, dim3((unsigned)((n + kBlk / 64 - 1) / (kBlk / 64))), dim3(kBlk), 0, h->stream, h->f_cand.p, h->f_ccount.p,
+                       (int)max_segs, n, topk, h->U.p, h->V.p, h->item_base.p, ub, d_users, u0, h->k, h->ld, h->perm.p,
+                       items_out, scores_out, h->f_fb_rows.p, h->f_counters.p);
+    HIP_CHECK(hipGetLastError());
+    std::vector<unsigned long long> counters(n_counters, 0ull);
+    HIP_CHECK(hipMemcpyAsync(counters.data(), h->f_counters.p, n_counters * sizeof(unsigned long long), hipMemcpyDeviceToHost,
+                             h->stream));
+    HIP_CHECK(hipStreamSynchronize(h->stream));
+    const int64_t n_fb = (int64_t)counters[0];
+    int64_t n_cand = 0;
+    for (int sl = 0; sl < kRescoreCounterSlots; ++sl) n_cand += (int64_t)counters[(size_t)kRescoreCounterStride * (1 + sl)];
+    h->filter_stats[0] += n - n_fb;
+    h->filter_stats[1] += n_fb;
+    h->filter_stats[2] += n_cand;
+    if (n_fb == 0) return;
+    h->f_fb_users.ensure((size_t)n_fb);
+    h->f_fb_keys.ensure((size_t)n_fb);
+    h->f_fb_items.ensure((size_t)(n_fb * topk));
+    h->f_fb_scores.ensure((size_t)(n_fb * topk));
+    hipLaunchKernelGGL(filter_fallback_keys_kernel, dim3((unsigned)((n_fb + kBlk - 1) / kBlk)), dim3(kBlk), 0, h->stream,
+                       h->f_fb_rows.p, n_fb, d_users, u0, excl_row0, excl_by_user ? 1 : 0, h->f_fb_users.p, h->f_fb_keys.p);
+    HIP_CHECK(hipGetLastError());
+    launch_rank_fp32_rows(h, h->f_fb_users.p, 0, n_fb, topk, d_excl_indptr, d_excl_indices, 0, h->f_fb_items.p,
+                          h->f_fb_scores.p, excl_by_user, d_excl_indptr ? h->f_fb_keys.p : nullptr);
+    hipLaunchKernelGGL(filter_fallback_scatter_kernel, dim3((unsigned)((n_fb * topk + kBlk - 1) / kBlk)), dim3(kBlk), 0,
+                       h->stream, h->f_fb_rows.p, n_fb, topk, h->f_fb_items.p, h->f_fb_scores.p, items_out, scores_out);
+    HIP_CHECK(hipGetLastError());
+}
+
+static void launch_rank_fused_rows(cornac_hip_scorer_t h, const int32_t *d_users, int64_t u0, int64_t n, int topk,
+                                   const int64_t *d_excl_indptr, const int32_t *d_excl_indices, int64_t excl_row0,
+                                   int32_t *items_out, float *scores_out, bool excl_by_user) {
+    if (can_filter(h, topk))
+        launch_rank_filter_rows(h, d_users, u0, n, topk, d_excl_indptr, d_excl_indices, excl_row0, items_out, scores_out,
+                                excl_by_user);
+    else
+        launch_rank_fp32_rows(h, d_users, u0, n, topk, d_excl_indptr, d_excl_indices, excl_row0, items_out, scores_out,
+                              excl_by_user);
+}
+
 constexpr int64_t kExclBitmapBudget = int64_t(512) << 20;
 static void launch_rank_fused(cornac_hip_scorer_t h, const int32_t *d_users, int64_t u0, int64_t n, int topk,
                               const int64_t *d_excl_indptr, const int32_t *d_excl_indices, int64_t excl_row0,
                               int32_t *items_out, float *scores_out, bool excl_by_user = false) {
     const int64_t n_item_tiles = (h->n_items + 31) / 32;
     int64_t rows = n;
+    h->filter_stats[0] = h->filter_stats[1] = h->filter_stats[2] = 0;
     if (d_excl_indptr && n_item_tiles <= kMaxBitmapTiles)
         rows = std::max<int64_t>(128, (kExclBitmapBudget / (n_item_tiles * 4)) / 128 * 128);
     for (int64_t r0 = 0; r0 < n; r0 += rows) {
@@ -1155,7 +1358,7 @@
         else HIP_CHECK(hipMemsetAsync(h->item_base.p, 0, (size_t)h->n_items * 4, h->stream));
         h->has_user_base = user_base != nullptr;
         if (user_base) h->user_base.upload(user_base, (size_t)h->n_users, h->stream);
-        build_rank_order(h, U, V, item_base);
+        build_rank_order(h, U, V, item_base, user_base);
         HIP_CHECK(hipStreamSynchronize(h->stream));
         h->is_set = true;
     });
@@ -1444,6 +1647,20 @@
     });
 }
 
+int cornac_hip_scorer_rank_filter(cornac_hip_scorer_t h, int mode, int64_t *stats) {
+    return guarded([&] {
+        sc_check(h, false);
+        REQUIRE(mode == 0 || mode == 1 || mode == -1, "mode must be 0 (fp32 only), 1 (automatic) or -1 (unchanged)");
+        if (mode >= 0) h->filter_mode = mode;
+        if (stats) {
+            stats[0] = h->filter_stats[0];
+            stats[1] = h->filter_stats[1];
+            stats[2] = h->filter_stats[2];
+            stats[3] = h->filter_valid ? 1 : 0;
+        }
+    });
+}
+
 int cornac_hip_scorer_host_buffer(cornac_hip_scorer_t h, size_t bytes, void **out) {
     return guarded([&] {
         sc_check(h);
diff --git a/include/cornac_hip.h b/include/cornac_hip.h
--- a/include/cornac_hip.h
+++ b/include/cornac_hip.h
@@ -265,6 +265,13 @@
                               int32_t *greater_out, int32_t *pos_out, int32_t *ge_out, float *tgt_scores_out);
 int cornac_hip_rank_topk_device(cornac_hip_scorer_t h, int64_t u0, int64_t n, int topk, int repeats, double *ms);
 
+#define CORNAC_HIP_RANK_FILTER_C 0.0079345703125
+#define CORNAC_HIP_RANK_FILTER_BASE_SLACK 0.000030517578125
+#define CORNAC_HIP_RANK_FILTER_USER_BASE_SLACK 0.0000002384185791015625
+#define CORNAC_HIP_RANK_FILTER_MIN_EXP (-40)
+#define CORNAC_HIP_RANK_FILTER_MAX_EXP 40
+int cornac_hip_scorer_rank_filter(cornac_hip_scorer_t h, int mode, int64_t *stats);
+
 typedef struct cornac_hip_knn_sim *cornac_hip_knn_sim_t;
 typedef struct cornac_hip_knn_scorer *cornac_hip_knn_scorer_t;
 #define CORNAC_HIP_KNN_MAX_K 64
```
